# PKU-MARL/HARL

Hardware: AMD Instinct MI355X
Metric: transitions/sec through HAPPO update (MPE spread, 3 agents) (higher is better)
Workload: dtype f32; 1 GPU; MPE simple_spread_v2 3-agent HAPPO update: compute_returns + train(), T=200, n_rollout_threads=4096/GPU (4096 global, weak scaling), obs18/share54/Box5, MLP[128, 128], ppo_epoch=5, critic_epoch=5; episode_length=200, n_rollout_threads_per_gpu=4096, n_rollout_threads_global=4096, n_agents=3, parallelism=dp1, collective=none, world_size=1, ranks_seen=1

## Files before the change

### harl_amd/_lib.py

```python
from __future__ import annotations

import ctypes as C
import os
from typing import Dict, Optional

import torch

from .traffic import algorithmic_bytes, algorithmic_flops

_HERE = os.path.dirname(os.path.abspath(__file__))
LIB_PATH = os.path.join(_HERE, "lib", "libharl_%s.so" % (os.environ.get("HARL_LIB") or "hip"))

PS_STRIDE = 48
DHEAD_LD = 32
SLAB = 32

_vp, _i, _l, _f, _d = C.c_void_p, C.c_int, C.c_long, C.c_float, C.c_double

SIGNATURES = {
    "harl_gae_returns": [_vp] * 8 + [_i, _i, _f, _f, _i, _i, _i, _vp],
    "harl_masked_moments": [_vp, _vp, _l, _vp, _vp, _vp],
    "harl_dist_rows": [_vp, _l, _i, _i, _vp, _f, _f, _vp, _vp, _vp, _i, _i, _vp, _vp, _vp, _vp, _vp, _vp],
    "harl_moments_mean": [_vp, _vp, _vp],
    "harl_clock_probe": [_vp, _l, _vp],
    "harl_build_seq": [_vp, _i, _i, _i, _l, _vp, _vp, _i, _vp, _vp, _vp, _vp, _vp],
    "harl_adv_normalize": [_vp, _vp, _vp, _l, _vp],
    "harl_factor_update": [_vp, _vp, _vp, _l, _i, _i, _vp],
    "harl_sum_sumsq": [_vp, _vp, _l, _vp, _vp],
    "harl_valuenorm_apply": [_vp, _vp, _d, _d, _vp],
    "harl_gradnorm_clip_adam": [_vp, _vp, _vp, _vp, _l, _vp, _i, _f, _d, _d, _d, _f, _f, _d, _d, _vp, _vp],
    "harl_fold_linear": [_vp] * 6 + [_i, _i, _vp],
    "harl_unfold_linear_grads": [_vp, _vp, _i, _vp, _vp, _vp, _vp, _vp, _vp, _vp, _i, _i, _i, _vp],
    "harl_mlp_fwd_input": [_vp, _l, _vp, _l, _i, _vp, _vp, _i, _i, _vp, _vp, _vp, _vp, _vp, _vp, _vp],
    "harl_mlp_x0n_wide": [_vp, _l, _vp, _l, _i, _i, _vp, _vp, _vp, _vp],
    "harl_x0n_multi": [_vp, _i, _i, _vp],
    "harl_mlp_fwd_wide": [_vp, _l, _i, _vp, _i, _vp, _i, _vp, _vp, _vp, _vp, _vp],
    "harl_mlp_linear_wide": [_vp, _l, _i, _vp, _i, _vp, _i, _vp, _vp, _vp],
    "harl_act_ln_fwd": [_vp, _l, _i, _i, _vp, _vp, _vp, _vp],
    "harl_act_bwd": [_vp, _vp, _vp, _vp, _l, _i, _i, _vp],
    "harl_act_ln_tangent": [_vp, _vp, _vp, _vp, _vp, _l, _i, _i, _vp, _vp],
    "harl_mlp_tangent_wide": [_vp, _l, _i, _vp, _i, _vp, _i, _vp, _vp, _vp, _vp, _vp, _vp],
    "harl_mlp_fwd_fused2x": [_vp, _l, _vp, _i, _vp, _vp, _vp, _i, _i, _vp, _vp, _vp, _vp, _vp, _vp, _vp],
    "harl_mlp_fwd_fused2": [_vp, _l, _vp, _l, _i, _vp, _vp, _i, _vp, _vp, _i, _i, _vp, _vp, _vp, _vp, _vp, _vp, _vp, _vp,
                            _vp, _vp],
    "harl_mlp_fwd_hidden": [_vp, _l, _i, _i, _vp, _vp, _vp, _vp, _vp, _vp],
    "harl_mlp_bwd_dx": [_vp, _vp, _vp, _vp, _l, _i, _i, _vp, _vp, _vp, _i, _vp, _i, _vp],
    "harl_mlp_bwd_dx_dw": [_vp, _vp, _vp, _vp, _l, _i, _i, _vp, _vp, _vp, _i, _vp, _vp, _i, _i, _vp],
    "harl_mlp_dw_partials": [_vp, _i, _i, _i, _vp, _i, _l, _vp, _vp, _vp, _i, _l, _vp, _i, _vp],
    "harl_mlp_dw_partials_multi": [_i, _vp, _vp, _vp, _i, _i, _l, _i, _vp],
    "harl_mlp_dw_partials_multi_v": [_i, _vp, _vp, _vp, _i, _vp, _vp, _vp, _l, _i, _vp],
    "harl_gru_dw6": [_vp, _vp, _vp, _vp, _vp, _vp, _vp, _l, _i, _vp],
    "harl_mlp_fwd_trunk": [_vp, _l, _i, _vp, _i, _vp, _i, _vp, _i, _vp, _vp, _vp, _vp, _vp, _vp, _vp, _vp, _vp, _vp],
    "harl_mlp_bwd_trunk": [_l, _i, _i, _vp, _vp, _vp, _vp, _vp, _vp, _vp, _vp, _vp, _vp, _vp],
    "harl_reduce_partials": [_vp, _i, _l, _vp, _vp],
    "harl_reduce_partials_multi": [_vp, _vp, _i, _i, _l, _vp, _vp],
    "harl_adam_fold": [_vp, _vp, _vp, _vp, _l, _vp, _vp, _i, _vp, _vp, _vp, _i, _vp, _i, _f, _i, _i, _vp, _i, _f, _d, _d,
                       _d, _f, _f, _d, _d, _vp, _vp],
    "harl_adam_fold_dev": [_vp, _vp, _vp, _vp, _l, _vp, _vp, _i, _vp, _vp, _vp, _i, _vp, _i, _f, _i, _i, _vp, _i, _f, _vp, _i,
                           _vp, _d, _d, _f, _f, _vp, _vp],
    "harl_pack_scalars_hilo": [_vp, _vp, _vp],
    "harl_reduce_pack_scalars": [_vp, _i, _vp, _vp, _vp],
    "harl_randperm_replay": [_vp, _l, _l, _vp, _vp, _vp],
    "harl_rng_advance": [_vp, _l, _l, _vp],
    "harl_rng_jump": [_vp, _l, _l, _vp],
    "harl_actor_head_logp": [_vp, _l, _i, _vp, _vp, _vp, _f, _f, _i, _i, _vp, _vp, _vp, _vp, _vp, _i, _vp, _l, _l, _vp],
    "harl_actor_head_loss": [_vp, _vp, _vp, _l, _i, _vp, _vp, _vp, _f, _f, _i, _i, _vp, _vp, _vp, _vp, _vp, _vp,
                             _vp, _vp, _d, _f, _i, _i, _l, _l, _vp, _vp, _vp, _vp, _vp, _i, _vp],
    "harl_critic_head_values": [_vp, _l, _i, _vp, _vp, _vp, _vp],
    "harl_critic_head_loss": [_vp, _vp, _vp, _l, _i, _vp, _vp, _vp, _vp, _vp, _vp, _f, _i, _i, _f, _l, _l, _vp, _vp, _vp,
                              _vp, _i, _vp],
    "harl_gru_fwd": [_vp] * 7 + [_i, _i, _l] + [_vp] * 8 + [_i, _vp, _vp],
    "harl_gru_bwd": [_vp] * 9 + [_i, _i, _l] + [_vp] * 8 + [_vp],
    "harl_fold_linear_tangent": [_vp] * 9 + [_i, _i, _vp],
    "harl_fold_table": [_vp, _vp, _vp, _i, _i, _vp],
    "harl_unfold_table": [_vp, _vp, _vp, _vp, _i, _i, _vp],
    "harl_fold_tangent_table": [_vp, _vp, _vp, _vp, _i, _i, _vp],
    "harl_mlp_tangent_input": [_vp, _l, _vp, _l, _i, _vp, _vp, _i, _i, _vp, _vp, _vp, _vp, _vp],
    "harl_gru_gates": [_vp, _vp, _i, _l, _vp, _vp, _vp, _i, _vp],
    "harl_gru_tangent": [_vp] * 15 + [_i, _i, _l, _vp, _vp],
    "harl_mlp_tangent_hidden": [_vp, _vp, _l, _i, _i, _vp, _vp, _vp, _vp, _vp, _vp, _vp, _vp],
    "harl_mlp_tangent_hidden2": [_vp, _vp, _l, _i, _i, _vp, _vp, _vp, _vp, _vp, _vp, _vp, _vp, _vp],
    "harl_actor_head_fvp": [_vp, _vp, _vp, _vp, _l, _i, _vp, _vp, _vp, _vp, _vp, _f, _f, _i, _i, _vp, _l, _l, _vp, _vp, _vp],
    "harl_trpo_kl_sum": [_vp, _vp, _vp, _vp, _f, _f, _l, _i, _i, _vp, _vp],
    "harl_update_supported": [_i, _i, _i, _i],
    "harl_update_fwd_actor": [_vp, _l, _i, _i] + [_vp] * 7 + [_f, _f, _i, _i] + [_vp] * 7 + [_d, _f, _i, _i] + [_vp] * 4 + [_i] + [_vp] * 4,
    "harl_update_logp": [_vp, _l, _i, _i] + [_vp] * 7 + [_f, _f, _i, _i] + [_vp] * 5 + [_i, _vp, _vp],
    "harl_update_last_actor": [_vp, _l, _i] + [_vp] * 5 + [_f, _f, _i, _i] + [_vp] * 8 + [_d, _f, _i, _i] + [_vp] * 4 + [_i, _vp],
    "harl_update_last_critic": [_vp, _l, _i] + [_vp] * 8 + [_f, _i, _i, _f] + [_vp] * 3 + [_i, _vp],
    "harl_update_fwd_critic": [_vp, _l, _i, _i] + [_vp] * 9 + [_f, _i, _i, _f] + [_vp] * 3 + [_i] + [_vp] * 4,
    "harl_update_values": [_vp, _l, _i, _i] + [_vp] * 7 + [_vp],
    "harl_update_bwd": [_vp, _vp, _l, _i, _i] + [_vp] * 5 + [_i, _vp],
    "harl_head_blocks": [_l],
    "harl_trpo_fvp_finish": [_vp, _vp, _vp, _vp, _l, _f, _f, _l, _i, _f, _f, _vp],
    "harl_trpo_cg_step": [_vp, _vp, _vp, _vp, _l, _vp, _vp, _vp],
    "harl_mlp_panel_fwd": [_vp, _l, _i, _vp, _i, _vp, _i, _vp, _vp, _vp, _vp],
    "harl_mlp_panel_bwd": [_vp, _vp, _vp, _vp, _l, _i, _i, _vp, _vp, _vp],
    "harl_head_dw_rows256": [_vp, _l, _i, _vp, _vp, _i, _vp],
    "harl_mlp_panel_tangent": [_vp, _vp, _l, _i, _vp, _vp, _i, _vp, _vp, _vp, _vp, _vp, _vp],
    "harl_reduce_scalars": [_vp, _i, _vp, _vp],
    "harl_mlp_linear": [_vp, _l, _i, _i, _vp, _vp, _vp, _vp],
    "harl_mlp_linear3": [_vp, _vp, _vp, _l, _i, _i, _vp, _vp, _vp, _vp, _vp, _vp, _vp, _vp, _vp, _vp],
    "harl_gru_cell_init": [_vp, _vp, _i, _l, _vp, _vp],
    "harl_gru_cell_fwd": [_vp] * 8 + [_i, _l] + [_vp] * 7 + [_vp],
    "harl_gru_cell_bwd": [_vp] * 10 + [_i, _l] + [_vp] * 5 + [_vp],
    "harl_rownorm": [_vp, _l, _i, _vp, _vp, _vp],
    "harl_gru_cell_tangent": [_vp] * 19 + [_i, _l] + [_vp] * 3,
    "harl_md_head_logp": [_vp, _i, _vp, _i, _vp, _vp, _l, _vp, _vp, _vp, _i, _vp, _i, _vp, _l, _l, _vp],
    "harl_md_head_loss": [_vp, _vp, _i, _vp, _i, _vp, _vp, _l, _vp, _vp, _vp, _i, _vp, _vp, _vp, _vp, _vp, _d, _f, _i, _i,
                          _l, _l, _vp, _vp, _i, _vp],
    "harl_cat_head_logp": [_vp, _i, _vp, _i, _l, _vp, _vp, _vp, _vp, _vp, _vp, _vp, _vp, _l, _l, _vp],
    "harl_cat_head_loss": [_vp, _i, _vp, _i, _l, _vp, _vp, _vp, _vp, _vp, _vp, _vp, _vp, _d, _f, _i, _l, _l, _vp, _vp, _i, _vp],
    "harl_trpo_begin": [_vp, _vp, _l, _i, _vp, _vp, _vp, _vp, _l, _vp, _vp, _vp, _vp],
    "harl_trpo_step": [_vp, _vp, _vp, _vp, _vp, _vp, _l, _f, _vp, _vp, _vp],
    "harl_trpo_ls_candidate": [_vp, _vp, _vp, _vp, _l, _vp],
    "harl_trpo_ls_test": [_vp, _vp, _d, _d, _d, _d, _vp, _vp],
    "harl_reduce_scalars_set": [_vp, _i, _vp, _vp],
    "harl_zero_bytes": [_vp, _l, _vp],
    "harl_comm_create": [_i, _i, _l, _i, _vp, _vp],
    "harl_comm_connect": [_vp, _vp],
    "harl_comm_allreduce": [_vp, _vp, _l, _i, _vp],
    "harl_comm_set_timeout": [_vp, _d],
    "harl_comm_status": [_vp],
    "harl_comm_destroy": [_vp],
    "harl_version": [],
}


class HipLibraryMissing(RuntimeError):
    pass


_lib: Optional[C.CDLL] = None


def load() -> C.CDLL:
    global _lib
    if _lib is not None:
        return _lib
    if not os.path.exists(LIB_PATH):
        raise HipLibraryMissing(
            f"{LIB_PATH} not found: build it with `python -m harl_amd._build` (hipcc, gfx950). "
            "harl_amd has no CPU fallback.")
    lib = C.CDLL(LIB_PATH)
    for name, argtypes in SIGNATURES.items():
        fn = getattr(lib, name)
        fn.argtypes = argtypes
        fn.restype = C.c_int
    lib.harl_last_error.argtypes = []
    lib.harl_last_error.restype = C.c_char_p
    _lib = lib
    return lib


def ptr(t: Optional[torch.Tensor]) -> Optional[int]:
    if t is None:
        return None
    assert t.is_contiguous(), "harl_amd kernels need contiguous tensors"
    return t.data_ptr()


_raw_stream = getattr(torch._C, "_cuda_getCurrentRawStream", None)
_raw_device = getattr(torch._C, "_cuda_getDevice", None)


def stream() -> int:
    if _raw_stream is not None and _raw_device is not None:
        return _raw_stream(_raw_device())
    return torch.cuda.current_stream().cuda_stream

# ... 4 lines not shown

_timing_tags = None


_event_pool: list = []


def reserve_timing_events(n: int) -> None:
    while len(_event_pool) < n:
        _event_pool.append(torch.cuda.Event(enable_timing=True))


def enable_kernel_timing(on: bool, tags=None) -> None:
    global _timing_on, _timing_tags
    _timing_on = bool(on)
    _timing_tags = set(tags) if tags else None
    if on:
        _timing_events.clear()


def collect_kernel_timing() -> dict:
    torch.cuda.synchronize()
    out = {}
    for tag, evs in _timing_events.items():
        ms = [e[0].elapsed_time(e[1]) for e in evs]
        nb = [e[2] for e in evs if e[2] is not None]
        out[tag] = dict(n=len(ms), avg_ms=sum(ms) / max(len(ms), 1), total_ms=sum(ms),
                        bytes=sum(nb) if len(nb) == len(evs) and nb else None,
                        flops=sum(e[3] or 0.0 for e in evs))
    return out


_fn_cache: dict = {}


def call(name: str, *args, tag: Optional[str] = None) -> None:
    fn = _fn_cache.get(name)
    if fn is None:
        fn = _fn_cache[name] = getattr(load(), name)
    if _timing_on and tag is not None and (_timing_tags is None or tag in _timing_tags):
        a = _event_pool.pop() if _event_pool else torch.cuda.Event(enable_timing=True)
        b = _event_pool.pop() if _event_pool else torch.cuda.Event(enable_timing=True)
        a.record()
        rc = fn(*args)
        b.record()
        _timing_events.setdefault(tag, []).append((a, b, algorithmic_bytes(name, args), algorithmic_flops(name, args)))
    else:
        rc = fn(*args)
    if rc != 0:
        raise RuntimeError(f"{name} failed ({rc}): {load().harl_last_error().decode()}")


X0N_MULTI_MAX = 32


class X0nProblem(C.Structure):
    _fields_ = [("X", _vp), ("ldx", _l), ("M", _l), ("D", _i), ("use_ln0", _i), ("x0n", _vp), ("mu0", _vp), ("rstd0", _vp)]


def x0n_multi(problems, max_workgroups: int = 0, tag: Optional[str] = "x0n_multi") -> bool:
    if not 1 <= len(problems) <= X0N_MULTI_MAX:
        return False
    table = (X0nProblem * len(problems))(*[X0nProblem(*p) for p in problems])
    fn = _fn_cache.get("harl_x0n_multi")
    if fn is None:
        fn = _fn_cache["harl_x0n_multi"] = load().harl_x0n_multi
    timed = _timing_on and tag is not None and (_timing_tags is None or tag in _timing_tags)
    if timed:
        a = _event_pool.pop() if _event_pool else torch.cuda.Event(enable_timing=True)
        b = _event_pool.pop() if _event_pool else torch.cuda.Event(enable_timing=True)
        a.record()
    rc = fn(table, len(problems), max_workgroups, stream())
    if rc == 1:
        return False
    if rc != 0:
        raise RuntimeError(f"harl_x0n_multi failed ({rc}): {load().harl_last_error().decode()}")
    if timed:
        b.record()
        nb = sum(4 * ((p[2] + 31) // 32 * 32) * (p[3] + (p[3] + 31) // 32 * 32 + 2) for p in problems)
        _timing_events.setdefault(tag, []).append((a, b, nb, 0.0))
    return True


SCRATCH_BYTES = {"mm": 24640, "cg": 1088}
_scratch: Dict[tuple, torch.Tensor] = {}


def scratch(kind: str) -> int:
    st = torch.cuda.current_stream()
    key = (st.device_index, st.cuda_stream, kind)
    t = _scratch.get(key)
    if t is None:
        t = _scratch[key] = torch.zeros(SCRATCH_BYTES[kind] // 8, dtype=torch.float64, device=torch.device("cuda", st.device_index))
    return t.data_ptr()


def default_device() -> torch.device:
    return torch.device(os.environ.get("HARL_DEVICE") or f"cuda:{int(os.environ.get('LOCAL_RANK', '0'))}")


def require_gpu(device: torch.device) -> None:
    if device.type != "cuda" or not torch.cuda.is_available():
        raise RuntimeError(
            "harl_amd runs on MI355X (PyTorch-ROCm device 'cuda') only; there is no CPU path. "
            f"Got device={device}, torch.cuda.is_available()={torch.cuda.is_available()}")
    load()
```

### harl_amd/csrc/elementwise.hip

```cpp
#include <mutex>
#include <map>
#include <unordered_map>
#include <utility>

#include "common.h"
#include "../../include/harl_hip.h"

#include <cstdio>
#include <cstring>

namespace harl {
bool lds_opt_in_needed(const void *kernel, size_t bytes) {
  static std::mutex mu;
  static std::unordered_map<const void *, size_t> done;
  std::lock_guard<std::mutex> lk(mu);
  size_t &have = done[kernel];
  if (have >= bytes) return false;
  have = bytes;
  return true;
}

static thread_local char g_err[512] = "";
void set_error(const char *msg) {
  std::strncpy(g_err, msg, sizeof(g_err) - 1);
// ... 62 lines not shown
  if (GAE) value_preds[(long)T * N + c] = nv;
  else returns[(long)T * N + c] = nv;
  auto load = [&](int t0, float (&r)[GAE_TC], float (&v0)[GAE_TC], float (&m1)[GAE_TC], float (&b1)[GAE_TC]) {
#pragma unroll
    for (int k = 0; k < GAE_TC; ++k) {
      const int t = t0 - k;
      const bool ok = t >= 0;
      const long o = (long)(ok ? t : 0) * N + c;
      r[k] = rewards[o];
      v0[k] = value_preds[o];
      m1[k] = masks[o + N];
      b1[k] = PTL ? bad_masks[o + N] : 1.f;
    }
  };
  auto scan = [&](int t0, const float (&r)[GAE_TC], const float (&v0)[GAE_TC], const float (&m1)[GAE_TC], const float (&b1)[GAE_TC]) {
#pragma clang fp contract(off)
#pragma unroll
    for (int k = 0; k < GAE_TC; ++k) {
      const int t = t0 - k;
      if (t < 0) break;
      const float dv0 = denorm(ds, v0[k]);
      float ret;
      if (GAE) {
        float delta = r[k] + (gamma * dv1) * m1[k];
        delta = delta - dv0;
        const float carry = FP_ORDER ? (gl * gae) * m1[k] : (gl * m1[k]) * gae;
        gae = delta + carry;
        if (PTL) gae = b1[k] * gae;
        ret = gae + dv0;
        dv1 = dv0;
      } else {
        ret = (ret1 * gamma) * m1[k] + r[k];
        if (PTL) ret = ret * b1[k] + (1.f - b1[k]) * dv0;
        ret1 = ret;
      }
      returns[(long)t * N + c] = ret;
      if (adv) adv[(long)t * N + c] = ret - dv0;
    }
  };
  float rA[GAE_TC], vA[GAE_TC], mA[GAE_TC], bA[GAE_TC], rB[GAE_TC], vB[GAE_TC], mB[GAE_TC], bB[GAE_TC];
  int t0 = T - 1;
  load(t0, rA, vA, mA, bA);
  while (t0 >= 0) {
    if (t0 - GAE_TC >= 0) load(t0 - GAE_TC, rB, vB, mB, bB);
    scan(t0, rA, vA, mA, bA);
    t0 -= GAE_TC;
    if (t0 < 0) break;
    if (t0 - GAE_TC >= 0) load(t0 - GAE_TC, rA, vA, mA, bA);
    scan(t0, rB, vB, mB, bB);
    t0 -= GAE_TC;
  }
}

extern "C" int harl_gae_returns(const float *rewards, float *value_preds, const float *masks,
                                const float *bad_masks, const float *next_value, const float *vn_stats,
                                float *returns, float *advantages, int T, int ncols, float gamma,
                                float gamma_lambda, int use_gae, int use_proper_time_limits, int fp_order,
                                void *stream) {
  if (T <= 0 || ncols <= 0) return 0;
  dim3 block(64), grid((ncols + 63) / 64);
  hipStream_t s = (hipStream_t)stream;
#define LAUNCH(G, P, F)                                                                                     \
  hipLaunchKernelGGL((k_gae<G, P, F>), grid, block, 0, s, rewards, value_preds, masks, bad_masks, next_value, \
                     vn_stats, returns, advantages, T, ncols, gamma, gamma_lambda)
  if (use_gae) {
    if (use_proper_time_limits) {
      if (fp_order) LAUNCH(true, true, true); else LAUNCH(true, true, false);
    } else {
      if (fp_order) LAUNCH(true, false, true); else LAUNCH(true, false, false);
    }
  } else {
    if (use_proper_time_limits) LAUNCH(false, true, false); else LAUNCH(false, false, false);
  }
#undef LAUNCH
  return check_launch("harl_gae_returns");
}

constexpr int MM_MAX_BLOCKS = 1024;
struct MmScratch {
  double part[MM_MAX_BLOCKS][3];
  unsigned ticket;
};

__global__ __launch_bounds__(256) void k_masked_moments(const float *__restrict__ x, const float *__restrict__ active,
                                                        long n, double *__restrict__ out3, MmScratch *__restrict__ ws) {
  double(*g_mm_part)[3] = ws->part;
  unsigned &g_mm_ticket = ws->ticket;
  double s1 = 0, s2 = 0, cnt = 0;
  for (long i = (long)blockIdx.x * blockDim.x + threadIdx.x; i < n; i += (long)gridDim.x * blockDim.x) {
    float a = active ? active[i] : 1.f;
    if (a != 0.f) {
      double v = x[i];
      s1 += v;
      s2 += v * v;
      cnt += 1.0;
    }
  }
  s1 = wave_reduce_sum_d(s1);
  s2 = wave_reduce_sum_d(s2);
  cnt = wave_reduce_sum_d(cnt);
  __shared__ double sh[3][4];
  __shared__ unsigned s_last;
  int w = threadIdx.x >> 6, l = threadIdx.x & 63;
  if (l == 0) {
    sh[0][w] = s1;
    sh[1][w] = s2;
    sh[2][w] = cnt;
  }
  __syncthreads();
  if (threadIdx.x < 3)
    __hip_atomic_store(&g_mm_part[blockIdx.x][threadIdx.x],
                       sh[threadIdx.x][0] + sh[threadIdx.x][1] + sh[threadIdx.x][2] + sh[threadIdx.x][3], __ATOMIC_RELAXED,
                       __HIP_MEMORY_SCOPE_AGENT);
  __syncthreads();
  if (threadIdx.x == 0) {
    __threadfence();
    s_last = __hip_atomic_fetch_add(&g_mm_ticket, 1u, __ATOMIC_ACQ_REL, __HIP_MEMORY_SCOPE_AGENT) == gridDim.x - 1 ? 1u : 0u;
  }
  __syncthreads();
  if (!s_last) return;
  __threadfence();
  __shared__ double red[3][256];
  for (int k = 0; k < 3; ++k) {
    double t = 0;
    for (unsigned b = threadIdx.x; b < gridDim.x; b += 256)
      t += __hip_atomic_load(&g_mm_part[b][k], __ATOMIC_RELAXED, __HIP_MEMORY_SCOPE_AGENT);
    red[k][threadIdx.x] = t;
  }
  __syncthreads();
  if (threadIdx.x < 3) {
    double t = 0;
    for (int i = 0; i < 256; ++i) t += red[threadIdx.x][i];
    out3[threadIdx.x] += t;
  }
}

static_assert(sizeof(MmScratch) <= HARL_MM_SCRATCH_BYTES, "HARL_MM_SCRATCH_BYTES too small");

extern "C" int harl_masked_moments(const float *x, const float *active, long n, double *out3, void *scratch, void *stream) {
  if (n <= 0) return 0;
  long nb = (n + 2047) / 2048;
  if (nb > MM_MAX_BLOCKS) nb = MM_MAX_BLOCKS;
  hipStream_t s = (hipStream_t)stream;
  MmScratch *ws = static_cast<MmScratch *>(scratch);
  if (!ws || (reinterpret_cast<uintptr_t>(ws) & 7) != 0) {
    set_error("harl_masked_moments: scratch must be HARL_MM_SCRATCH_BYTES of 8-byte aligned device memory");
    return -2;
  }
  (void)hipMemsetAsync(&ws->ticket, 0, sizeof(unsigned), s);
  hipLaunchKernelGGL(k_masked_moments, dim3((unsigned)nb), dim3(256), 0, s, x, active, n, out3, ws);
  return check_launch("harl_masked_moments");
}

__global__ __launch_bounds__(256) void k_adv_normalize(const float *__restrict__ adv, const double *__restrict__ mom,
                                                       float *__restrict__ out, long n) {
  double cnt = mom[2];
  double meand = mom[0] / cnt;
  double vard = mom[1] / cnt - meand * meand;
  float mean = (float)meand;
  float denom = (float)sqrt(vard > 0 ? vard : 0.0) + 1e-5f;
  for (long i = (long)blockIdx.x * blockDim.x + threadIdx.x; i < n; i += (long)gridDim.x * blockDim.x)
    out[i] = (adv[i] - mean) / denom;
}

extern "C" int harl_adv_normalize(const float *adv, const double *moments3, float *adv_out, long n, void *stream) {
  if (n <= 0) return 0;
  long nb = (n + 1023) / 1024;
  if (nb > 2048) nb = 2048;
  hipLaunchKernelGGL(k_adv_normalize, dim3((unsigned)nb), dim3(256), 0, (hipStream_t)stream, adv, moments3, adv_out, n);
  return check_launch("harl_adv_normalize");
}

__global__ __launch_bounds__(256) void k_dist_rows(const float *__restrict__ head, long M, int D, int kind,
                                                   const float *__restrict__ log_std, float std_x_coef, float std_y_coef,
                                                   const float *__restrict__ noise, float *__restrict__ actions,
                                                   const int *__restrict__ head_off, int n_heads, int sum_heads,
                                                   float *__restrict__ logp, float *__restrict__ probs,
                                                   float *__restrict__ argmax_out, float *__restrict__ ent_rows,
                                                   float *__restrict__ sigma_out) {
  const long i = (long)blockIdx.x * blockDim.x + threadIdx.x;
  if (kind == 0) {
    if (sigma_out && i < D) sigma_out[i] = (1.0f / (1.0f + expf(-log_std[i] / std_x_coef))) * std_y_coef;
    if (i >= M) return;
    float ent = 0.f;
    for (int d = 0; d < D; ++d) {
      const float sig = (1.0f / (1.0f + expf(-log_std[d] / std_x_coef))) * std_y_coef;
      const float lsig = logf(sig);
      const float mu = head[i * D + d];
      const float a = noise ? mu + sig * noise[i * D + d] : mu;
      if (actions) actions[i * D + d] = a;
      if (logp) {
        const float diff = a - mu;
        logp[i * D + d] = -(diff * diff) / (2.0f * sig * sig) - lsig - 0.9189385332046727f;
      }
      ent += 0.5f + 0.9189385332046727f + lsig;
    }
    if (ent_rows) ent_rows[i] = ent;
    return;
  }
  if (i >= M) return;
  float ent = 0.f, lsum = 0.f;
  for (int hd = 0; hd < n_heads; ++hd) {
    const int lo = head_off ? head_off[hd] : 0, hi = head_off ? head_off[hd + 1] : D;
    int best = lo;
    float bv = head[i * D + lo];
    for (int j = lo; j < hi; ++j) {
      const float lg = head[i * D + j];
      const float p = expf(lg);
      if (probs) probs[i * D + j] = p;
      ent -= fmaxf(lg, -3.4028234663852886e38f) * p;
      if (lg > bv) {
        bv = lg;
        best = j;
      }
    }
    if (argmax_out) argmax_out[i * n_heads + hd] = (float)(best - lo);
    if (logp) {
// ... 59 lines not shown
    return -1;
  }
  const long work = (long)L * m_pad > (long)m_pad * H ? (long)L * m_pad : (long)m_pad * H;
  long blocks = (work + 255) / 256;
  if (blocks > 1024) blocks = 1024;
  hipLaunchKernelGGL(k_build_seq, dim3((unsigned)blocks), dim3(256), 0, (hipStream_t)stream, first, m, m_pad, L, stride,
                     masks_src, h0_src, H, idx, valid_idx, mask_rows, h0);
  return check_launch("harl_build_seq");
}

__global__ void k_clock_probe(long long *__restrict__ out, long long ticks) {
  if (threadIdx.x != 0) return;
  const long long r0 = __builtin_amdgcn_s_memrealtime();
  const long long c0 = __builtin_readcyclecounter();
  long long r;
  do {
    __builtin_amdgcn_s_sleep(64);
    r = __builtin_amdgcn_s_memrealtime();
  } while (r - r0 < ticks);
  out[0] = __builtin_readcyclecounter() - c0;
  out[1] = r - r0;
}

extern "C" int harl_clock_probe(long long *cycles_ticks, long ticks, void *stream) {
  if (ticks <= 0 || ticks > 100000000L) {
    set_error("harl_clock_probe: ticks must be in (0, 1e8]");
    return -1;
  }
  hipLaunchKernelGGL(k_clock_probe, dim3(1), dim3(64), 0, (hipStream_t)stream, cycles_ticks, (long long)ticks);
  return check_launch("harl_clock_probe");
}

__global__ __launch_bounds__(256) void k_factor_update(float *__restrict__ factor, const float *__restrict__ nl,
                                                       const float *__restrict__ ol, long n, int D, int agg_mean) {
  for (long i = (long)blockIdx.x * blockDim.x + threadIdx.x; i < n; i += (long)gridDim.x * blockDim.x) {
    float acc = agg_mean ? 0.f : 1.f;
    for (int d = 0; d < D; ++d) {
      float r = expf(nl[i * D + d] - ol[i * D + d]);
      acc = agg_mean ? acc + r : acc * r;
    }
    if (agg_mean) acc = acc / (float)D;
    factor[i] = factor[i] * acc;
  }
}

extern "C" int harl_factor_update(float *factor, const float *new_logp, const float *old_logp, long n, int act_dim,
                                  int agg_mean, void *stream) {
  if (n <= 0) return 0;
  long nb = (n + 255) / 256;
  if (nb > 2048) nb = 2048;
  hipLaunchKernelGGL(k_factor_update, dim3((unsigned)nb), dim3(256), 0, (hipStream_t)stream, factor, new_logp, old_logp,
                     n, act_dim, agg_mean);
  return check_launch("harl_factor_update");
}

__global__ __launch_bounds__(256) void k_sum_sumsq(const float *__restrict__ x, const int64_t *__restrict__ idx, long m,
                                                   double *__restrict__ out2) {
  double s1 = 0, s2 = 0;
  for (long i = (long)blockIdx.x * blockDim.x + threadIdx.x; i < m; i += (long)gridDim.x * blockDim.x) {
    double v = x[idx ? idx[i] : i];
    s1 += v;
    s2 += v * v;
  }
  s1 = wave_reduce_sum_d(s1);
  s2 = wave_reduce_sum_d(s2);
  __shared__ double sh[2][4];
  int w = threadIdx.x >> 6, l = threadIdx.x & 63;
  if (l == 0) {
    sh[0][w] = s1;
    sh[1][w] = s2;
  }
  __syncthreads();
  if (threadIdx.x < 2) atomicAdd(&out2[threadIdx.x], sh[threadIdx.x][0] + sh[threadIdx.x][1] + sh[threadIdx.x][2] + sh[threadIdx.x][3]);
}

extern "C" int harl_sum_sumsq(const float *x, const int64_t *idx, long m, double *sums2, void *stream) {
  if (m <= 0) return 0;
  long nb = (m + 2047) / 2048;
  if (nb > 1024) nb = 1024;
  hipLaunchKernelGGL(k_sum_sumsq, dim3((unsigned)nb), dim3(256), 0, (hipStream_t)stream, x, idx, m, sums2);
  return check_launch("harl_sum_sumsq");
}

__global__ void k_valuenorm_apply(float *__restrict__ vn, const double *__restrict__ sums2, double count, float w,
                                  float omw) {
#pragma clang fp contract(off)
  if (threadIdx.x == 0 && blockIdx.x == 0) {
    float bm = (float)(sums2[0] / count);
    float bsq = (float)(sums2[1] / count);
    float rm = vn[0] * w;
    vn[0] = rm + bm * omw;
    float rs = vn[1] * w;
    vn[1] = rs + bsq * omw;
    float db = vn[2] * w;
    vn[2] = db + omw;
  }
}

extern "C" int harl_valuenorm_apply(float *vn_stats, const double *sums2, double count, double beta, void *stream) {
  float w = (float)beta;
  float omw = (float)(1.0 - beta);
  hipLaunchKernelGGL(k_valuenorm_apply, dim3(1), dim3(64), 0, (hipStream_t)stream, vn_stats, sums2, count, w, omw);
  return check_launch("harl_valuenorm_apply");
}

__global__ __launch_bounds__(1024) void k_gradnorm_clip_adam(float *__restrict__ p, const float *__restrict__ g,
                                                             float *__restrict__ m, float *__restrict__ v, long n,
                                                             const float *__restrict__ grad_scale, int use_clip,
                                                             float max_norm, float lr_over_bc1, float beta1,
                                                             float beta2, float omb1, float omb2, float eps, float wd,
                                                             float bc2_sqrt, double *__restrict__ info_out) {
  const float scale = grad_scale ? *grad_scale : 1.f;
  double ss = 0;
  for (long i = threadIdx.x; i < n; i += blockDim.x) {
    float gi = g[i] * scale;
    ss += (double)gi * gi;
  }
  ss = wave_reduce_sum_d(ss);
  __shared__ double sh[16];
  __shared__ float s_coef;
  int w = threadIdx.x >> 6, l = threadIdx.x & 63;
  if (l == 0) sh[w] = ss;
  __syncthreads();
  if (threadIdx.x == 0) {
    double t = 0;
    for (int i = 0; i < (int)(blockDim.x >> 6); ++i) t += sh[i];
    float norm = (float)sqrt(t);
    float coef = 1.f;
    if (use_clip) {
      coef = max_norm / (norm + 1e-6f);
      coef = coef > 1.f ? 1.f : coef;
    }
    s_coef = coef;
    if (info_out) info_out[0] += norm;
  }
  __syncthreads();
  const float coef = s_coef * scale;
  for (long i = threadIdx.x; i < n; i += blockDim.x) {
    float gi = g[i] * coef;
    float pi = p[i];
    if (wd != 0.f) gi = gi + wd * pi;
    float mi = m[i];
    mi = mi + omb1 * (gi - mi);
    float vi = v[i] * beta2 + (omb2 * gi) * gi;
    m[i] = mi;
    v[i] = vi;
    float denom = sqrtf(vi) / bc2_sqrt + eps;
    p[i] = pi - lr_over_bc1 * (mi / denom);
  }
}

extern "C" int harl_gradnorm_clip_adam(float *param, float *grad, float *exp_avg, float *exp_avg_sq, long n,
                                       const float *grad_scale, int use_clip, float max_norm, double lr, double beta1,
                                       double beta2, float eps, float weight_decay, double bias_correction1,
                                       double bias_correction2, double *info_out, void *stream) {
  if (n <= 0) return 0;
  float step_size = (float)(lr / bias_correction1);
  float bc2_sqrt = (float)sqrt(bias_correction2);
  hipLaunchKernelGGL(k_gradnorm_clip_adam, dim3(1), dim3(1024), 0, (hipStream_t)stream, param, grad, exp_avg,
                     exp_avg_sq, n, grad_scale, use_clip, max_norm, step_size, (float)beta1, (float)beta2,
                     (float)(1.0 - beta1), (float)(1.0 - beta2), eps, weight_decay, bc2_sqrt, info_out);
  return check_launch("harl_gradnorm_clip_adam");
}

__global__ __launch_bounds__(64) void k_fold_linear(const float *__restrict__ W, const float *__restrict__ b,
                                                    const float *__restrict__ gamma, const float *__restrict__ beta,
// ... 279 lines not shown
  __shared__ double sh[16][64];
  const int j = threadIdx.x & 63, rg = threadIdx.x >> 6;
  double s = 0;
  if (j < PS_STRIDE)
    for (int b = rg; b < n_blocks; b += 16) s += (double)ps[(long)b * PS_STRIDE + j];
  sh[rg][j] = s;
  __syncthreads();
  if (threadIdx.x < PS_STRIDE) {
    double r = 0;
#pragma unroll
    for (int g = 0; g < 16; ++g) r += sh[g][threadIdx.x];
    out[threadIdx.x] = r;
#pragma unroll
    for (int k = 0; k < HILO_PIECES; ++k) {
      const double p = trunc(r / HILO_Q[k]) * HILO_Q[k];
      hilo[k * PS_STRIDE + threadIdx.x] = (float)p;
      r -= p;
    }
  }
}

extern "C" int harl_reduce_pack_scalars(const float *part_scalars, int n_blocks, double *scalars, float *hilo, void *stream) {
  if (n_blocks > 0 && !part_scalars) { set_error("harl_reduce_pack_scalars: part_scalars is NULL"); return -2; }
  hipLaunchKernelGGL(k_reduce_pack_scalars, dim3(1), dim3(1024), 0, (hipStream_t)stream, part_scalars, n_blocks, scalars, hilo);
  return check_launch("harl_reduce_pack_scalars");
}

constexpr int TS = 12;

__global__ __launch_bounds__(64) void k_unfold_table(const float *__restrict__ p, float *__restrict__ g,
                                                     const float *__restrict__ dwp, const int *__restrict__ tab, int n_layers) {
  int k = blockIdx.x, l = 0;
  for (; l < n_layers; ++l) {
    if (k < tab[l * TS + 5]) break;
    k -= tab[l * TS + 5];
  }
  if (l >= n_layers) return;
  const int *t = tab + l * TS;
  const int O = t[4], K = t[5], kp = t[9], op = t[10], go = t[2], beo = t[3];
  const float *dW_ = dwp + t[8];
  const float *db_ = dW_ + (long)op * kp;
  const float gam = go >= 0 ? p[go + k] : 1.f, bet = beo >= 0 ? p[beo + k] : 0.f;
  for (int o = threadIdx.x; o < O; o += 64) {
    const float d = dW_[(long)o * kp + k], dbo = db_[o];
    g[t[0] + (long)o * K + k] = d * gam + dbo * bet;
    if (k == 0) g[t[1] + o] = dbo;
  }
  if (go < 0) return;
  for (int l2 = 0; l2 < l; ++l2)
    if (tab[l2 * TS + 2] == go) return;
  float accg = 0.f, accb = 0.f;
  bool first = true;
  for (int l2 = l; l2 < n_layers; ++l2) {
    const int *t2 = tab + l2 * TS;
    if (t2[2] != go) continue;
    const int O2 = t2[4], K2 = t2[5], kp2 = t2[9], op2 = t2[10];
    const float *dW2 = dwp + t2[8];
    const float *db2 = dW2 + (long)op2 * kp2;
    double sg = 0.0, sb = 0.0;
    for (int o = threadIdx.x; o < O2; o += 64) {
      const float w = p[t2[0] + (long)o * K2 + k];
      sg += (double)w * (double)dW2[(long)o * kp2 + k];
      sb += (double)w * (double)db2[o];
    }
    sg = wave_reduce_sum_d(sg);
    sb = wave_reduce_sum_d(sb);
    accg = first ? (float)sg : (float)((double)accg + sg);
    accb = first ? (float)sb : (float)((double)accb + sb);
    first = false;
  }
  if (threadIdx.x == 0) {
    g[go + k] = accg;
    g[beo + k] = accb;
  }
}

extern "C" int harl_unfold_table(const float *param, float *grad, const float *dwp, const int *table, int n_layers,
                                 int total_cols, void *stream) {
  if (n_layers <= 0 || total_cols <= 0) return 0;
  hipLaunchKernelGGL(k_unfold_table, dim3(total_cols), dim3(64), 0, (hipStream_t)stream, param, grad, dwp, table, n_layers);
  return check_launch("harl_unfold_table");
}

__global__ __launch_bounds__(64) void k_fold_table(const float *__restrict__ p, float *__restrict__ packs,
                                                   const int *__restrict__ tab, int n_layers) {
  int o = blockIdx.x, l = 0;
  for (; l < n_layers; ++l) {
    if (o < tab[l * TS + 4]) break;
    o -= tab[l * TS + 4];
  }
  if (l >= n_layers) return;
  const int *t = tab + l * TS;
  const int in_dim = t[5];
  const float *W = p + t[0], *b = p + t[1];
  const float *gamma = t[2] >= 0 ? p + t[2] : nullptr, *beta = t[3] >= 0 ? p + t[3] : nullptr;
  float *Wp = packs + t[6], *bp = packs + t[7];
  float acc = 0.f;
  for (int k = threadIdx.x; k < in_dim; k += 64) {
    float w = W[(long)o * in_dim + k];
    Wp[(long)o * in_dim + k] = gamma ? w * gamma[k] : w;
    if (beta) acc += w * beta[k];
  }
  acc = wave_reduce_sum(acc);
  if (threadIdx.x == 0) bp[o] = b[o] + acc;
}

extern "C" int harl_fold_table(const float *param, float *packs, const int *table, int n_layers, int total_rows, void *stream) {
  if (n_layers <= 0 || total_rows <= 0) return 0;
  hipLaunchKernelGGL(k_fold_table, dim3(total_rows), dim3(64), 0, (hipStream_t)stream, param, packs, table, n_layers);
  return check_launch("harl_fold_table");
}

__global__ __launch_bounds__(64) void k_fold_tangent_table(const float *__restrict__ p, const float *__restrict__ vec,
                                                           float *__restrict__ packd, const int *__restrict__ tab, int n_layers) {
  int o = blockIdx.x, l = 0;
  for (; l < n_layers; ++l) {
    if (o < tab[l * TS + 4]) break;
    o -= tab[l * TS + 4];
  }
  if (l >= n_layers) return;
  const int *t = tab + l * TS;
  const int K = t[5], go = t[2], beo = t[3];
  const float *W = p + t[0] + (long)o * K, *Wd = vec + t[0] + (long)o * K;
  float *Wpd = packd + t[6] + (long)o * K;
  float acc = 0.f;
  for (int k = threadIdx.x; k < K; k += 64) {
    const float w = W[k], wd = Wd[k];
    Wpd[k] = go >= 0 ? wd * p[go + k] + w * vec[go + k] : wd;
    if (beo >= 0) acc += wd * p[beo + k] + w * vec[beo + k];
  }
  acc = wave_reduce_sum(acc);
  if (threadIdx.x == 0) packd[t[7] + o] = vec[t[1] + o] + acc;
}

extern "C" int harl_fold_tangent_table(const float *param, const float *vec, float *pack_d, const int *table, int n_layers,
                                       int total_rows, void *stream) {
  if (n_layers <= 0 || total_rows <= 0) return 0;
  hipLaunchKernelGGL(k_fold_tangent_table, dim3(total_rows), dim3(64), 0, (hipStream_t)stream, param, vec, pack_d, table,
                     n_layers);
  return check_launch("harl_fold_tangent_table");
}

#ifndef HARL_REDUCE_DEPTH
#define HARL_REDUCE_DEPTH 16
#endif
__global__ __launch_bounds__(256) void k_reduce_partials_multi(const float *__restrict__ part, const int *__restrict__ tab,
                                                               int n_layers, int n_wg, float *__restrict__ dwp) {
  __shared__ double sh[4][64];
  const int lane = threadIdx.x & 63, rg = threadIdx.x >> 6;
  long e = (long)blockIdx.x * 64 + lane;
  double total = 0.0;
  long out_idx = -1;
  for (int l = 0; l < n_layers; ++l) {
    const int *t = tab + l * TS;
    const long elems = (long)t[10] * t[9] + t[10];
    if (e < elems) {
      const float *p = part + (long)t[11] + e;
      constexpr int RD = HARL_REDUCE_DEPTH;
      double acc[RD];
#pragma unroll
      for (int u = 0; u < RD; ++u) acc[u] = 0.0;
      int w = rg;
      for (; w + 4 * (RD - 1) < n_wg; w += 4 * RD) {
        float v[RD];
#pragma unroll
        for (int u = 0; u < RD; ++u) v[u] = p[(long)(w + 4 * u) * elems];
#pragma unroll
        for (int u = 0; u < RD; ++u) acc[u] += (double)v[u];
      }
      for (; w < n_wg; w += 4) acc[0] += (double)p[(long)w * elems];
#pragma unroll
      for (int st = 1; st < RD; st *= 2)
#pragma unroll
        for (int u = 0; u + st < RD; u += 2 * st) acc[u] += acc[u + st];
      total = acc[0];
      out_idx = t[8] + e;
      break;
    }
    e -= elems;
  }
  sh[rg][lane] = total;
  __syncthreads();
  if (rg == 0 && out_idx >= 0) dwp[out_idx] = (float)((sh[0][lane] + sh[1][lane]) + (sh[2][lane] + sh[3][lane]));
}

extern "C" int harl_reduce_partials_multi(const float *part, const int *table, int n_layers, int n_wg, long total_elems,
                                          float *dwp, void *stream) {
  if (total_elems <= 0) return 0;
  hipLaunchKernelGGL(k_reduce_partials_multi, dim3((unsigned)((total_elems + 63) / 64)), dim3(256), 0,
                     (hipStream_t)stream, part, table, n_layers, n_wg, dwp);
  return check_launch("harl_reduce_partials_multi");
}

// ... 674 lines not shown
```

### harl_amd/csrc/heads.hip

```cpp
#include "common.h"
#include "../../include/harl_hip.h"

using namespace harl;

#include "heads_common.h"

namespace {

template <int H, int DAP, bool DISCRETE, bool TRAIN, bool FUSE = false>
__global__ __launch_bounds__(WG_THREADS, (FUSE && DAP <= 8) ? 2 : 1) void k_actor_head(ActorArgs A) {
  extern __shared__ __attribute__((aligned(16))) float lds[];
  PHASE_BEGIN();
  float *whl = lds;
  float *cst = whl + 2 * (H / 2) * DAP;
  float *red = cst + 7 * DAP;
  float *dwl = red + 4 * PS_STRIDE;
  constexpr bool LDSACC = FUSE && DAP <= 8;
  constexpr int HROWS = DAP <= 8 ? DAP : 8;
  float *hacc = dwl + WAVES_PER_WG * HeadDw<H>::WAVE_FLOATS;
  if (FUSE)
    for (int e = threadIdx.x; e < WAVES_PER_WG * HeadDw<H>::WAVE_FLOATS; e += WG_THREADS) dwl[e] = 0.f;
  if (LDSACC)
    for (int e = threadIdx.x; e < WAVES_PER_WG * HROWS * H; e += WG_THREADS) hacc[e] = 0.f;
  stage_head<H, DAP>(whl, cst, A.Whp, A.bhp, A.act_dim);
// ... 410 lines not shown
  for (int k = threadIdx.x; k < in_dim; k += 64) {
    const float w = W[(long)o * in_dim + k], wd = Wd[(long)o * in_dim + k];
    Wpd[(long)o * in_dim + k] = g ? wd * g[k] + w * gd[k] : wd;
    if (be) acc += wd * be[k] + w * bed[k];
  }
  acc = wave_reduce_sum(acc);
  if (threadIdx.x == 0) bpd[o] = bd[o] + acc;
}

template <int H, int DAP, bool DISC>
void launch_fvp(const FvpArgs &A, int grid, hipStream_t s) {
  const size_t shm = ((size_t)4 * (H / 2) * DAP + 10 * DAP) * sizeof(float);
  allow_big_lds(k_actor_head_fvp<H, DAP, DISC>, shm);
  hipLaunchKernelGGL((k_actor_head_fvp<H, DAP, DISC>), dim3(grid), dim3(WG_THREADS), shm, s, A);
}

int head_grid(long M) { return persistent_grid(n_slabs_of(M), 4); }

template <int H, int DAP, bool DISC, bool TRAIN>
void launch_actor(const ActorArgs &A, int grid, hipStream_t s) {
  const size_t base = ((size_t)2 * (H / 2) * DAP + 7 * DAP + 4 * PS_STRIDE) * sizeof(float);
  if constexpr (TRAIN && DAP <= 32) {
    if (A.dw_part) {
      size_t fl = (size_t)WAVES_PER_WG * HeadDw<H>::WAVE_FLOATS;
      if (fl < (size_t)HeadDw<H>::OUT_FLOATS) fl = HeadDw<H>::OUT_FLOATS;
      if (DAP <= 8) fl = (size_t)WAVES_PER_WG * HeadDw<H>::WAVE_FLOATS + (size_t)WAVES_PER_WG * DAP * H;
      const size_t shm = base + fl * sizeof(float);
      allow_big_lds(k_actor_head<H, DAP, DISC, true, true>, shm);
      hipLaunchKernelGGL((k_actor_head<H, DAP, DISC, true, true>), dim3(grid), dim3(WG_THREADS), shm, s, A);
      return;
    }
  }
  hipLaunchKernelGGL((k_actor_head<H, DAP, DISC, TRAIN>), dim3(grid), dim3(WG_THREADS), base, s, A);
}

template <bool TRAIN>
int dispatch_actor(const ActorArgs &A, int H, int discrete, int grid, hipStream_t s) {
  const int D = A.act_dim;
  if (D < 1 || D > 64 || (D > 32 && !discrete)) {
    set_error("actor head: act_dim must be in [1, 32] (Categorical heads: [1, 64])");
    return -2;
  }
  if (D > 32 && A.dw_part) {
    set_error("actor head: the fused head weight gradient stops at 32 outputs (pass dw_part = NULL and run harl_mlp_dw_partials on the ATL(64) dhead image)");
    return -2;
  }
  const int dap = D <= 4 ? 4 : (D <= 8 ? 8 : (D <= 16 ? 16 : (D <= 32 ? 32 : 64)));
#define CASE(Hv, DAPv)                                                    \
  if (H == Hv && dap == DAPv) {                                           \
    if (discrete) launch_actor<Hv, DAPv, true, TRAIN>(A, grid, s);        \
    else launch_actor<Hv, DAPv, false, TRAIN>(A, grid, s);                \
    return check_launch("harl_actor_head");                               \
  }
  CASE(128, 4) CASE(128, 8) CASE(128, 16) CASE(128, 32) CASE(64, 4) CASE(64, 8) CASE(64, 16) CASE(64, 32)
  CASE(256, 4) CASE(256, 8) CASE(256, 16) CASE(256, 32)
#undef CASE
  if (dap == 64 && (H == 64 || H == 128)) {
    if (H == 64) launch_actor<64, 64, true, TRAIN>(A, grid, s);
    else launch_actor<128, 64, true, TRAIN>(A, grid, s);
    return check_launch("harl_actor_head");
  }
  set_error("actor head: hidden width must be 64 or 128");
  return -2;
}
}

HARL_PHASE_ACCESSOR(heads)

extern "C" int harl_head_blocks(long M) { return head_grid(M); }

extern "C" int harl_actor_head_logp(const float *xL, long M, int H, const float *Whp, const float *bhp,
                                    const float *log_std, float std_x_coef, float std_y_coef, int discrete,
                                    int act_dim, const float *actions, const float *avail, float *logp_out,
                                    const float *old_logp, float *factor, int agg_mean, float *head_out, long m_valid,
                                    long m_pad, void *stream) {
  if (M <= 0) return 0;
  ActorArgs A{};
  A.head_out = head_out;
  A.m_valid = m_valid; A.m_pad = m_pad;
  A.xL = xL; A.M = M; A.Whp = Whp; A.bhp = bhp; A.log_std = log_std;
  A.std_x_coef = std_x_coef; A.std_y_coef = std_y_coef; A.act_dim = act_dim;
  A.actions = actions; A.avail = avail; A.old_logp = old_logp; A.agg_mean = agg_mean;
  A.logp_out = logp_out; A.factor_out = factor; A.n_slabs = n_slabs_of(M);
  if (factor && !old_logp) {
    set_error("harl_actor_head_logp: factor update needs old_logp");
    return -2;
  }
  return dispatch_actor<false>(A, H, discrete, head_grid(M), (hipStream_t)stream);
}

extern "C" int harl_actor_head_loss(const float *xL, const uint32_t *relu_mask, const float *rstd, long M, int H,
                                    const float *Whp, const float *bhp, const float *log_std, float std_x_coef,
                                    float std_y_coef, int discrete, int act_dim, const int64_t *idx,
                                    const float *actions, const float *avail, const float *old_logp, const float *adv,
                                    const double *adv_moments, const float *factor, const float *active,
                                    double clip_param, float entropy_coef, int agg_mean, int trpo, long m_valid,
                                    long m_pad, float *logp_out, float *dzL, float *dhead, float *part_scalars,
                                    float *dw_part, int n_wg, void *stream) {
  if (M <= 0) return 0;
  ActorArgs A{};
  A.trpo = trpo;
  A.logp_out = logp_out;
  A.dw_part = dw_part;
  if (dw_part && n_wg <= 0) { set_error("harl_actor_head_loss: fused head gradient needs n_wg > 0"); return -2; }
  A.m_valid = m_valid; A.m_pad = m_pad;
  A.xL = xL; A.relu_mask = relu_mask; A.rstd = rstd; A.M = M; A.Whp = Whp; A.bhp = bhp; A.log_std = log_std;
  A.std_x_coef = std_x_coef; A.std_y_coef = std_y_coef; A.act_dim = act_dim; A.idx = idx;
  A.actions = actions; A.avail = avail; A.old_logp = old_logp; A.adv = adv; A.adv_moments = adv_moments;
  A.factor_in = factor; A.active = active; A.entropy_coef = entropy_coef;
  A.clip_lo = (float)(1.0 - clip_param); A.clip_hi = (float)(1.0 + clip_param);
  A.agg_mean = agg_mean; A.dzL = dzL; A.dhead = dhead; A.part_scalars = part_scalars; A.n_slabs = n_slabs_of(M);
  return dispatch_actor<true>(A, H, discrete, dw_part ? n_wg : head_grid(M), (hipStream_t)stream);
}

extern "C" int harl_critic_head_values(const float *xL, long M, int H, const float *Whp, const float *bhp,
                                       float *values, void *stream) {
  if (M <= 0) return 0;
  CriticArgs A{};
  A.xL = xL; A.M = M; A.Whp = Whp; A.bhp = bhp; A.values_out = values; A.n_slabs = n_slabs_of(M);
  const int grid = head_grid(M);
  const size_t shm = ((size_t)2 * (H / 2) * 4 + 20 + 4 * PS_STRIDE) * sizeof(float);
  if (H == 128) hipLaunchKernelGGL((k_critic_head<128, false>), dim3(grid), dim3(WG_THREADS), shm, (hipStream_t)stream, A);
  else if (H == 64) hipLaunchKernelGGL((k_critic_head<64, false>), dim3(grid), dim3(WG_THREADS), shm, (hipStream_t)stream, A);
  else if (H == 256) hipLaunchKernelGGL((k_critic_head<256, false>), dim3(grid), dim3(WG_THREADS), shm, (hipStream_t)stream, A);
  else { set_error("critic head: hidden width must be 64, 128 or 256"); return -2; }
  return check_launch("harl_critic_head_values");
}

extern "C" int harl_critic_head_loss(const float *xL, const uint32_t *relu_mask, const float *rstd, long M, int H,
                                     const float *Whp, const float *bhp, const int64_t *idx, const float *value_preds,
                                     const float *returns, const float *vn_stats, float clip_param, int use_clipped,
                                     int use_huber, float huber_delta, long m_valid, long m_pad, float *dzL, float *dhead,
                                     float *part_scalars, float *dw_part, int n_wg, void *stream) {
  if (M <= 0) return 0;
  CriticArgs A{};
  A.m_valid = m_valid; A.m_pad = m_pad;
  A.xL = xL; A.relu_mask = relu_mask; A.rstd = rstd; A.M = M; A.Whp = Whp; A.bhp = bhp; A.idx = idx;
  A.value_preds = value_preds; A.returns = returns; A.vn_stats = vn_stats; A.clip_param = clip_param;
  A.huber_delta = huber_delta; A.use_clipped = use_clipped; A.use_huber = use_huber; A.dzL = dzL; A.dhead = dhead;
  A.part_scalars = part_scalars; A.n_slabs = n_slabs_of(M);
  A.dw_part = dw_part;
  if (dw_part && n_wg <= 0) { set_error("harl_critic_head_loss: fused head gradient needs n_wg > 0"); return -2; }
  const int grid = dw_part ? n_wg : head_grid(M);
  const size_t base = ((size_t)2 * (H / 2) * 4 + 20 + 4 * PS_STRIDE) * sizeof(float);
  hipStream_t s = (hipStream_t)stream;
#define CL(Hv)                                                                                                     \
  if (H == Hv) {                                                                                                   \
    if (dw_part) {                                                                                                 \
      const size_t fl = (size_t)WAVES_PER_WG * HeadDw<Hv>::WAVE_FLOATS + (size_t)WAVES_PER_WG * Hv;    \
      const size_t shm = base + fl * sizeof(float);                                                                \
      allow_big_lds(k_critic_head<Hv, true, true>, shm);                                                           \
      hipLaunchKernelGGL((k_critic_head<Hv, true, true>), dim3(grid), dim3(WG_THREADS), shm, s, A);                \
    } else {                                                                                                       \
      hipLaunchKernelGGL((k_critic_head<Hv, true>), dim3(grid), dim3(WG_THREADS), base, s, A);                     \
    }                                                                                                              \
    return check_launch("harl_critic_head_loss");                                                                  \
  }
  CL(128) CL(64) CL(256)
#undef CL
  set_error("critic head: hidden width must be 64 or 128");
  return -2;
}

extern "C" int harl_actor_head_fvp(const float *xL, const float *xLdot, const uint32_t *relu_mask, const float *rstd, long M,
                                   int H, const float *Whp, const float *bhp, const float *Whdp, const float *bhdp,
                                   const float *log_std, float std_x_coef, float std_y_coef, int discrete, int act_dim,
// ... 52 lines not shown
```

### harl_amd/csrc/heads_common.h

```cpp
#pragma once
#include "common.h"

using namespace harl;

namespace {
constexpr float LOG_SQRT_2PI = 0.918938533204672741780329736406f;
constexpr float HALF_LOG_2PI_PLUS_HALF = 1.418938533204672741780329736406f;

struct ActorArgs {
  const float *xL;
  const uint32_t *relu_mask;
  const float *rstd;
  long M;
  const float *Whp, *bhp, *log_std;
  float std_x_coef, std_y_coef;
  int act_dim;
  const int64_t *idx;
  const float *actions, *avail, *old_logp, *adv;
  const double *adv_moments;
  const float *factor_in, *active;
  float clip_lo, clip_hi, entropy_coef;
  int agg_mean;
  float *dzL, *dhead, *part_scalars;
  float *dw_part;
// ... 364 lines not shown
        float *p = buf + 32 * H + lane;
        *p = (w == 0 ? 0.f : *p) + v;
      }
    }
    __syncthreads();
  }
  for (int e = threadIdx.x; e < HeadDw<H>::OUT_FLOATS; e += WG_THREADS) out[e] = buf[e];
}

template <int DAP>
__device__ __forceinline__ void store_dhead(float *__restrict__ dhead, long slab, int lane, const float (&dzh)[DAP]) {
  const int i = lane & 31, h = lane >> 5;
  if constexpr (DAP <= 32) {
    float *dh = dhead + (slab * SLAB + i) * DHEAD_LD + 16 * h;
#pragma unroll
    for (int c = 0; c < 16; ++c) {
      float v0 = 0.f, v1 = 0.f;
      if (c < DAP) v0 = dzh[c < DAP ? c : 0];
      if (16 + c < DAP) v1 = dzh[16 + c < DAP ? 16 + c : 0];
      dh[c] = h ? v1 : v0;
    }
  } else {
    static_assert(DAP == 64, "wide heads are padded to 64 outputs");
    float v[32];
#pragma unroll
    for (int R = 0; R < 32; ++R) {
      const int f0 = 32 * (R >> 4) + (R & 3) + 8 * ((R & 15) >> 2);
      v[R] = h ? dzh[f0 + 4] : dzh[f0];
    }
    atl_store<64>(dhead, slab, lane, v);
  }
}

template <int NV>
__device__ __forceinline__ void block_reduce_store(float (&v)[NV], float *red , float *out_row) {
  const int lane = threadIdx.x & 63, wave = wave_id();
#pragma unroll
  for (int k = 0; k < NV; ++k) {
    float t = wave_reduce_sum(v[k]);
    if (lane == 0) red[wave * PS_STRIDE + k] = t;
  }
  __syncthreads();
  if (threadIdx.x < PS_STRIDE) {
    float t = 0.f;
    if (threadIdx.x < NV)
      t = (red[0 * PS_STRIDE + threadIdx.x] + red[1 * PS_STRIDE + threadIdx.x]) +
          (red[2 * PS_STRIDE + threadIdx.x] + red[3 * PS_STRIDE + threadIdx.x]);
    out_row[threadIdx.x] = t;
  }
}

template <int DAP>
struct ActorRow {
  float a[DAP];
  float olp[DAP];
  float av[DAP];
  float act, adv, fct;
};
template <int DAP, bool DISCRETE, bool TRAIN, int DA = 0>
__device__ __forceinline__ void actor_row_load(const ActorArgs &A, long slab, int lane, ActorRow<DAP> &R) {
  const int i = lane & 31;
  const int D = DA ? DA : A.act_dim;
  const long j = slab * SLAB + i;
  const long jc = j < A.M ? j : A.M - 1;
  const long row = A.idx ? A.idx[jc] : jc;
  const long orow = TRAIN ? row : jc;
  if (!DISCRETE) {
#pragma unroll
    for (int d = 0; d < DAP; ++d) {
      R.a[d] = (A.actions && d < D) ? A.actions[row * D + d] : 0.f;
      R.olp[d] = ((TRAIN || A.old_logp) && d < D) ? A.old_logp[orow * D + d] : 0.f;
    }
  } else {
    R.a[0] = A.actions ? A.actions[row] : 0.f;
    R.olp[0] = (TRAIN || A.old_logp) ? A.old_logp[orow] : 0.f;
#pragma unroll
    for (int d = 0; d < DAP; ++d) R.av[d] = (A.avail && d < D) ? A.avail[row * D + d] : 1.f;
  }
  if (TRAIN) {
    R.act = A.active ? A.active[row] : 1.f;
    R.adv = A.adv[row];
    R.fct = A.factor_in ? A.factor_in[row] : 1.f;
  } else {
    R.fct = A.factor_out ? A.factor_out[jc] : 1.f;
  }
}

__device__ __forceinline__ long row_index_request(const int64_t *idx, const float *mapped, long slab, int lane, long M) {
  const long j = slab * SLAB + (lane & 31);
  const long jc = j < M ? j : M - 1;
  const int64_t *p = idx ? idx + jc : reinterpret_cast<const int64_t *>(mapped);
  return *p;
}
__device__ __forceinline__ long row_index_resolve(const int64_t *idx, long raw, long slab, int lane, long M) {
  const long j = slab * SLAB + (lane & 31);
  return idx ? raw : (j < M ? j : M - 1);
}
template <int DAP, bool DISCRETE, bool TRAIN, int DA>
__device__ __forceinline__ void actor_row_load_at(const ActorArgs &A, long slab, int lane, long row, ActorRow<DAP> &R) {
  static_assert(DA > 0 && DA <= DAP, "compile-time action width");
  const long j = slab * SLAB + (lane & 31);
  const long jc = j < A.M ? j : A.M - 1;
  const long orow = TRAIN ? row : jc;
  const float *mapped = A.Whp;
  const bool has_olp = TRAIN || A.old_logp;
  if (!DISCRETE) {
    const float *ap = A.actions ? A.actions + row * DA : mapped;
    const float *op = has_olp ? A.old_logp + orow * DA : mapped;
#pragma unroll
    for (int d = 0; d < DAP; ++d) {
      R.a[d] = d < DA ? ap[d < DA ? d : 0] : 0.f;
      R.olp[d] = d < DA ? op[d < DA ? d : 0] : 0.f;
    }
  } else {
    R.a[0] = *(A.actions ? A.actions + row : mapped);
    R.olp[0] = *(has_olp ? A.old_logp + orow : mapped);
    const float *vp = A.avail ? A.avail + row * DA : mapped;
#pragma unroll
    for (int d = 0; d < DAP; ++d) R.av[d] = d < DA ? vp[d < DA ? d : 0] : 1.f;
  }
  if (TRAIN) {
    R.act = *(A.active ? A.active + row : mapped);
    R.adv = A.adv[row];
    R.fct = *(A.factor_in ? A.factor_in + row : mapped);
  } else {
    R.fct = *(A.factor_out ? A.factor_out + jc : mapped);
  }
}

template <int DAP, bool DISCRETE, bool TRAIN, int DA = 0>
__device__ __forceinline__ bool actor_sample(const ActorArgs &A, const float *cst, float (&z)[DAP], long slab, int lane,
                                             float adv_mean, float adv_den, float (&sc)[8 + DAP], float (&dzh)[DAP],
                                             float &s1_out, float &s2_out, const ActorRow<DAP> &R) {
  const int i = lane & 31, h = lane >> 5;
  const int D = DA ? DA : A.act_dim;
  const int act_w = DISCRETE ? 1 : D;
  const float inv_D = uniform_f(1.0f / (float)D);
  float zlin[DAP];
#pragma unroll
  for (int d = 0; d < DAP; ++d) zlin[d] = z[d] - cst[d];

  const long j = slab * SLAB + i;
  const bool valid = j < A.M && (A.m_pad == 0 || (j % A.m_pad) < A.m_valid);
  const long jc = j < A.M ? j : A.M - 1;
  const long row = A.idx ? A.idx[jc] : jc;
  const bool count_me = valid && h == 0;

#pragma unroll
  for (int d = 0; d < DAP; ++d) dzh[d] = 0.f;

  float imp = 1.f;
  float ratio_d[DAP];
  float ent = 0.f;
  float logp_d[DAP];

  if (!DISCRETE) {
    float prod = 1.f, sum = 0.f;
#pragma unroll
    for (int d = 0; d < DAP; ++d) {
      ratio_d[d] = 1.f;
      logp_d[d] = 0.f;
      if (d < D) {
        const float sig = cst[DAP + d], lsig = cst[2 * DAP + d];
        const float a = A.actions ? R.a[d] : z[d];
        const float diff = a - z[d];
        const float var = sig * sig;
        const float lp = -(diff * diff) * (0.5f * cst[6 * DAP + d]) - lsig - LOG_SQRT_2PI;
        logp_d[d] = lp;
        ent += HALF_LOG_2PI_PLUS_HALF + lsig;
        if (TRAIN || A.old_logp) {
          const float r = expf(lp - R.olp[d]);
          ratio_d[d] = r;
          prod *= r;
          sum += r;
        }
      }
    }
    imp = A.agg_mean ? sum * inv_D : prod;
  } else {
    float mx = -3.0e38f;
#pragma unroll
    for (int d = 0; d < DAP; ++d) {
      if (d < D) {
        if (A.avail && R.av[d] == 0.f) z[d] = -1e10f;
        mx = fmaxf(mx, z[d]);
      }
    }
    float se = 0.f;
#pragma unroll
    for (int d = 0; d < DAP; ++d)
      if (d < D) se += expf(z[d] - mx);
    const float lse = mx + logf(se);
    const int a = A.actions ? (int)R.a[0] : 0;
    float lpa = 0.f;
#pragma unroll
    for (int d = 0; d < DAP; ++d) {
      logp_d[d] = 0.f;
      ratio_d[d] = 0.f;
      if (d < D) {
        const float lp = z[d] - lse;
        logp_d[d] = lp;
        const float p = expf(lp);
        ratio_d[d] = p;
        ent -= fmaxf(lp, -3.4028234663852886e38f) * p;
        if (d == a) lpa = lp;
      }
    }
    if (TRAIN || A.old_logp) imp = expf(lpa - R.olp[0]);
    z[0] = lpa;
  }

  if (!TRAIN) {
    if (valid && h == 0 && A.head_out) {
#pragma unroll
      for (int d = 0; d < DAP; ++d)
        if (d < D) A.head_out[j * D + d] = DISCRETE ? logp_d[d] : z[d];
    }
    if (valid && h == 0) {
      if (A.logp_out) {
        if (DISCRETE) A.logp_out[j] = z[0];
        else {
#pragma unroll
          for (int d = 0; d < DAP; ++d)
            if (d < D) A.logp_out[j * D + d] = logp_d[d];
        }
      }
      if (A.factor_out) A.factor_out[j] = R.fct * imp;
    }
    return false;
  }

  if (A.logp_out && valid && h == 0) {
    if (DISCRETE) A.logp_out[j] = z[0];
    else {
#pragma unroll
      for (int d = 0; d < DAP; ++d)
        if (d < D) A.logp_out[j * D + d] = logp_d[d];
    }
  }
  const float act = A.active ? R.act : 1.f;
  const float advn = (R.adv - adv_mean) * adv_den;
  const float fct = A.factor_in ? R.fct : 1.f;
  const float lo = A.clip_lo, hi = A.clip_hi;
  const float surr1 = imp * advn;
  const float impc = fminf(fmaxf(imp, lo), hi);
  const float surr2 = impc * advn;
  const float mn = fminf(surr1, surr2);
  const float inrange = (imp >= lo && imp <= hi) ? 1.f : 0.f;
  float gsel = surr1 < surr2 ? 1.f : (surr1 > surr2 ? inrange : 0.5f + 0.5f * inrange);
  if (A.trpo != 0) gsel = 1.f;
  const float dimp = valid ? (A.trpo == 1 ? fct * act * advn : -fct * act * advn * gsel) : 0.f;
  const float ecoef = (valid && A.trpo != 1) ? -A.entropy_coef * act : 0.f;

  if (count_me) {
    sc[0] += A.trpo == 1 ? surr1 * fct * act : -fct * (A.trpo == 2 ? surr1 : mn) * act;
    sc[1] += act;
    sc[2] += ent * act;
    sc[3] += imp;
    sc[4] += 1.f;
  }

  if (!DISCRETE) {
#pragma unroll
    for (int d = 0; d < DAP; ++d) {
      if (d < D) {
        const float sig = cst[DAP + d];
        const float var = sig * sig;
        const float a = R.a[d];
        const float diff = a - z[d];
        const float dlp = dimp * (A.agg_mean ? ratio_d[d] * inv_D : imp);
        const float isig = cst[5 * DAP + d], ivar = cst[6 * DAP + d];
        dzh[d] = dlp * diff * ivar;
        const float dsig = dlp * (diff * diff * ivar * isig - isig) + ecoef * isig;
        if (h == 0) sc[8 + d] += dsig * cst[3 * DAP + d];
      }
    }
  } else {
    const int a = (int)R.a[0];
    const float dlp = dimp * imp;
#pragma unroll
    for (int d = 0; d < DAP; ++d) {
      if (d < D) {
        const float p = ratio_d[d];
        const float onehot = d == a ? 1.f : 0.f;
        dzh[d] = dlp * (onehot - p) + ecoef * (-p * (logp_d[d] + ent));
        if (p == 0.f) dzh[d] = dlp * onehot;
      }
    }
  }
  float s1 = 0.f, s2 = 0.f;
#pragma unroll
  for (int d = 0; d < DAP; ++d) {
    s1 += dzh[d] * cst[4 * DAP + d];
    s2 += dzh[d] * zlin[d];
  }
  s1_out = s1;
  s2_out = s2;
  return true;
}

struct CriticArgs {
  const float *xL;
  const uint32_t *relu_mask;
  const float *rstd;
  long M;
  const float *Whp, *bhp;
  const int64_t *idx;
  const float *value_preds, *returns, *vn_stats;
  float clip_param, huber_delta;
  long m_valid, m_pad;
// ... 66 lines not shown
```

### harl_amd/csrc/update.hip

```cpp
#include <type_traits>
#include "common.h"
#include "split_mfma.h"
#include "heads_common.h"
#include "mfma_transpose.h"
#include "../../include/harl_hip.h"

using namespace harl;

namespace {

int bad(const char *m) {
  set_error(m);
  return -2;
}

template <int H, bool MASK>
__device__ __forceinline__ void relu_ln(const f32x16 (&acc)[H / 32], float (&v)[H / 2], uint32_t (&bits)[(H / 2 + 31) / 32],
                                        float &rstd_out) {
  constexpr int NR = H / 2;
#pragma unroll
  for (int w = 0; w < (NR + 31) / 32; ++w) bits[w] = 0u;
#pragma unroll
  for (int R = 0; R < NR; ++R) {
    if constexpr (MASK) v[R] = relu_push(acc[R >> 4][R & 15], bits[R >> 5]);
// ... 579 lines not shown
#define CASE(Hv, Kv)                                                                \
  if (H == Hv && kp0 == Kv) {                                                       \
    const int rc = launch_actor_width<Hv, Kv, TRAIN>(U, A, discrete, s);             \
    return rc ? rc : check_launch("harl_update_fwd");                               \
  }
  CASE(128, 32) CASE(128, 64) CASE(64, 32) CASE(64, 64)
#undef CASE
  return bad("harl_update_fwd: hidden width must be 64 or 128");
}

int dispatch_last_actor(const UpdFwdArgs &U, const ActorArgs &A, int H, int discrete, hipStream_t s) {
  const int D = A.act_dim;
  if (D < 1 || D > 8) return bad("harl_update_last_actor: act_dim must be in [1, 8]");
  int rc;
  if (H == 128) rc = launch_actor_width<128, 0, true>(U, A, discrete, s);
  else if (H == 64) rc = launch_actor_width<64, 0, true>(U, A, discrete, s);
  else return bad("harl_update_last_actor: hidden width must be 64 or 128");
  return rc ? rc : check_launch("harl_update_last_actor");
}

int dispatch_last_critic(const UpdFwdArgs &U, const CriticArgs &A, int H, hipStream_t s) {
  int rc;
  if (H == 128) rc = launch_fwd<128, 0, 1, false, true, CriticArgs>(U, A, s);
  else if (H == 64) rc = launch_fwd<64, 0, 1, false, true, CriticArgs>(U, A, s);
  else return bad("harl_update_last_critic: hidden width must be 64 or 128");
  return rc ? rc : check_launch("harl_update_last_critic");
}

template <bool TRAIN>
int dispatch_fwd_critic(const UpdFwdArgs &U, const CriticArgs &A, int H, hipStream_t s) {
  const int kp0 = U.D <= 32 ? 32 : 64;
#define CASE(Hv, Kv)                                                     \
  if (H == Hv && kp0 == Kv) {                                            \
    const int rc = launch_fwd<Hv, Kv, 1, false, TRAIN, CriticArgs>(U, A, s); \
    return rc ? rc : check_launch("harl_update_fwd");                        \
  }
  CASE(128, 32) CASE(128, 64) CASE(64, 32) CASE(64, 64)
#undef CASE
  return bad("harl_update_fwd: hidden width must be 64 or 128");
}

}

HARL_PHASE_ACCESSOR(update)

extern "C" int harl_update_supported(int D, int H, int act_dim, int kind) {
  if (!(D >= 0 && D <= 64 && (H == 64 || H == 128) && act_dim >= 1 && act_dim <= 8)) return 0;
  const int dap = act_dim <= 4 ? 4 : 8;
  const int hrows = kind == 0 ? 0 : (kind == 2 ? 1 : act_dim);
  return fwd_lds_bytes(H, D == 0 ? 0 : (D <= 32 ? 32 : 64), dap, hrows, kind == 2 ? 1 : act_dim) <= LDS_PER_WG_MAX ? 1 : 0;
}

extern "C" int harl_update_fwd_actor(const float *x0n, long M, int D, int H, const float *W1p, const float *b1p,
                                     const float *W2p, const float *b2p, const float *Whp, const float *bhp,
                                     const float *log_std, float std_x_coef, float std_y_coef, int discrete, int act_dim,
                                     const float *actions, const float *avail, const float *old_logp, const float *adv,
                                     const double *adv_moments, const float *factor, const float *active,
                                     double clip_param, float entropy_coef, int agg_mean, int trpo, float *logp_out,
                                     float *dz2, float *part_scalars, float *dw_part_head, int n_part_rows, float *xh1,
                                     uint32_t *rmask1, float *rstd1, void *stream) {
  if (M <= 0) return 0;
  if (D < 1 || D > 64) return bad("harl_update_fwd_actor: input width must be <= 64");
  if (!dz2 || !part_scalars || !dw_part_head || n_part_rows <= 0) return bad("harl_update_fwd_actor: missing outputs");
  if (xh1 && (!rmask1 || !rstd1)) return bad("harl_update_fwd_actor: xh1 needs rmask1 and rstd1");
  UpdFwdArgs U{x0n, W1p, b1p, W2p, b2p, D, n_slabs_of(M), dz2, n_part_rows, xh1, rmask1, rstd1};
  if (fwd_grid(U.n_slabs) > n_part_rows) return bad("harl_update_fwd_actor: n_part_rows smaller than the launch grid");
  ActorArgs A{};
  A.trpo = trpo;
  A.logp_out = logp_out;
  A.dw_part = dw_part_head;
  A.M = M; A.Whp = Whp; A.bhp = bhp; A.log_std = log_std;
  A.std_x_coef = std_x_coef; A.std_y_coef = std_y_coef; A.act_dim = act_dim;
  A.actions = actions; A.avail = avail; A.old_logp = old_logp; A.adv = adv; A.adv_moments = adv_moments;
  A.factor_in = factor; A.active = active; A.entropy_coef = entropy_coef;
  A.clip_lo = (float)(1.0 - clip_param); A.clip_hi = (float)(1.0 + clip_param);
  A.agg_mean = agg_mean; A.part_scalars = part_scalars; A.n_slabs = U.n_slabs;
  return dispatch_fwd_actor<true>(U, A, H, discrete, (hipStream_t)stream);
}

extern "C" int harl_update_logp(const float *x0n, long M, int D, int H, const float *W1p, const float *b1p,
                                const float *W2p, const float *b2p, const float *Whp, const float *bhp,
                                const float *log_std, float std_x_coef, float std_y_coef, int discrete, int act_dim,
                                const float *actions, const float *avail, float *logp_out, const float *old_logp,
                                float *factor, int agg_mean, float *head_out, void *stream) {
  if (M <= 0) return 0;
  if (D < 1 || D > 64) return bad("harl_update_logp: input width must be <= 64");
  if (factor && !old_logp) return bad("harl_update_logp: factor update needs old_logp");
  UpdFwdArgs U{x0n, W1p, b1p, W2p, b2p, D, n_slabs_of(M), nullptr, 0, nullptr, nullptr, nullptr};
  ActorArgs A{};
  A.head_out = head_out;
  A.M = M; A.Whp = Whp; A.bhp = bhp; A.log_std = log_std;
  A.std_x_coef = std_x_coef; A.std_y_coef = std_y_coef; A.act_dim = act_dim;
  A.actions = actions; A.avail = avail; A.old_logp = old_logp; A.agg_mean = agg_mean;
  A.logp_out = logp_out; A.factor_out = factor; A.n_slabs = U.n_slabs;
  return dispatch_fwd_actor<false>(U, A, H, discrete, (hipStream_t)stream);
}

extern "C" int harl_update_fwd_critic(const float *x0n, long M, int D, int H, const float *W1p, const float *b1p,
                                      const float *W2p, const float *b2p, const float *Whp, const float *bhp,
                                      const float *value_preds, const float *returns, const float *vn_stats,
                                      float clip_param, int use_clipped, int use_huber, float huber_delta, float *dz2,
                                      float *part_scalars, float *dw_part_head, int n_part_rows, float *xh1,
                                      uint32_t *rmask1, float *rstd1, void *stream) {
  if (M <= 0) return 0;
  if (D < 1 || D > 64) return bad("harl_update_fwd_critic: input width must be <= 64");
  if (!dz2 || !part_scalars || !dw_part_head || n_part_rows <= 0) return bad("harl_update_fwd_critic: missing outputs");
  if (xh1 && (!rmask1 || !rstd1)) return bad("harl_update_fwd_critic: xh1 needs rmask1 and rstd1");
  UpdFwdArgs U{x0n, W1p, b1p, W2p, b2p, D, n_slabs_of(M), dz2, n_part_rows, xh1, rmask1, rstd1};
  if (fwd_grid(U.n_slabs) > n_part_rows) return bad("harl_update_fwd_critic: n_part_rows smaller than the launch grid");
  CriticArgs A{};
  A.M = M; A.Whp = Whp; A.bhp = bhp;
  A.value_preds = value_preds; A.returns = returns; A.vn_stats = vn_stats; A.clip_param = clip_param;
  A.huber_delta = huber_delta; A.use_clipped = use_clipped; A.use_huber = use_huber;
  A.part_scalars = part_scalars; A.n_slabs = U.n_slabs;
  A.dw_part = dw_part_head;
  return dispatch_fwd_critic<true>(U, A, H, (hipStream_t)stream);
}

extern "C" int harl_update_last_actor(const float *xin, long M, int H, const float *Wp, const float *bp, const float *Whp,
                                      const float *bhp, const float *log_std, float std_x_coef, float std_y_coef,
                                      int discrete, int act_dim, const int64_t *idx, const float *actions,
                                      const float *avail, const float *old_logp, const float *adv,
                                      const double *adv_moments, const float *factor, const float *active,
                                      double clip_param, float entropy_coef, int agg_mean, int trpo, float *logp_out,
                                      float *dz, float *part_scalars, float *dw_part_head, int n_part_rows, void *stream) {
  if (M <= 0) return 0;
  if (!xin || !dz || !part_scalars || !dw_part_head || n_part_rows <= 0) return bad("harl_update_last_actor: missing arguments");
  UpdFwdArgs U{xin, nullptr, nullptr, Wp, bp, 0, n_slabs_of(M), dz, n_part_rows, nullptr, nullptr, nullptr};
  if (fwd_grid(U.n_slabs) > n_part_rows) return bad("harl_update_last_actor: n_part_rows smaller than the launch grid");
  ActorArgs A{};
  A.trpo = trpo;
  A.logp_out = logp_out;
  A.dw_part = dw_part_head;
  A.M = M; A.Whp = Whp; A.bhp = bhp; A.log_std = log_std;
  A.std_x_coef = std_x_coef; A.std_y_coef = std_y_coef; A.act_dim = act_dim; A.idx = idx;
  A.actions = actions; A.avail = avail; A.old_logp = old_logp; A.adv = adv; A.adv_moments = adv_moments;
  A.factor_in = factor; A.active = active; A.entropy_coef = entropy_coef;
  A.clip_lo = (float)(1.0 - clip_param); A.clip_hi = (float)(1.0 + clip_param);
  A.agg_mean = agg_mean; A.part_scalars = part_scalars; A.n_slabs = U.n_slabs;
  return dispatch_last_actor(U, A, H, discrete, (hipStream_t)stream);
}

extern "C" int harl_update_last_critic(const float *xin, long M, int H, const float *Wp, const float *bp, const float *Whp,
                                       const float *bhp, const int64_t *idx, const float *value_preds, const float *returns,
                                       const float *vn_stats, float clip_param, int use_clipped, int use_huber,
                                       float huber_delta, float *dz, float *part_scalars, float *dw_part_head,
                                       int n_part_rows, void *stream) {
  if (M <= 0) return 0;
  if (!xin || !dz || !part_scalars || !dw_part_head || n_part_rows <= 0) return bad("harl_update_last_critic: missing arguments");
  UpdFwdArgs U{xin, nullptr, nullptr, Wp, bp, 0, n_slabs_of(M), dz, n_part_rows, nullptr, nullptr, nullptr};
  if (fwd_grid(U.n_slabs) > n_part_rows) return bad("harl_update_last_critic: n_part_rows smaller than the launch grid");
  CriticArgs A{};
  A.M = M; A.Whp = Whp; A.bhp = bhp; A.idx = idx;
  A.value_preds = value_preds; A.returns = returns; A.vn_stats = vn_stats; A.clip_param = clip_param;
  A.huber_delta = huber_delta; A.use_clipped = use_clipped; A.use_huber = use_huber;
  A.part_scalars = part_scalars; A.n_slabs = U.n_slabs;
  A.dw_part = dw_part_head;
  return dispatch_last_critic(U, A, H, (hipStream_t)stream);
}

extern "C" int harl_update_values(const float *x0n, long M, int D, int H, const float *W1p, const float *b1p,
                                  const float *W2p, const float *b2p, const float *Whp, const float *bhp, float *values,
                                  void *stream) {
  if (M <= 0) return 0;
  if (D < 1 || D > 64) return bad("harl_update_values: input width must be <= 64");
  UpdFwdArgs U{x0n, W1p, b1p, W2p, b2p, D, n_slabs_of(M), nullptr, 0, nullptr, nullptr, nullptr};
  CriticArgs A{};
  A.M = M; A.Whp = Whp; A.bhp = bhp; A.values_out = values; A.n_slabs = U.n_slabs;
  return dispatch_fwd_critic<false>(U, A, H, (hipStream_t)stream);
}

extern "C" int harl_update_bwd(const float *x0n, const float *dz2, long M, int D, int H, const float *W1p,
                               const float *b1p, const float *W2p, float *dw_part1, float *dw_part2, int n_part_rows,
                               void *stream) {
  if (M <= 0) return 0;
  if (D < 1 || D > 64) return bad("harl_update_bwd: input width must be <= 64");
  if (!dw_part1 || !dw_part2 || n_part_rows <= 0) return bad("harl_update_bwd: missing outputs");
// ... 25 lines not shown
```

### harl_amd/dropin.py

```python
from __future__ import annotations

import os
import runpy
import sys
import types
from typing import Optional

_INSTALLED = False


def stub_optional_modules() -> None:
    def missing(name):
        try:
            __import__(name)
            return False
        except ImportError:
            return True

    if missing("absl"):
        absl, flags = types.ModuleType("absl"), types.ModuleType("absl.flags")
        flags.FLAGS = lambda argv: argv
        absl.flags = flags
        sys.modules["absl"], sys.modules["absl.flags"] = absl, flags
    if missing("setproctitle"):
        sp = types.ModuleType("setproctitle")
        sp.setproctitle = lambda s: None
        sys.modules["setproctitle"] = sp
    if missing("tensorboardX"):
        tb = types.ModuleType("tensorboardX")

        class SummaryWriter:
            def __init__(self, *a, **k):
                self.scalars = {}

            def add_scalars(self, main_tag, tag_scalar_dict, global_step=None):
                for k, v in tag_scalar_dict.items():
                    self.scalars.setdefault(f"{main_tag}/{k}", []).append((global_step, float(v)))

            def export_scalars_to_json(self, path):
                import json
                with open(path, "w", encoding="utf-8") as f:
                    json.dump(self.scalars, f)

            def close(self):
                pass

        tb.SummaryWriter = SummaryWriter
        sys.modules["tensorboardX"] = tb


def _runner_class(base_cls, ours):
    import torch

    class Runner(base_cls):
        __doc__ = f"harl_amd drop-in: {base_cls.__module__}.{base_cls.__name__} + device-resident {ours.__name__} methods"

        _init_update_state = ours._init_update_state
        _ensure_update_state = ours._ensure_update_state
        _critic_first_ok = getattr(ours, "_critic_first_ok", None)
        _prepare_inputs = ours._prepare_inputs
        _fp_normalised_advantages = ours._fp_normalised_advantages
        _check_comms = ours._check_comms
        warmup = ours.warmup
        insert = ours.insert
        compute = ours.compute
        train = ours.train
        after_update = ours.after_update

        def __init__(self, *a, **k):
            super().__init__(*a, **k)
            if not self.algo_args["render"]["use_render"]:
                from .dist import Comm
                self.comm = Comm()
                self._critic_comm = self.comm.second_group()
                self._init_update_state()

        @torch.no_grad()
        def collect(self, step):
            values, actions, logp, rnn, rnn_c = ours.collect(self, step)
            return values, actions.cpu().numpy(), logp, rnn, rnn_c

    Runner.__name__ = ours.__name__
    Runner.__qualname__ = ours.__name__
    return Runner


def install(reference_root: Optional[str] = None, stubs: bool = True) -> dict:
    global _INSTALLED
    if reference_root and reference_root not in sys.path:
        sys.path.insert(0, reference_root)
    if stubs:
        stub_optional_modules()
    import harl.algorithms.actors as ref_actors
    import harl.runners as ref_runners
    import harl.runners.on_policy_base_runner as base

    from . import buffers, runner, valuenorm
    from .happo import HAA2C, HAPPO
    from .hatrpo import HATRPO
    from .mappo import MAPPO
    from .v_critic import VCritic

    ours_algos = {"happo": HAPPO, "hatrpo": HATRPO, "haa2c": HAA2C, "mappo": MAPPO}
    ref_actors.ALGO_REGISTRY.update(ours_algos)
    base.ALGO_REGISTRY = ref_actors.ALGO_REGISTRY
    base.VCritic = VCritic
    base.ValueNorm = valuenorm.ValueNorm
    base.OnPolicyActorBuffer = buffers.OnPolicyActorBuffer
    base.OnPolicyCriticBufferEP = buffers.OnPolicyCriticBufferEP
    base.OnPolicyCriticBufferFP = buffers.OnPolicyCriticBufferFP
    ha = _runner_class(base.OnPolicyBaseRunner, runner.OnPolicyHARunner)
    ma = _runner_class(base.OnPolicyBaseRunner, runner.OnPolicyMARunner)
    installed = {"happo": ha, "hatrpo": ha, "haa2c": ha, "mappo": ma}
    ref_runners.RUNNER_REGISTRY.update(installed)
    _INSTALLED = True
    return installed


def main(argv=None) -> None:
    argv = list(sys.argv[1:] if argv is None else argv)
    ref = os.environ.get("HARL_REFERENCE")
    if "--reference" in argv:
        i = argv.index("--reference")
        ref = argv[i + 1]
        del argv[i:i + 2]
    if "--" in argv:
        argv.remove("--")
    if not ref or not os.path.exists(os.path.join(ref, "examples", "train.py")):
        raise SystemExit("harl_amd.dropin: --reference /path/to/HARL (or HARL_REFERENCE) must contain examples/train.py")
    install(ref)
    sys.argv = [os.path.join(ref, "examples", "train.py")] + argv
    runpy.run_path(sys.argv[0], run_name="__main__")


if __name__ == "__main__":
    main()
```

### harl_amd/happo.py

```python
from __future__ import annotations

import os
from typing import Optional

import numpy as np
import torch

from . import _lib, graphs
from ._lib import PS_STRIDE, call, ptr, stream
from .buffers import OnPolicyActorBuffer, consume_randperm, minibatch_indices, rng_sync
from .dist import Comm, local_minibatch_rows
from .nets import FusedAdam, StochasticPolicy, build_seq, seq_compact
from .valuenorm import _as_dev


class OnPolicyBase:

    def __init__(self, args, obs_space, act_space, device=torch.device("cuda:0")):
        self.args = args
        self.device = torch.device(device)
        _lib.require_gpu(self.device)
        self.tpdv = dict(dtype=torch.float32, device=self.device)
        self.data_chunk_length = args["data_chunk_length"]
        self.use_recurrent_policy = args["use_recurrent_policy"]
        self.use_naive_recurrent_policy = args["use_naive_recurrent_policy"]
        self.use_policy_active_masks = args["use_policy_active_masks"]
        self.action_aggregation = args["action_aggregation"]
        self.lr = args["lr"]
        self.opti_eps = args["opti_eps"]
        self.weight_decay = args["weight_decay"]
        self.obs_space = obs_space
        self.act_space = act_space
        self.actor = StochasticPolicy(args, obs_space, act_space, self.device)
        self.actor_optimizer = FusedAdam(self.actor, self.lr, self.opti_eps, self.weight_decay)
        self.comm = Comm()
        self.shard = None
        self._old_logp: Optional[torch.Tensor] = None
        self._graph = graphs.GraphedStep("the actor")
        self._graph_bufs: dict = {}
        self._graph_gen = None

    def graph_stats(self) -> dict:
        return self._graph.stats()

    def _graph_config_ok(self) -> bool:
        return (graphs.enabled() and not (self.use_recurrent_policy or self.use_naive_recurrent_policy)
                and not self.actor.recurrent and not self.actor.grouped and not self.comm.enabled and self.shard is None)

    def _graph_stage(self, name: str, t: Optional[torch.Tensor]) -> Optional[torch.Tensor]:
        if t is None:
            return None
        b = self._graph_bufs.get(name)
        if b is None or b.shape != t.shape or b.dtype != t.dtype or b.device != t.device:
            b = self._graph_bufs[name] = torch.empty_like(t, memory_format=torch.contiguous_format)
        b.copy_(t)
        return b

    def lr_decay(self, episode, episodes):
        lr = self.lr - (self.lr * ((episode - 1) / float(episodes)))
        for g in self.actor_optimizer.param_groups:
            g["lr"] = lr

    def _logp_pass(self, obs, actions, avail, M, logp_out, old_logp=None, factor=None, head_out=None,
                   rnn_states=None, masks=None, h_last=False, reuse_trunk=False):
        net = self.actor
        agg = int(self.action_aggregation == "mean")
        if net.grouped and not net.recurrent:
            if not reuse_trunk:
                net.forward_trunk(obs, None, M, for_backward=False)
            net.md_logits(M)
            if net.cat_wide:
                call("harl_cat_head_logp", *net.cat_layout(), M, None, ptr(actions), ptr(avail), ptr(logp_out), None,
                     ptr(old_logp), ptr(factor), ptr(head_out), 0, 0, stream(), tag="cat_head_logp")
                return None
            call("harl_md_head_logp", *net.md_layout(), M, ptr(actions), ptr(logp_out), ptr(old_logp),
                 0 if old_logp is None else old_logp.shape[1], ptr(factor), agg, ptr(head_out), 0, 0, stream(),
                 tag="md_head_logp")
            return None
        if not reuse_trunk and net.fused_update_ok(None, train=False):
            call("harl_update_logp", *net.fused_args(obs, M), ptr(net.log_std()), net.std_x_coef, net.std_y_coef,
                 int(net.discrete), net.act_dim, ptr(actions), ptr(avail), ptr(logp_out), ptr(old_logp), ptr(factor), agg,
                 ptr(head_out), stream(), tag="update_logp")
            return None
        if not net.recurrent:
            if not reuse_trunk:
                net.forward_trunk(obs, None, M, for_backward=False)
            Wp, bp = net._packs[-1]
            call("harl_actor_head_logp", ptr(net.xh[-1]), M, net.hidden_sizes[-1], ptr(Wp), ptr(bp), ptr(net.log_std()),
                 net.std_x_coef, net.std_y_coef, int(net.discrete), net.act_dim, ptr(actions), ptr(avail), ptr(logp_out),
                 ptr(old_logp), ptr(factor), agg, ptr(head_out), 0, 0, stream(), tag="actor_head_logp")
            return None
        H = net.hidden_sizes[-1]
        m = rnn_states.shape[0]
        L = M // m
        HS = H * net.recurrent_n
        seq = build_seq(self.device, L, m, HS, h0=_as_dev(rnn_states, self.device).reshape(m, HS),
                        masks_src=_as_dev(masks, self.device), want_h_last=h_last)
        idx, Mp = seq["idx"], L * seq["m_pad"]
        padded = idx is not None
        g = (lambda t: None if t is None else t[idx].contiguous()) if padded else (lambda t: t)
        tmp = (lambda t: None if t is None else torch.empty(Mp, *t.shape[1:], **self.tpdv)) if padded else (lambda t: t)
        a_p, av_p, old_p, f_p = g(actions), g(avail), g(old_logp), g(factor)
        lo_p, ho_p = tmp(logp_out), tmp(head_out)
        net.forward_trunk(obs, idx, Mp, for_backward=False, seq=seq)
        fx, _, _, fh = net.feat()
        Wp, bp = net._packs[-1]
        if net.cat_wide:
            net.md_logits(Mp)
            call("harl_cat_head_logp", *net.cat_layout(), Mp, None, ptr(a_p), ptr(av_p), ptr(lo_p), None, ptr(old_p), ptr(f_p),
                 ptr(ho_p), m, seq["m_pad"], stream(), tag="cat_head_logp")
        elif net.md:
            net.md_logits(Mp)
            call("harl_md_head_logp", *net.md_layout(), Mp, ptr(a_p), ptr(lo_p), ptr(old_p),
                 0 if old_p is None else old_p.shape[1], ptr(f_p), agg, ptr(ho_p), m, seq["m_pad"], stream(),
                 tag="md_head_logp")
        else:
            call("harl_actor_head_logp", ptr(fx), Mp, fh, ptr(Wp), ptr(bp), ptr(net.log_std()), net.std_x_coef,
                 net.std_y_coef, int(net.discrete), net.act_dim, ptr(a_p), ptr(av_p), ptr(lo_p), ptr(old_p), ptr(f_p), agg,
                 ptr(ho_p), m, seq["m_pad"], stream(), tag="actor_head_logp")
        if padded:
            for dst, src in ((logp_out, lo_p), (head_out, ho_p), (factor, f_p)):
                if dst is not None:
                    dst.copy_(seq_compact(src, seq))
        return None if not h_last else seq["h_last"][:m]

    def _dist_rows(self, head, M, *, noise=None, actions=None, logp=None, probs=None, argmax_out=None, ent_rows=None,
                   sigma_out=None):
        net = self.actor
        if net.md and getattr(self, "_head_off", None) is None:
            off = [0]
            for n in net.nvec:
                off.append(off[-1] + int(n))
            self._head_off = torch.tensor(off, dtype=torch.int32, device=self.device)
        call("harl_dist_rows", ptr(head), M, net.act_dim, int(net.discrete), None if net.discrete else ptr(net.log_std()),
             net.std_x_coef, net.std_y_coef, ptr(noise), ptr(actions), ptr(self._head_off) if net.md else None,
             len(net.nvec) if net.md else 1, 1, ptr(logp), ptr(probs), ptr(argmax_out), ptr(ent_rows), ptr(sigma_out), stream(),
             tag="dist_rows")

    def evaluate_actions(self, obs, rnn_states_actor, action, masks, available_actions=None, active_masks=None):
        obs = _as_dev(obs, self.device)
        obs = obs.reshape(obs.shape[0], -1)
        action = _as_dev(action, self.device).reshape(obs.shape[0], -1)
        avail = None if available_actions is None else _as_dev(available_actions, self.device).reshape(obs.shape[0], -1)
        M = obs.shape[0]
        net = self.actor
        out = torch.empty(M, net.act_w, **self.tpdv)
        head = torch.empty(M, net.act_dim, **self.tpdv)
        net.fold()
        self._logp_pass(obs, action, avail, M, out, head_out=head, rnn_states=rnn_states_actor, masks=masks)
        ent_rows = torch.empty(M, **self.tpdv)
        sigma = None if net.discrete else torch.empty(net.act_dim, **self.tpdv)
        self._dist_rows(head, M, ent_rows=ent_rows, sigma_out=sigma)
        am = None
        if not net.md and active_masks is not None and self.use_policy_active_masks:
            am = _as_dev(active_masks, self.device).reshape(M).contiguous()
        mom = torch.zeros(3, dtype=torch.float64, device=self.device)
        entropy = torch.empty((), **self.tpdv)
        call("harl_masked_moments", ptr(ent_rows), ptr(am), M, ptr(mom), _lib.scratch("mm"), stream())
        call("harl_moments_mean", ptr(mom), ptr(entropy), stream())
        if net.md:
            return out, entropy, None
        dist = (torch.distributions.Categorical(logits=head) if net.discrete
                else torch.distributions.Normal(head, sigma.expand_as(head)))
        return out, entropy, dist

# ... 354 lines not shown
```

### harl_amd/nets.py

```python
from __future__ import annotations

import math
import os
from typing import Dict, List, Optional, Sequence, Tuple

import torch
import torch.nn as nn

from . import _lib
from . import graphs as _graphs
from ._lib import DHEAD_LD, PS_STRIDE, SLAB, call, ptr, stream
from .configs import CAT_WIDE_REFUSALS

SUPPORTED_WIDTHS = (64, 128, 256)
ACT_IDS = {"relu": 0, "leaky_relu": 1, "tanh": 2, "sigmoid": 3, "selu": 4}


_FUSED_UPDATE_MODES = ("hybrid", "logp", "1", "actor", "0")


def _fused_update_mode() -> str:
    mode = os.environ.get("HARL_FUSED_UPDATE", "hybrid")
    if mode not in _FUSED_UPDATE_MODES:
        raise ValueError(f"HARL_FUSED_UPDATE={mode!r}: expected one of {_FUSED_UPDATE_MODES}")
# ... 207 lines not shown

    @property
    def grouped(self) -> bool:
        return bool(self._md_sp)

    def _build_tables(self) -> None:
        ents = self._entries()
        dev = self.device_
        L = len(self.hidden_sizes)
        rows, pack_off, dwp_off = [], 0, 0
        pack_slots = []
        self._dwp_offs, self._elems = [], []
        if self.recurrent:
            H = self.hidden_sizes[-1]
        for ei, (wo, bo, go, beo, o, k) in enumerate(ents):
            gru_i = ei - L if (self.recurrent and L <= ei < L + 6 * self.recurrent_n) else -1
            if gru_i >= 0:
                layer, within = divmod(gru_i, 6)
                mat, gate = divmod(within, 3)
                base = self._gru_pack_base + (2 * layer + mat) * (3 * H * H + 3 * H)
                pw, pb = base + gate * H * H, base + 3 * H * H + gate * H
            else:
                if self.recurrent and ei == L:
                    pass
                orows = self._md_sp[ei - (len(ents) - len(self._md_sp))] if (self.grouped and ei >= len(ents) - len(self._md_sp)) else o
                pw, pb = pack_off, pack_off + orows * k
                pack_off += orows * k + orows
                if self.recurrent and ei == L - 1:
                    self._gru_pack_base = pack_off
                    pack_off += 2 * self.recurrent_n * (3 * H * H + 3 * H)
            kp, op = ((k + 31) // 32) * 32, ((o + 31) // 32) * 32
            if self.grouped and ei >= len(ents) - len(self._md_sp):
                op = self._md_sp[ei - (len(ents) - len(self._md_sp))]
            elems = op * kp + op
            rows.append([wo, bo, go, beo, o, k, pw, pb, dwp_off, kp, op, 0])
            pack_slots.append((pw, pb, o, k))
            self._dwp_offs.append(dwp_off)
            self._elems.append(elems)
            dwp_off += elems
        self._table_rows = rows
        self.n_entries = len(rows)
        self._ws_gen = getattr(self, "_ws_gen", 0) + 1
        self.pack_arena = torch.zeros(pack_off, dtype=torch.float32, device=dev)
        self.dwp_msg = torch.zeros(dwp_off + 4 * PS_STRIDE, dtype=torch.float32, device=dev)
        self.dwp = self.dwp_msg[:dwp_off]
        self.total_dwp = dwp_off
        self._pack_slots = pack_slots
        views = [(self.pack_arena[pw:pw + o * k], self.pack_arena[pb:pb + o]) for (pw, pb, o, k) in pack_slots]
        self._packs = views[:L] + [views[-1]]
        nh = len(self._head_layers())
        self._head_packs = views[-nh:]
        if self.recurrent:
            n = 3 * H * H
            self.gru_packs = []
            for l in range(self.recurrent_n):
                b0 = self._gru_pack_base + 2 * l * (n + 3 * H)
                self.gru_packs.append(dict(Wih=self.pack_arena[b0:b0 + n], bih=self.pack_arena[b0 + n:b0 + n + 3 * H],
                                           Whh=self.pack_arena[b0 + n + 3 * H:b0 + 2 * n + 3 * H],
                                           bhh=self.pack_arena[b0 + 2 * n + 3 * H:b0 + 2 * n + 6 * H]))
            self.gru_pack = self.gru_packs[0]
        covered = sum(o * k + o for (_, _, _, _, o, k) in ents)
        covered += sum(k for go, k in {(go, k) for (_, _, go, _, _, k) in ents if go >= 0}) * 2
        if isinstance(self, StochasticPolicy) and not self.discrete:
            covered += self.act_dim
        assert covered == self.n_params, f"layer table covers {covered} of {self.n_params} parameters"
        self.table = None

    def fold(self) -> None:
        if not self._packs:
            self._build_tables()
        ver = self.flat_param._version
        if getattr(self, "_fold_version", None) == ver and os.environ.get("HARL_ALWAYS_FOLD", "0") != "1":
            return
        s = stream()
        fp, pa = self.flat_param, self.pack_arena
        if self.table is not None and os.environ.get("HARL_FOLD_TABLE", "1") != "0":
            call("harl_fold_table", ptr(fp), ptr(pa), ptr(self.table), self.n_entries, sum(r[4] for r in self._table_rows), s)
            self._fold_version = ver
            return
        for (wo, bo, go, beo, o, k), (pw, pb, _, _) in zip(self._entries(), self._pack_slots):
            call("harl_fold_linear", ptr(fp[wo:]), ptr(fp[bo:]), ptr(fp[go:]) if go >= 0 else None,
                 ptr(fp[beo:]) if beo >= 0 else None, ptr(pa[pw:]), ptr(pa[pb:]), o, k, s)
        self._fold_version = ver

    def _ensure_ws(self, M: int) -> None:
        if M <= self._max_rows:
            return
        dev = self.device_
        self._ws_gen = getattr(self, "_ws_gen", 0) + 1
        n_slabs = (M + SLAB - 1) // SLAB
        mp = n_slabs * SLAB
        f32, u32 = torch.float32, torch.int32
        self.xh = [torch.empty(mp * h, dtype=f32, device=dev) for h in self.hidden_sizes]
        self.rmask = [torch.empty(n_slabs * max(h // 64, 1) * 64, dtype=u32, device=dev) for h in self.hidden_sizes]
        self.rstd = [torch.empty(mp, dtype=f32, device=dev) for _ in self.hidden_sizes]
        self.mu0 = torch.empty(mp, dtype=f32, device=dev)
        self.rstd0 = torch.empty(mp, dtype=f32, device=dev)
        self.kp0 = ((self.in_dim + 31) // 32) * 32
        self.wide = 32 < self.in_dim <= 512
        self._x0n_key = None
        self.x0n = torch.empty(mp * self.kp0, dtype=f32, device=dev) if (self.in_dim <= 64 or self.wide) else None
        self.w1img = (torch.empty(3 * self.hidden_sizes[0] * self.kp0 // 2, dtype=f32, device=dev)
                      if (self.wide or self.act_id) else None)
        hmax = max(self.hidden_sizes)
        if self.act_id:
            self.zraw = torch.empty(mp * hmax, dtype=f32, device=dev)
            self.amean = [torch.empty(mp, dtype=f32, device=dev) for _ in self.hidden_sizes]
            self.ones_mask = torch.full((n_slabs * 64 * 2,), -1, dtype=u32, device=dev)
        self.dz = [torch.empty(mp * hmax, dtype=f32, device=dev) for _ in range(3 if len(self.hidden_sizes) == 3 and self.trunk_fused() else 2)]
        self._trunk_cache = {}
        self.wide_head = (not self.grouped) and self._layers()[-1][4] > 32
        self.dhead = torch.zeros(mp * (64 if self.wide_head else DHEAD_LD), dtype=f32, device=dev)
        self.md_z = [torch.zeros(mp * sp, dtype=f32, device=dev) for sp in self._md_sp]
        n_iter = (n_slabs + 1) // 2
        nwg_env = os.environ.get("HARL_NWG")
        nwg_cap = int(nwg_env) if nwg_env else max(256, min(512, n_slabs // 10))
        if (not nwg_env and _bwd_fused_mode(M) == "1" and len(self.hidden_sizes) >= 2 and all(h == 128 for h in self.hidden_sizes)
                and ((self.in_dim + 31) // 32) * 32 == 32 and not (self.recurrent or self.grouped or self.act_id or self.panel)):
            nwg_cap = 256
        self.n_wg = max(1, min(nwg_cap, n_iter))
        part_off, rows = 0, [list(r) for r in self._table_rows]
        self._part_offs = []
        for r, elems in zip(rows, self._elems):
            r[11] = part_off
            self._part_offs.append(part_off)
            part_off += self.n_wg * elems
        self.part = torch.empty(part_off, dtype=f32, device=dev)
        self.table = torch.tensor(rows, dtype=torch.int32, device=dev).reshape(-1).contiguous()
        if self.recurrent:
            H = self.hidden_sizes[-1]
            a = lambda: torch.empty(mp * H, dtype=f32, device=dev)
            self.rnn_y, self.rnn_rstd = a(), torch.empty(mp, dtype=f32, device=dev)
            self.rnn_saved_l = [[a() for _ in range(5)] for _ in range(self.recurrent_n)]
            self.rnn_dgate_l = [[a() for _ in range(4)] for _ in range(self.recurrent_n)]
            self.rnn_saved, self.rnn_dgate = self.rnn_saved_l[0], self.rnn_dgate_l[0]
            self.rnn_ones = torch.full((n_slabs * 64 * ((H // 2 + 31) // 32),), -1, dtype=u32, device=dev)
            self.rnn_gi = torch.empty(3 * mp * H, dtype=f32, device=dev)
            if self.gru_wide:
                from . import gru_wide
                gru_wide.ensure_ws(self, mp)
        self.n_head_blocks = max(_lib.load().harl_head_blocks(M), self.n_wg)
        self.part_scalars = torch.zeros(self.n_head_blocks * PS_STRIDE, dtype=f32, device=dev)
        self.scalars = torch.zeros(PS_STRIDE, dtype=torch.float64, device=dev)
        self._max_rows = M

    def feat(self):
        if self.recurrent:
            return self.rnn_y, self.rnn_ones, self.rnn_rstd, self.hidden_sizes[-1]
        if self.act_id:
            return self.xh[-1], self.ones_mask, self.rstd[-1], self.hidden_sizes[-1]
        return self.xh[-1], self.rmask[-1], self.rstd[-1], self.hidden_sizes[-1]

    def forward_rnn(self, seq: dict, save: bool, gates_done: bool = False) -> None:
        if self.gru_wide:
            from . import gru_wide
            return gru_wide.forward(self, seq, save)
        gp = self.gru_pack
        sv = self.rnn_saved
        call("harl_gru_fwd", ptr(self.xh[-1]), ptr(seq["mask_rows"]), ptr(seq["h0"]), ptr(gp["Wih"]), ptr(gp["bih"]),
             ptr(gp["Whh"]), ptr(gp["bhh"]), self.hidden_sizes[-1], seq["L"], seq["m_pad"], ptr(self.rnn_y),
             ptr(self.rnn_rstd), ptr(sv[0]), ptr(sv[1]), ptr(sv[2]), ptr(sv[3]), ptr(sv[4]), ptr(seq.get("h_last")),
             int(save) | (2 if gates_done else 0), ptr(self.rnn_gi), stream(), tag="gru_fwd")

    def trunk_fused(self) -> bool:
        hs = self.hidden_sizes
        return (os.environ.get("HARL_TRUNK_FUSED", "1") != "0" and self.wide and not self.act_id and not self.panel
# ... 769 lines not shown
```

### harl_amd/runner.py

```python
from __future__ import annotations

import os
from typing import List, Optional

import torch

from . import _lib
from .buffers import OnPolicyActorBuffer, OnPolicyCriticBufferEP, OnPolicyCriticBufferFP, rng_sync
from ._lib import call, ptr, stream
from .dist import Comm, shard_columns
from .happo import HAA2C, HAPPO
from .hatrpo import HATRPO
from .mappo import MAPPO
from .v_critic import VCritic
from .valuenorm import ValueNorm

ALGO_REGISTRY = {"happo": HAPPO, "hatrpo": HATRPO, "haa2c": HAA2C, "mappo": MAPPO}


class OnPolicyHARunner:
    CRITIC_STREAM_MAX_ROWS = 150_000

    def __init__(self, args: dict, algo_args: dict, env_args: Optional[dict] = None, *, obs_spaces=None,
                 share_obs_space=None, act_spaces=None, device: Optional[torch.device] = None,
# ... 20 lines not shown
        self.share_param = bool(algo_args["algo"].get("share_param", False))
        if self.share_param and algo != "mappo":
            raise NotImplementedError("share_param is a MAPPO feature (HAPPO/HATRPO/HAA2C need per-agent actors)")
        self.fixed_order = algo_args["algo"].get("fixed_order", True)
        self.action_aggregation = algo_args["algo"]["action_aggregation"]
        if self.share_param and self.comm.world_size > 1 and (algo_args["model"].get("use_recurrent_policy")
                                                             or algo_args["model"].get("use_naive_recurrent_policy")):
            raise NotImplementedError("share_param with recurrent policies under data parallelism is not implemented")

        n_global = algo_args["train"]["n_rollout_threads"]
        lo, hi = shard_columns(n_global, self.comm.rank, self.comm.world_size)
        self.n_global, self.col_lo, self.col_hi = n_global, lo, hi
        train_local = dict(algo_args["train"])
        train_local["n_rollout_threads"] = hi - lo
        margs = {**algo_args["model"], **algo_args["algo"]}
        self.actor: List[HAPPO] = []
        for a in range(self.num_agents):
            if self.share_param and a > 0:
                self.actor.append(self.actor[0])
            else:
                self.actor.append(ALGO_REGISTRY[algo](margs, obs_spaces[a], act_spaces[a], device=self.device))
        self.actor_buffer = [OnPolicyActorBuffer({**train_local, **algo_args["model"]}, obs_spaces[a], act_spaces[a],
                                                 device=self.device) for a in range(self.num_agents)]
        self.critic = VCritic(margs, share_obs_space, device=self.device)
        cb_args = {**train_local, **algo_args["model"], **algo_args["algo"]}
        if self.state_type == "EP":
            self.critic_buffer = OnPolicyCriticBufferEP(cb_args, share_obs_space, device=self.device)
        else:
            self.critic_buffer = OnPolicyCriticBufferFP(cb_args, share_obs_space, self.num_agents, device=self.device)
        self.value_normalizer = ValueNorm(1, device=self.device) if algo_args["train"]["use_valuenorm"] else None
        self._critic_comm = self.comm.second_group()
        self._init_update_state(n_global)
        if algo_args["train"].get("model_dir") is not None:
            self.restore(algo_args["train"]["model_dir"])

    def _init_update_state(self, n_global: Optional[int] = None, comm: Optional[Comm] = None) -> None:
        if not hasattr(self, "comm") or self.comm is None:
            self.comm = comm if comm is not None else Comm()
        if n_global is None:
            n_global = self.algo_args["train"]["n_rollout_threads"]
        if not hasattr(self, "col_lo"):
            self.n_global = n_global
            self.col_lo, self.col_hi = shard_columns(n_global, self.comm.rank, self.comm.world_size)
        shard = (self.n_global, self.col_lo, self.col_hi) if self.comm.enabled else None
        for x in list(self.actor) + [self.critic]:
            x.comm, x.shard = self.comm, shard
        self.critic.comm = getattr(self, "_critic_comm", None) or self.comm
        self._logp_old = None
        self._counts_host = None
        self._update_state_ready = True

    def _ensure_update_state(self) -> None:
        if not getattr(self, "_update_state_ready", False):
            self._init_update_state()

    def _check_comms(self) -> None:
        self.comm.check()
        if self.critic.comm is not self.comm:
            self.critic.comm.check()

    @torch.no_grad()
    def compute(self):
        self._ensure_update_state()
        cb = self.critic_buffer
        if self.state_type == "EP":
            next_value, _ = self.critic.get_values(cb.share_obs[-1], cb.rnn_states_critic[-1], cb.masks[-1])
        else:
            so = cb.share_obs[-1]
            rows = so.shape[0] * so.shape[1]
            next_value, _ = self.critic.get_values(so.reshape(rows, -1), cb.rnn_states_critic[-1].reshape(rows, 1, -1),
                                                   cb.masks[-1].reshape(rows, 1))
        cb.compute_returns(next_value, self.value_normalizer)

    @torch.no_grad()
    def train(self):
        self._ensure_update_state()
        T = self.algo_args["train"]["episode_length"]
        N = self.col_hi - self.col_lo
        B = T * N
        dev = self.device
        actor_train_infos = []
        for x in self.actor:
            x.actor.invalidate_caches()
        self._prepare_inputs()
        factor = torch.ones(T, N, 1, dtype=torch.float32, device=dev)
        advantages = self.critic_buffer.advantages
        if self.state_type == "FP":
            advantages = self._fp_normalised_advantages(advantages)
        if self.fixed_order:
            agent_order = list(range(self.num_agents))
        else:
            rng_sync()
            agent_order = [int(a) for a in torch.randperm(self.num_agents).numpy()]
        fast = [hasattr(a, "masked_moments") for a in self.actor]
        mom_all = torch.zeros(self.num_agents, 3, dtype=torch.float64, device=dev)
        for a in range(self.num_agents):
            if fast[a]:
                adv_a = advantages if self.state_type == "EP" else advantages[:, :, a].contiguous()
                self.actor[a].masked_moments(self.actor_buffer[a], adv_a, mom_all[a])
        self.comm.all_reduce_sum(mom_all)
        if self._counts_host is None or self._counts_host.numel() != self.num_agents:
            self._counts_host = torch.empty(self.num_agents, dtype=torch.float64, pin_memory=torch.cuda.is_available())
        self._counts_host.copy_(mom_all[:, 2], non_blocking=True)
        ev = torch.cuda.Event()
        ev.record()
        cinfo, critic_done = None, None
        if self._critic_first_ok(fast):
            cs_mode = os.environ.get("HARL_CRITIC_STREAM", "auto")
            if (dev.type == "cuda" and (not self.comm.enabled or self.critic.comm is not self.comm)
                    and cs_mode != "0" and (cs_mode == "1" or B <= self.CRITIC_STREAM_MAX_ROWS)):
                if getattr(self, "_critic_stream", None) is None:
                    self._critic_stream = torch.cuda.Stream(device=dev)
                main_s = torch.cuda.current_stream(dev)
                self._critic_stream.wait_stream(main_s)
                with torch.cuda.stream(self._critic_stream):
                    cinfo = self.critic.train(self.critic_buffer, self.value_normalizer, _defer=True)
                    critic_done = torch.cuda.Event()
                    critic_done.record(self._critic_stream)
            else:
                cinfo = self.critic.train(self.critic_buffer, self.value_normalizer, _defer=True)
        ev.synchronize()
        counts = self._counts_host.tolist()
        rng_after = None
        if (cinfo is None and dev.type == "cuda" and all(hasattr(a, "rng_footprint") for a in self.actor)
                and (not self.comm.enabled or self.critic.comm is not self.comm)
                and os.environ.get("HARL_CRITIC_STREAM", "1") != "0" and os.environ.get("HARL_CRITIC_EARLY", "1") != "0"):
            from .buffers import consume_randperm
            rng_sync()
            rng_start = torch.get_rng_state()
            for a in agent_order:
                if counts[a] > 0.0:
                    for n in self.actor[a].rng_footprint(self.actor_buffer[a]):
                        consume_randperm(n)
            rng_sync()
            if getattr(self, "_critic_stream", None) is None:
                self._critic_stream = torch.cuda.Stream(device=dev)
            self._critic_stream.wait_stream(torch.cuda.current_stream(dev))
            staggered = dict(gen=self.critic._train_epochs(self.critic_buffer, self.value_normalizer), state=torch.get_rng_state(),
                             left=self.critic.critic_epoch)
            torch.set_rng_state(rng_start)

            def critic_epoch(after_event=None, _st=staggered):
                if _st["left"] <= 0:
                    return
                rng_sync()
                actor_state = torch.get_rng_state()
                torch.set_rng_state(_st["state"])
                if after_event is not None:
                    self._critic_stream.wait_event(after_event)
                with torch.cuda.stream(self._critic_stream):
                    next(_st["gen"])
                _st["left"] -= 1
                rng_sync()
                _st["state"] = torch.get_rng_state()
                torch.set_rng_state(actor_state)
            rng_after = staggered
        old_all, old_ev = {}, {}
        side_agents = [a for a in agent_order
                       if not (fast[a] and self.actor[a].fuses_old_logp() and counts[a] > 0.0) and os.environ.get("HARL_SIDE_STREAM", "1") != "0"]
        def enqueue_old_logp(a):
            act_a, buf_a = self.actor[a], self.actor_buffer[a]
            with torch.cuda.stream(self._side_stream):
                act_a.actor.fold()
                kw_a = dict(rnn_states=buf_a.rnn_states[0], masks=buf_a.flat("masks")) if act_a.actor.recurrent else {}
                act_a._logp_pass(buf_a.flat("obs"), buf_a.flat("actions"),
                                 None if buf_a.available_actions is None else buf_a.flat("available_actions"), B, old_all[a], **kw_a)
                old_ev[a] = torch.cuda.Event()
                old_ev[a].record(self._side_stream)

        side_lazy = os.environ.get("HARL_SIDE_AHEAD", "1") != "0"
        side_pending = []
        if side_agents:
            if getattr(self, "_side_stream", None) is None:
                self._side_stream = torch.cuda.Stream(device=dev)
            main = torch.cuda.current_stream(dev)
            self._side_stream.wait_stream(main)
            for a in side_agents:
                act_a, buf_a = self.actor[a], self.actor_buffer[a]
                old_all[a] = torch.empty(B, act_a.actor.act_w, dtype=torch.float32, device=dev)
            side_pending = list(side_agents)
            for a in (side_pending[:1] if side_lazy else list(side_pending)):
                enqueue_old_logp(a)
                side_pending.remove(a)
        pending = []
        post_ok = dev.type == "cuda" and os.environ.get("HARL_POST_STREAM", "1") != "0"
        factor_ev, keep_alive, prev_overlapped = None, [], False
        last_post = os.environ.get("HARL_LAST_POST_PASS", "0") == "1" or dev.type != "cuda"
        for pos, agent_id in enumerate(agent_order):
            buf, actor = self.actor_buffer[agent_id], self.actor[agent_id]
            if agent_id in old_ev:
                torch.cuda.current_stream(dev).wait_event(old_ev[agent_id])
            buf.update_factor(factor)
            if prev_overlapped:
                keep_alive.append(self._logp_old)
                self._logp_old = None
            obs, actions = buf.flat("obs"), buf.flat("actions")
            avail = None if buf.available_actions is None else buf.flat("available_actions")
            if self._logp_old is None or self._logp_old.shape != (B, actor.actor.act_w):
                self._logp_old = torch.empty(B, actor.actor.act_w, dtype=torch.float32, device=dev)
            actor.actor.fold()
            rnn_kw = dict(rnn_states=buf.rnn_states[0], masks=buf.flat("masks")) if actor.actor.recurrent else {}
            adv_a = advantages if self.state_type == "EP" else advantages[:, :, agent_id].contiguous()
            kw = dict(_pre=(mom_all[agent_id], counts[agent_id]), _defer=True) if fast[agent_id] else {}
            fused_old = fast[agent_id] and actor.fuses_old_logp() and counts[agent_id] > 0.0
            if fused_old:
                kw["_old_logp_out"] = self._logp_old
            elif agent_id in old_all:
                self._logp_old = old_all.pop(agent_id)
            else:
                actor._logp_pass(obs, actions, avail, B, self._logp_old, **rnn_kw)
            if factor_ev is not None and hasattr(actor, "_factor_ready"):
                actor._factor_ready = factor_ev
            info = actor.train(buf, adv_a, self.state_type, **kw)
            if side_pending:
                enqueue_old_logp(side_pending.pop(0))
            if rng_after is not None and rng_after["left"] > 0:
                ev_a = torch.cuda.Event()
                ev_a.record(torch.cuda.current_stream(dev))
                critic_epoch(ev_a)
            if factor_ev is not None:
                if hasattr(actor, "_factor_ready"):
                    actor._factor_ready = None
                torch.cuda.current_stream(dev).wait_event(factor_ev)
                factor_ev = None
            pending.append((len(actor_train_infos), info, actor._INFO_KEYS) if torch.is_tensor(info) else None)
            actor_train_infos.append(info)
            nxt = agent_order[pos + 1] if pos + 1 < len(agent_order) else None
            prev_overlapped = bool(post_ok and nxt is not None and actor.actor.recurrent and hasattr(self.actor[nxt], "_factor_ready"))
            if nxt is None and not last_post:
                continue
            if prev_overlapped:
                if getattr(self, "_post_stream", None) is None:
                    self._post_stream = torch.cuda.Stream(device=dev)
                ps = self._post_stream
                ps.wait_stream(torch.cuda.current_stream(dev))
                keep_alive += [factor, self._logp_old]
                with torch.cuda.stream(ps):
                    new_factor = factor.clone()
                    actor._logp_pass(obs, actions, avail, B, None, old_logp=self._logp_old, factor=new_factor.reshape(B), **rnn_kw)
                    factor_ev = torch.cuda.Event()
                    factor_ev.record(ps)
                factor = new_factor
                continue
            new_factor = factor.clone()
            actor._logp_pass(obs, actions, avail, B, None, old_logp=self._logp_old, factor=new_factor.reshape(B), **rnn_kw)
            factor = new_factor
        if keep_alive:
            torch.cuda.current_stream(dev).wait_stream(self._post_stream)
            keep_alive.clear()
        if rng_after is not None:
            while rng_after["left"] > 0:
                critic_epoch(None)
            for _ in rng_after["gen"]:
                pass
            with torch.cuda.stream(self._critic_stream):
                cinfo = self.critic._train_result(True)
                critic_done = torch.cuda.Event()
                critic_done.record(self._critic_stream)
        if cinfo is None:
            cinfo = self.critic.train(self.critic_buffer, self.value_normalizer, _defer=True)
        if critic_done is not None:
            torch.cuda.current_stream(dev).wait_event(critic_done)
        rng_sync()
        if rng_after is not None:
            torch.set_rng_state(rng_after["state"])
        dev_infos = [p[1] for p in pending if p is not None] + [cinfo]
        flat = torch.cat([t.reshape(-1) for t in dev_infos]).cpu().tolist()
        self._check_comms()
        off = 0
        for p in pending:
            if p is not None:
                i, _, keys = p
                actor_train_infos[i] = dict(zip(keys, flat[off:off + len(keys)]))
                off += len(keys)
        critic_train_info = {"value_loss": flat[off], "critic_grad_norm": flat[off + 1]}
        return actor_train_infos, critic_train_info

    def _prepare_inputs(self) -> None:
        from . import graphs
        if os.environ.get("HARL_X0N_MULTI", "1") == "0" or self.device.type != "cuda" or graphs.enabled():
            return
        from .nets import prepare_x0n_multi
        items = []
        for a, buf in zip(self.actor, self.actor_buffer):
            if hasattr(a, "fuses_old_logp") and a.fuses_old_logp():
                items.append((a.actor, buf.flat("obs")))
        c = self.critic
        crit = (c.critic_num_mini_batch == 1 and not (c.use_recurrent_policy or c.use_naive_recurrent_policy)
                and hasattr(c, "_inputs_prepared"))
        if crit:
            c.critic.invalidate_caches()
            items.append((c.critic, self.critic_buffer.flat("share_obs")))
        for net, _ in items:
            net.fold()
        built = prepare_x0n_multi([(net, X, X.shape[0]) for net, X in items])
        if crit and built:
            c._inputs_prepared = True

    def graph_stats(self) -> dict:
        from .graphs import sum_stats
        return sum_stats(list(self.actor) + [self.critic])

    def _critic_first_ok(self, fast) -> bool:
        if not all(fast) or os.environ.get("HARL_CRITIC_FIRST", "1") == "0":
            return False
        c = self.critic
        if c.critic_num_mini_batch != 1 or c.use_recurrent_policy or c.use_naive_recurrent_policy:
            return False
        return all(hasattr(a, "fuses_old_logp") and a.fuses_old_logp() for a in self.actor)

    def after_update(self):
        for b in self.actor_buffer:
            b.after_update()
        self.critic_buffer.after_update()

    def _fp_normalised_advantages(self, advantages):
        dev = self.device
        active = torch.stack([b.active_masks[:-1] for b in self.actor_buffer], dim=2).contiguous()
        mom = torch.zeros(3, dtype=torch.float64, device=dev)
        n = advantages.numel()
        call("harl_masked_moments", ptr(advantages), ptr(active), n, ptr(mom), _lib.scratch("mm"), stream())
        self.comm.all_reduce_sum(mom)
        adv_n = torch.empty_like(advantages)
        call("harl_adv_normalize", ptr(advantages), ptr(mom), ptr(adv_n), n, stream())
        return adv_n

    def warmup(self):
        obs, share_obs, available_actions = self.envs.reset()
        obs = torch.as_tensor(obs, dtype=torch.float32).to(self.device)
        for a in range(self.num_agents):
            self.actor_buffer[a].obs[0].copy_(obs[:, a])
            if self.actor_buffer[a].available_actions is not None:
                av = torch.as_tensor(available_actions, dtype=torch.float32).to(self.device)
                self.actor_buffer[a].available_actions[0].copy_(av[:, a])
        so = torch.as_tensor(share_obs, dtype=torch.float32).to(self.device)
        self.critic_buffer.share_obs[0].copy_(so[:, 0] if self.state_type == "EP" else so)

    @torch.no_grad()
    def collect(self, step: int):
        acts, logps, rnns = [], [], []
        for a in range(self.num_agents):
            b = self.actor_buffer[a]
            action, logp, rnn = self.actor[a].get_actions(
                b.obs[step], b.rnn_states[step], b.masks[step],
                b.available_actions[step] if b.available_actions is not None else None)
            acts.append(action)
            logps.append(logp)
            rnns.append(rnn.reshape(rnn.shape[0], b.recurrent_n, -1))
        actions, action_log_probs, rnn_states = torch.stack(acts, 1), torch.stack(logps, 1), torch.stack(rnns, 1)
        cb = self.critic_buffer
        if self.state_type == "EP":
            values, rnn_c = self.critic.get_values(cb.share_obs[step], cb.rnn_states_critic[step], cb.masks[step])
            rnn_c = rnn_c.reshape(values.shape[0], cb.recurrent_n, -1)
        else:
            so = cb.share_obs[step]
            N, A = so.shape[:2]
            values, rnn_c = self.critic.get_values(so.reshape(N * A, -1), cb.rnn_states_critic[step].reshape(N * A, 1, -1),
                                                   cb.masks[step].reshape(N * A, 1))
            values, rnn_c = values.reshape(N, A, 1), rnn_c.reshape(N, A, cb.recurrent_n, -1)
        return values, actions, action_log_probs, rnn_states, rnn_c

    @torch.no_grad()
    def insert(self, data):
        (obs, share_obs, rewards, dones, infos, available_actions, values, actions, action_log_probs, rnn_states,
         rnn_states_critic) = data
        dev, A = self.device, self.num_agents
        up = lambda x: torch.as_tensor(x, dtype=torch.float32).to(dev)
        dones = torch.as_tensor(dones).to(dev).bool()
        N = dones.shape[0]
        dones_env = dones.all(dim=1)
        keep = (~dones_env).to(torch.float32)
        rnn_states = rnn_states * keep.view(N, 1, 1, 1)
        rnn_states_critic = rnn_states_critic * (keep.view(N, 1, 1) if self.state_type == "EP" else keep.view(N, 1, 1, 1))
        masks = keep.view(N, 1, 1).expand(N, A, 1)
        active_masks = torch.where(dones & ~dones_env.view(N, 1), 0.0, 1.0).view(N, A, 1)
        if self.state_type == "EP":
            bad = [[0.0] if info[0].get("bad_transition", False) is True else [1.0] for info in infos]
        else:
            bad = [[[0.0] if info[a].get("bad_transition", False) is True else [1.0] for a in range(A)] for info in infos]
        bad_masks = torch.tensor(bad, dtype=torch.float32, device=dev)
# ... 221 lines not shown
```

### harl_amd/traffic.py

```python
from __future__ import annotations

from typing import Callable, Dict, Optional, Sequence


def _act(H: int) -> float:
    return 4.0 * H + H / 8.0 + 4.0


def _kp(D: int) -> int:
    return 32 * ((int(D) + 31) // 32)


def _fwd_fused2x(a: Sequence) -> float:
    M, D, H, store1 = a[1], a[3], a[7], a[8]
    return M * (4.0 * _kp(D) + (_act(H) if store1 else 0.0) + _act(H))


def _fwd_fused2(a: Sequence) -> float:
    M, D, H, store1, x0n = a[3], a[4], a[10], a[11], a[20]
    return M * (4.0 * D + (8.0 if a[2] else 0.0) + (_act(H) if store1 else 0.0) + _act(H) + 8.0 + (4.0 * _kp(D) if x0n else 0.0))


def _fwd_hidden(a: Sequence) -> float:
    return a[1] * (4.0 * a[2] + _act(a[3]))
# ... 36 lines not shown


def _gru_fwd(a: Sequence) -> float:
    H, L, m_pad, save = a[7], a[8], a[9], a[18]
    xin = 3 * 4.0 * H if (save & 2) else 4.0 * H
    return L * m_pad * (xin + 4.0 + 4.0 * H + 4.0 + (5 * 4.0 * H if (save & 1) else 0.0))


def _gru_bwd(a: Sequence) -> float:
    H, L, m_pad = a[9], a[10], a[11]
    if not a[19]:
        return L * m_pad * (6 * 4.0 * H + 4.0 + 4 * 4.0 * H)
    return L * m_pad * (6 * 4.0 * H + 4.0 + _act(H) + 4 * 4.0 * H + 4.0 * H)


def _cat_head_logp(a: Sequence) -> float:
    G, n, M = a[1], a[3], a[4]
    row = 4.0 * sum(a[2][g] for g in range(G)) + (4.0 * n if a[7] else 0.0) + (8.0 if a[5] else 0.0)
    row += sum(4.0 for k in (6, 8, 9, 10) if a[k]) + (8.0 if a[11] else 0.0) + (4.0 * n if a[12] else 0.0)
    return M * row


def _cat_head_loss(a: Sequence) -> float:
    G, n, M = a[1], a[3], a[4]
    row = 2 * 4.0 * sum(a[2][g] for g in range(G)) + (4.0 * n if a[7] else 0.0) + (8.0 if a[5] else 0.0)
    row += 3 * 4.0 + sum(4.0 for k in (11, 12, 18) if a[k])
    return M * row


def _nonnull(arr) -> int:
    return sum(1 for p in arr if p)


def _fwd_trunk(a: Sequence) -> float:
    M, KP, H = a[1], a[2], a[6]
    return M * (4.0 * KP + _nonnull(a[11]) * _act(H) + (3 * 4.0 * H if a[17] else 0.0))


def _bwd_trunk(a: Sequence) -> float:
    M, H, nh = a[0], a[1], a[2]
    top = (3 * 4.0 * H + _act(H) + 4.0 * H) if a[3] else 4.0 * H
    return M * (top + nh * (_act(H) + 4.0 * H))


def _dw_partials_multi_v(a: Sequence) -> float:
    n, HO, M = a[0], a[4], a[8]
    return M * sum(4.0 * HO + 4.0 * 32 * a[7][k] for k in range(n))


def _head_rows(discrete: int, act_dim: int, avail) -> float:
    w = 1 if discrete else act_dim
    return 4.0 * w + 4.0 * w + (4.0 * act_dim if avail else 0.0)


def _actor_head_loss(a: Sequence) -> float:
    M, H, disc, ad = a[3], a[4], a[10], a[11]
    w = 1 if disc else ad
    return M * (_act(H) + _head_rows(disc, ad, a[14]) + 4.0 + (4.0 if a[18] else 0.0) + (4.0 if a[19] else 0.0)
                + (4.0 * w if a[26] else 0.0) + 4.0 * H + (4.0 * 32 if (a[28] and not a[30]) else 0.0))


def _actor_head_logp(a: Sequence) -> float:
    M, H, disc, ad = a[1], a[2], a[8], a[9]
    w = 1 if disc else ad
    return M * (4.0 * H + 4.0 * w + (4.0 * ad if a[11] else 0.0) + (4.0 * w if a[12] else 0.0) + (4.0 * w if a[13] else 0.0)
                + (8.0 if a[14] else 0.0) + (4.0 * ad if a[16] else 0.0))


def _critic_head_loss(a: Sequence) -> float:
    return a[3] * (_act(a[4]) + 8.0 + 4.0 * a[4])


def _update_fwd_actor(a: Sequence) -> float:
    M, D, H, disc, ad = a[1], a[2], a[3], a[13], a[14]
    w = 1 if disc else ad
    return M * (4.0 * _kp(D) + _head_rows(disc, ad, a[16]) + 4.0 + (4.0 if a[20] else 0.0) + (4.0 if a[21] else 0.0)
                + (4.0 * w if a[26] else 0.0) + 4.0 * H + (_act(H) if a[31] else 0.0))


def _update_logp(a: Sequence) -> float:
    M, D, disc, ad = a[1], a[2], a[13], a[14]
    w = 1 if disc else ad
    return M * (4.0 * _kp(D) + 4.0 * w + (4.0 * ad if a[16] else 0.0) + (4.0 * w if a[17] else 0.0) + (4.0 * w if a[18] else 0.0)
                + (8.0 if a[19] else 0.0) + (4.0 * ad if a[21] else 0.0))


def _update_fwd_critic(a: Sequence) -> float:
    return a[1] * (4.0 * _kp(a[2]) + 8.0 + 4.0 * a[3] + (_act(a[3]) if a[21] else 0.0))


def _update_last_actor(a: Sequence) -> float:
    M, H, disc, ad = a[1], a[2], a[10], a[11]
    w = 1 if disc else ad
    return M * (4.0 * H + _head_rows(disc, ad, a[14]) + 4.0 + (4.0 if a[18] else 0.0) + (4.0 if a[19] else 0.0)
                + (4.0 * w if a[24] else 0.0) + 4.0 * H)


def _update_last_critic(a: Sequence) -> float:
    return a[1] * (4.0 * a[2] + 8.0 + 4.0 * a[2])


def _update_values(a: Sequence) -> float:
    return a[1] * (4.0 * _kp(a[2]) + 4.0)


def _update_bwd(a: Sequence) -> float:
    return a[2] * (4.0 * _kp(a[3]) + 4.0 * a[4])


def _panel_fwd(a: Sequence) -> float:
    return a[1] * (4.0 * a[2] + _act(a[6]))


def _panel_bwd(a: Sequence) -> float:
    return a[4] * (4.0 * a[5] + _act(a[6]) + 4.0 * a[6])


def _tangent_hidden(a: Sequence) -> float:
    return a[2] * (2 * 4.0 * a[3] + _act(a[4]) + 4.0 * a[4])


def _gae(a: Sequence) -> float:
    T, n = a[8], a[9]
    return 4.0 * n * (T + 3 * (T + 1) + (T + 1) + T)


ALGORITHMIC_BYTES: Dict[str, Callable[[Sequence], float]] = {
    "harl_mlp_fwd_fused2x": _fwd_fused2x,
    "harl_mlp_fwd_fused2": _fwd_fused2,
    "harl_mlp_fwd_hidden": _fwd_hidden,
    "harl_mlp_fwd_wide": _fwd_wide,
    "harl_mlp_fwd_input": _fwd_input,
    "harl_mlp_x0n_wide": _x0n_wide,
    "harl_mlp_tangent_wide": _tangent_wide,
    "harl_mlp_bwd_dx": _bwd_dx,
    "harl_mlp_bwd_dx_dw": _bwd_dx_dw,
    "harl_mlp_dw_partials": _dw_partials,
    "harl_mlp_dw_partials_multi": _dw_partials_multi,
    "harl_mlp_dw_partials_multi_v": _dw_partials_multi_v,
    "harl_gru_dw6": lambda a: a[7] * 6 * 4.0 * 64,
    "harl_mlp_fwd_trunk": _fwd_trunk,
    "harl_mlp_bwd_trunk": _bwd_trunk,
    "harl_gru_fwd": _gru_fwd,
    "harl_gru_bwd": _gru_bwd,
    "harl_actor_head_loss": _actor_head_loss,
    "harl_actor_head_logp": _actor_head_logp,
    "harl_critic_head_loss": _critic_head_loss,
    "harl_update_fwd_actor": _update_fwd_actor,
    "harl_update_logp": _update_logp,
    "harl_update_fwd_critic": _update_fwd_critic,
    "harl_update_values": _update_values,
    "harl_update_last_actor": _update_last_actor,
    "harl_update_last_critic": _update_last_critic,
    "harl_update_bwd": _update_bwd,
    "harl_gae_returns": _gae,
    "harl_mlp_panel_fwd": _panel_fwd,
    "harl_mlp_panel_bwd": _panel_bwd,
    "harl_cat_head_logp": _cat_head_logp,
    "harl_cat_head_loss": _cat_head_loss,
    "harl_mlp_tangent_hidden": _tangent_hidden,
    "harl_mlp_tangent_hidden2": _tangent_hidden,
}


def algorithmic_bytes(name: str, args: Sequence) -> Optional[float]:
    f = ALGORITHMIC_BYTES.get(name)
    return None if f is None else float(f(args))


def _f_fused2x(a):
    return 2.0 * a[1] * (a[3] * a[7] + a[7] * a[7])


def _f_fused2(a):
    return 2.0 * a[3] * (a[4] * a[10] + a[10] * a[10])


def _f_update_fwd_actor(a):
    M, D, H, ad = a[1], a[2], a[3], a[14]
    return 2.0 * M * (D * H + H * H + 3 * ad * H)


def _f_update_logp(a):
    M, D, H, ad = a[1], a[2], a[3], a[14]
    return 2.0 * M * (D * H + H * H + ad * H)


def _f_update_fwd_critic(a):
    M, D, H = a[1], a[2], a[3]
    return 2.0 * M * (D * H + H * H + 3 * H)


def _f_update_values(a):
    M, D, H = a[1], a[2], a[3]
    return 2.0 * M * (D * H + H * H + H)


def _f_update_last_actor(a):
    return 2.0 * a[1] * (a[2] * a[2] + 3 * a[11] * a[2])


def _f_update_last_critic(a):
    return 2.0 * a[1] * (a[2] * a[2] + 3 * a[2])


def _f_update_bwd(a):
    M, D, H = a[2], a[3], a[4]
    return 2.0 * M * (2 * D * H + 2 * H * H + D * H)


def _f_bwd_dx(a):
    M, HO, HI = a[4], a[5], a[6]
    return 2.0 * M * (HO * HI + (HI * a[10] if a[9] else 0))


def _f_bwd_dx_dw(a):
    M, HO, HI = a[4], a[5], a[6]
    return 2.0 * M * (2 * HO * HI + (HI * a[10] if a[9] else 0))


def _f_dw(a):
    return 2.0 * a[11] * a[3] * a[10]


def _f_dw_multi(a):
    return 2.0 * a[0] * a[6] * a[4] * a[5]


def _f_gru_fwd(a):
    H, L, m_pad = a[7], a[8], a[9]
    return 2.0 * L * m_pad * (3 if (a[18] & 2) else 6) * H * H

# ... 67 lines not shown
```

### harl_amd/v_critic.py

```python
from __future__ import annotations

import os
from typing import Optional

import torch

from . import _lib, graphs
from ._lib import PS_STRIDE, call, ptr, stream
from .buffers import OnPolicyCriticBufferEP, consume_randperm, minibatch_indices, rng_sync
from .dist import Comm, local_minibatch_rows
from .nets import FusedAdam, VNet, build_seq
from .valuenorm import ValueNorm, _as_dev


class VCritic:
    def __init__(self, args, cent_obs_space, device=torch.device("cuda:0")):
        self.args = args
        self.device = torch.device(device)
        _lib.require_gpu(self.device)
        self.tpdv = dict(dtype=torch.float32, device=self.device)
        self.clip_param = args["clip_param"]
        self.critic_epoch = args["critic_epoch"]
        self.critic_num_mini_batch = args["critic_num_mini_batch"]
        self.data_chunk_length = args["data_chunk_length"]
        self.value_loss_coef = args["value_loss_coef"]
        self.max_grad_norm = args["max_grad_norm"]
        self.huber_delta = args["huber_delta"]
        self.use_recurrent_policy = args["use_recurrent_policy"]
        self.use_naive_recurrent_policy = args["use_naive_recurrent_policy"]
        self.use_max_grad_norm = args["use_max_grad_norm"]
        self.use_clipped_value_loss = args["use_clipped_value_loss"]
        self.use_huber_loss = args["use_huber_loss"]
        self.use_policy_active_masks = args["use_policy_active_masks"]
        self.critic_lr = args["critic_lr"]
        self.opti_eps = args["opti_eps"]
        self.weight_decay = args["weight_decay"]
        self.share_obs_space = cent_obs_space
        self.critic = VNet(args, cent_obs_space, self.device)
        self.critic_optimizer = FusedAdam(self.critic, self.critic_lr, self.opti_eps, self.weight_decay)
        self.comm = Comm()
        self.shard = None
        self._inputs_prepared = False
        self._info = torch.zeros(2, dtype=torch.float64, device=self.device)
        self._grad_tap = None
        self._trace = None
        self._state_tap = None
        self._graph = graphs.GraphedStep("the critic")
        self._graph_idx: Optional[torch.Tensor] = None
        self._graph_gen = None

    def graph_stats(self) -> dict:
        return self._graph.stats()

    def _graph_config_ok(self) -> bool:
        return (graphs.enabled() and not (self.use_recurrent_policy or self.use_naive_recurrent_policy)
                and not self.critic.recurrent and not self.comm.enabled and self.shard is None)

    def lr_decay(self, episode, episodes):
        lr = self.critic_lr - (self.critic_lr * ((episode - 1) / float(episodes)))
        for g in self.critic_optimizer.param_groups:
            g["lr"] = lr

    def get_values(self, cent_obs, rnn_states_critic, masks):
        x = _as_dev(cent_obs, self.device)
        x = x.reshape(x.shape[0], -1)
        M = x.shape[0]
        net = self.critic
        net.fold()
        Wp, bp = net._packs[-1]
        out = torch.empty(M, 1, **self.tpdv)
        if net.fused_update_ok(None, train=False):
            call("harl_update_values", *net.fused_args(x, M), ptr(out), stream(), tag="update_values")
            return out, (None if rnn_states_critic is None else _as_dev(rnn_states_critic, self.device))
        if not net.recurrent:
            net.forward_trunk(x, None, M, for_backward=False)
            call("harl_critic_head_values", ptr(net.xh[-1]), M, net.hidden_sizes[-1], ptr(Wp), ptr(bp), ptr(out), stream())
            return out, (None if rnn_states_critic is None else _as_dev(rnn_states_critic, self.device))
        H = net.hidden_sizes[-1]
        h0 = _as_dev(rnn_states_critic, self.device)
        m = h0.shape[0]
        HS = H * net.recurrent_n
        seq = build_seq(self.device, M // m, m, HS, h0=h0.reshape(m, HS), masks_src=_as_dev(masks, self.device),
                        want_h_last=True)
        Mp = seq["L"] * seq["m_pad"]
        net.forward_trunk(x, seq["idx"], Mp, for_backward=False, seq=seq)
        fx, _, _, fh = net.feat()
        outp = out if seq["idx"] is None else torch.empty(Mp, 1, **self.tpdv)
        call("harl_critic_head_values", ptr(fx), Mp, fh, ptr(Wp), ptr(bp), ptr(outp), stream())
        if seq["idx"] is not None:
            out.copy_(outp.reshape(seq["L"], seq["m_pad"], 1)[:, :m].reshape(M, 1))
        return out, seq["h_last"][:m].reshape(m, net.recurrent_n, H).clone()

    def _update_core(self, share_obs, idx, m, m_global, value_preds, returns, vn: Optional[ValueNorm], seq=None, _graph=False):
        if not _graph:
            return self._step(share_obs, idx, m, m_global, value_preds, returns, vn, seq)
        G, net, opt = self._graph, self.critic, self.critic_optimizer
        step = lambda: self._step(share_obs, idx, m, m_global, value_preds, returns, vn, seq)
        if (seq is not None or m <= 0 or self._trace is not None or self._grad_tap is not None or self._state_tap is not None
                or not graphs.launches_capturable(self.device) or opt.hyper_rows_left() < 1):
            return G.eager(step)
        net.prepare_x0n(share_obs, idx, m)
        if self._graph_gen != net._ws_gen:
            G.drop()
            self._graph_gen = net._ws_gen
        p = lambda t: 0 if t is None else t.data_ptr()
        g = opt.param_groups[0]
        e = os.environ.get
        warm = (m, m_global, idx is None, vn is None, float(self.clip_param), bool(self.use_clipped_value_loss),
                bool(self.use_huber_loss), float(self.huber_delta), float(self.value_loss_coef), bool(self.use_max_grad_norm),
                float(self.max_grad_norm), tuple(g["betas"]), float(g["eps"]), float(g["weight_decay"]),
                None if vn is None else vn.beta, e("HARL_FUSED_UPDATE"), e("HARL_BWD_FUSED"), e("HARL_BWD_K64"),
                e("HARL_TRUNK_FUSED"))
        key = warm + (p(share_obs), p(idx), p(value_preds), p(returns), None if vn is None else (p(vn.stats), p(vn._sums)),
                      p(self._info), p(net.flat_param), p(net.pack_arena), p(opt.exp_avg), p(opt._hyper_dev), opt._hyper_rows)
        G.run(warm, key, step, opt)

    def _step(self, share_obs, idx, m, m_global, value_preds, returns, vn: Optional[ValueNorm], seq=None):
        net = self.critic
        s = stream()
        if vn is not None:
            vidx = seq["valid_idx"] if seq is not None else idx
            vn.update(returns, vidx, count=m_global, reduce_fn=self.comm.all_reduce_sum if self.comm.enabled else None,
                      local_count=(seq["L"] * seq["m"] if seq is not None else m))
        net._ensure_ws(max(m, 1))
        sc = net.scalars
        self._forward_backward(net, share_obs, idx, m, value_preds, returns, vn, seq, s)
        nblk = net.n_wg if m > 0 else 0
        ps_kw = dict(part_scalars=net.part_scalars, n_scalar_blocks=nblk)
        if self.comm.enabled:
            if m <= 0:
                net.dwp.zero_()
            hilo = net.dwp_msg[net.total_dwp:]
            call("harl_reduce_pack_scalars", ptr(net.part_scalars), nblk, ptr(sc), ptr(hilo), s)
            self.comm.all_reduce_message(net.dwp_msg)
            ps_kw = dict(scalars_hilo=hilo)
        scale = float(self.value_loss_coef) / float(m_global)
        if self._state_tap is not None:
            o = self.critic_optimizer
            self._state_tap.append((net.flat_param.clone(), o.exp_avg.clone(), o.exp_avg_sq.clone(), o.step_count))
        self.critic_optimizer.step(1, scale, self.use_max_grad_norm, self.max_grad_norm, self._info, **ps_kw)
        if self._trace is not None:
            self._trace.append(self._info.clone())
        if self._grad_tap is not None:
            self._grad_tap(net.flat_grad * scale, sc.clone())

    def _forward_backward(self, net, share_obs, idx, m, value_preds, returns, vn, seq, s) -> None:
        if m > 0 and net.fused_update_ok(idx, seq):
            call("harl_update_fwd_critic", *net.fused_args(share_obs, m), ptr(value_preds), ptr(returns),
                 ptr(vn.stats) if vn is not None else None, float(self.clip_param), int(self.use_clipped_value_loss),
                 int(self.use_huber_loss), float(self.huber_delta), ptr(net.dz[0]), ptr(net.part_scalars),
                 ptr(net.part[net._part_offs[-1]:]), net.n_wg, *net.hybrid_outputs(), s, tag="update_fwd_critic")
            net.backward_after_fused(share_obs, m)
        elif m > 0 and net.fused_last_ok(idx, seq):
            L = len(net.hidden_sizes)
            net.forward_trunk(share_obs, idx, m, upto=L - 1)
            (Wl, bl), (Wh, bh) = net._packs[L - 1], net._packs[-1]
            call("harl_update_last_critic", ptr(net.xh[L - 2]), m, net.hidden_sizes[-1], ptr(Wl), ptr(bl), ptr(Wh), ptr(bh),
                 ptr(idx), ptr(value_preds), ptr(returns), ptr(vn.stats) if vn is not None else None, float(self.clip_param),
                 int(self.use_clipped_value_loss), int(self.use_huber_loss), float(self.huber_delta), ptr(net.dz[0]),
                 ptr(net.part_scalars), ptr(net.part[net._part_offs[-1]:]), net.n_wg, s, tag="update_last_critic")
            net.backward_trunk(share_obs, idx, m, head_dw_done=True)
        elif m > 0:
            net.forward_trunk(share_obs, idx, m, seq=seq)
            Wp, bp = net._packs[-1]
            fx, fmask, frstd, fh = net.feat()
            mv, mp = (seq["m"], seq["m_pad"]) if seq is not None else (0, 0)
            call("harl_critic_head_loss", ptr(fx), ptr(fmask), ptr(frstd), m, fh,
                 ptr(Wp), ptr(bp), ptr(idx), ptr(value_preds), ptr(returns), ptr(vn.stats) if vn is not None else None,
                 float(self.clip_param), int(self.use_clipped_value_loss), int(self.use_huber_loss), float(self.huber_delta),
                 mv, mp, ptr(net.dz[0]), ptr(net.dhead), ptr(net.part_scalars), ptr(net.part[net._part_offs[-1]:]),
                 net.n_wg, s, tag="critic_head_loss")
            net.backward_trunk(share_obs, idx, m, seq=seq, head_dw_done=True)

    def update(self, sample, value_normalizer=None):
        share_obs, _rnn, value_preds, returns, _masks = sample
        dev = self.device
        x = _as_dev(share_obs, dev)
        m = x.shape[0]
        before = self._info.clone()
        self.critic.fold()
        if self.critic.recurrent:
            HS = self.critic.hidden_sizes[-1] * self.critic.recurrent_n
            h0 = _as_dev(_rnn, dev)
            seq = build_seq(dev, m // h0.shape[0], h0.shape[0], HS, h0=h0.reshape(-1, HS), masks_src=_as_dev(_masks, dev))
            self._update_core(x.reshape(m, -1), seq["idx"], seq["L"] * seq["m_pad"], m, _as_dev(value_preds, dev).reshape(m),
                              _as_dev(returns, dev).reshape(m), value_normalizer, seq=seq)
            d = self._info - before
            return d[0], d[1]
        self._update_core(x.reshape(m, -1), None, m, m, _as_dev(value_preds, dev).reshape(m),
                          _as_dev(returns, dev).reshape(m), value_normalizer)
        d = self._info - before
        return d[0], d[1]

    def train(self, critic_buffer: OnPolicyCriticBufferEP, value_normalizer: Optional[ValueNorm] = None, _defer=False):
        for _ in self._train_epochs(critic_buffer, value_normalizer):
            pass
        return self._train_result(_defer)

    def _train_result(self, _defer: bool):
        n_upd = self.critic_epoch * self.critic_num_mini_batch
        if _defer:
            return self._info / n_upd
        rng_sync()
        vals = (self._info / n_upd).cpu().tolist()
        return {"value_loss": vals[0], "critic_grad_norm": vals[1]}

    def _train_epochs(self, critic_buffer: OnPolicyCriticBufferEP, value_normalizer: Optional[ValueNorm] = None):
        buf = critic_buffer
        T, N = buf.rewards.shape[:2]
        A = getattr(buf, "num_agents", None)
        B = T * N * (A or 1)
        dev = self.device
        self._info.zero_()
        if self._inputs_prepared:
            self._inputs_prepared = False
        else:
            self.critic.invalidate_caches()
        buf.__dict__.pop("_seq_cache", None)
        self.critic.fold()
        share_obs = buf.flat("share_obs")
        value_preds = buf.flat("value_preds").reshape(B)
        returns = buf.flat("returns").reshape(B)
        n_global = self.shard[0] * T * (A or 1) if self.shard else B
        graph = False
        if self._graph_config_ok():
            self.critic_optimizer.begin_steps(self.critic_epoch * self.critic_num_mini_batch)
            graph = graphs.launches_capturable(dev)
        try:
            yield from self._epochs(buf, share_obs, value_preds, returns, value_normalizer, A, B, n_global, graph)
        finally:
            self.critic_optimizer.end_steps()

    def _epochs(self, buf, share_obs, value_preds, returns, value_normalizer, A, B, n_global, graph: bool):
        dev = self.device
        for _ in range(self.critic_epoch):
            if self.use_recurrent_policy or self.use_naive_recurrent_policy:
                for seq in buf.recurrent_batches(self.critic_num_mini_batch, self.data_chunk_length,
                                                 naive=not self.use_recurrent_policy, shard=self.shard):
                    if seq.get("empty"):
                        self._update_core(share_obs, None, 0, seq["L"] * seq["m_global"], value_preds, returns,
                                          value_normalizer)
                        continue
                    self._update_core(share_obs, seq["idx"], seq["L"] * seq["m_pad"], seq["L"] * seq["m_global"],
                                      value_preds, returns, value_normalizer, seq=seq)
                yield
                continue
            if self.critic_num_mini_batch == 1:
                consume_randperm(n_global)
                self._update_core(share_obs, None, B, n_global, value_preds, returns, value_normalizer, _graph=graph)
                yield
                continue
            sampler = minibatch_indices(n_global, self.critic_num_mini_batch, dev)
            for ind in sampler:
                m_global = ind.numel()
                if self.shard:
                    ind = local_minibatch_rows(ind, self.shard[0], self.shard[1], self.shard[2], agents=A or 1)
                if graph:
                    if self._graph_idx is None or self._graph_idx.shape != ind.shape or self._graph_idx.device != dev:
                        self._graph_idx = torch.empty(ind.shape, dtype=ind.dtype, device=dev)
                    self._graph_idx.copy_(ind)
                self._update_core(share_obs, self._graph_idx if graph else ind.to(dev), ind.numel(), m_global, value_preds, returns,
                                  value_normalizer, _graph=graph)
            yield

    def prep_training(self):
        self.critic.train()
        self.critic.invalidate_caches()

    def prep_rollout(self):
        self.critic.eval()
        self.critic.invalidate_caches()
```

### harl_amd/valuenorm.py

```python
from __future__ import annotations

from typing import Optional

import numpy as np
import torch

from . import _lib
from ._lib import call, ptr, stream


class ValueNorm:
    def __init__(self, input_shape=1, norm_axes=1, beta=0.99999, per_element_update=False, epsilon=1e-5,
                 device=torch.device("cuda:0")):
        if input_shape != 1 or norm_axes != 1 or per_element_update:
            raise NotImplementedError("only the scalar-value configuration used by the on-policy runners")
        _lib.require_gpu(torch.device(device))
        self.device = torch.device(device)
        self.beta = float(beta)
        self.epsilon = float(epsilon)
        self.stats = torch.zeros(3, dtype=torch.float32, device=self.device)
        self._sums = torch.zeros(2, dtype=torch.float64, device=self.device)

    @property
    def running_mean(self):
        return self.stats[0:1]

    @property
    def running_mean_sq(self):
        return self.stats[1:2]

    @property
    def debiasing_term(self):
        return self.stats[2]

    def running_mean_var(self):
        d = self.stats[2].clamp(min=self.epsilon)
        mean = self.stats[0:1] / d
        var = (self.stats[1:2] / d - mean ** 2).clamp(min=1e-2)
        return mean, var

    @torch.no_grad()
    def update(self, input_vector, idx: Optional[torch.Tensor] = None, count: Optional[int] = None, reduce_fn=None,
               local_count: Optional[int] = None):
        x = _as_dev(input_vector, self.device).reshape(-1)
        m = x.numel() if idx is None else idx.numel()
        if local_count is not None and idx is None:
            m = local_count
        self._sums.zero_()
        if m > 0:
            call("harl_sum_sumsq", ptr(x), ptr(idx), m, ptr(self._sums), stream())
        if reduce_fn is not None:
            reduce_fn(self._sums)
        call("harl_valuenorm_apply", ptr(self.stats), ptr(self._sums), float(count if count is not None else m),
             self.beta, stream())

    def normalize(self, input_vector):
        x = _as_dev(input_vector, self.device)
        mean, var = self.running_mean_var()
        return (x - mean[None]) / torch.sqrt(var)[None]

    def denormalize(self, input_vector):
        x = _as_dev(input_vector, self.device)
        mean, var = self.running_mean_var()
        return (x * torch.sqrt(var)[None] + mean[None]).cpu().numpy()

    def state_dict(self):
        return {"running_mean": self.stats[0:1].clone(), "running_mean_sq": self.stats[1:2].clone(),
                "debiasing_term": self.stats[2].clone()}

    def load_state_dict(self, sd):
        if not sd:
            return
        self.stats[0] = torch.as_tensor(sd["running_mean"]).reshape(-1)[0]
        self.stats[1] = torch.as_tensor(sd["running_mean_sq"]).reshape(-1)[0]
        self.stats[2] = torch.as_tensor(sd["debiasing_term"]).reshape(-1)[0]

    def to(self, *a, **k):
        return self


def _as_dev(x, device) -> torch.Tensor:
    if isinstance(x, np.ndarray):
        x = torch.from_numpy(x)
    elif x.dtype == torch.float32 and x.device == device and x.is_contiguous():
        return x
    return x.to(device=device, dtype=torch.float32).contiguous()
```

### include/harl_hip.h

```cpp
#ifndef HARL_HIP_H
#define HARL_HIP_H

#include <stdint.h>

#ifdef __cplusplus
extern "C" {
#endif

#define HARL_PS_STRIDE 48
#define HARL_DHEAD_LD 32
#define HARL_MD_MAX_HEADS 8
#define HARL_MD_MAX_GROUPS 4
#define HARL_MM_SCRATCH_BYTES 24640
#define HARL_CG_SCRATCH_BYTES 1088

int harl_version(void);
const char *harl_last_error(void);

int harl_gae_returns(const float *rewards, float *value_preds, const float *masks, const float *bad_masks,
                     const float *next_value, const float *vn_stats, float *returns, float *advantages,
                     int T, int ncols, float gamma, float gamma_lambda, int use_gae,
                     int use_proper_time_limits, int fp_order, void *stream);

int harl_masked_moments(const float *x, const float *active, long n, double *out3, void *scratch, void *stream);

int harl_dist_rows(const float *head, long M, int act_dim, int kind, const float *log_std, float std_x_coef, float std_y_coef,
                   const float *noise, float *actions, const int *head_off, int n_heads, int sum_heads, float *logp,
                   float *probs, float *argmax_out, float *ent_rows, float *sigma_out, void *stream);
int harl_moments_mean(const double *moments3, float *mean_out, void *stream);
int harl_build_seq(const int64_t *first, int m, int m_pad, int L, long stride, const float *masks_src, const float *h0_src,
                   int H, int64_t *idx, int64_t *valid_idx, float *mask_rows, float *h0, void *stream);
int harl_clock_probe(long long *cycles_ticks, long ticks, void *stream);
int harl_adv_normalize(const float *adv, const double *moments3, float *adv_out, long n, void *stream);

int harl_factor_update(float *factor, const float *new_logp, const float *old_logp, long n, int act_dim,
                       int agg_mean, void *stream);

int harl_sum_sumsq(const float *x, const int64_t *idx, long m, double *sums2, void *stream);
int harl_valuenorm_apply(float *vn_stats, const double *sums2, double count, double beta, void *stream);

int harl_gradnorm_clip_adam(float *param, float *grad, float *exp_avg, float *exp_avg_sq, long n,
                            const float *grad_scale, int use_clip, float max_norm, double lr, double beta1,
                            double beta2, float eps, float weight_decay, double bias_correction1,
                            double bias_correction2, double *info_out, void *stream);

int harl_fold_linear(const float *W, const float *b, const float *gamma, const float *beta, float *Wp,
                     float *bp, int out_dim, int in_dim, void *stream);
int harl_unfold_linear_grads(const float *dWp, const float *dbp, int ldp, const float *W, const float *gamma,
                             const float *beta, float *dW, float *db, float *dgamma, float *dbeta,
                             int out_dim, int in_dim, int accumulate, void *stream);

int harl_mlp_fwd_input(const float *X, long ldx, const int64_t *idx, long M, int D, const float *Wp,
                       const float *bp, int use_ln0, int H, float *xout, uint32_t *relu_mask, float *rstd,
                       float *mu0, float *rstd0, float *x0n, void *stream);
int harl_mlp_x0n_wide(const float *X, long ldx, const int64_t *idx, long M, int D, int use_ln0, float *x0n, float *mu0,
                      float *rstd0, void *stream);
#define HARL_X0N_MULTI_MAX 32
typedef struct {
  const float *X;
  long ldx, M;
  int D, use_ln0;
  float *x0n, *mu0, *rstd0;
} harl_x0n_problem;
int harl_x0n_multi(const harl_x0n_problem *table, int n, int max_workgroups, void *stream);
int harl_mlp_fwd_wide(const float *x0n, long M, int KP, const float *Wp, int D, const float *bp, int H, void *w_img,
                      float *xout, uint32_t *relu_mask, float *rstd, void *stream);
int harl_mlp_panel_fwd(const float *xin, long M, int KP, const float *Wp, int D, const float *bp, int HO, float *xout,
                       uint32_t *relu_mask, float *rstd, void *stream);
int harl_head_dw_rows256(const float *dhead, long M, int act_dim, const float *xhat, float *part, int n_wg, void *stream);
int harl_mlp_panel_tangent(const float *xin_dot, const float *xin, long M, int KP, const float *Wp, const float *Wdp, int D,
                           const float *bdp, const float *xprimal, const uint32_t *mask_in, const float *rstd_in,
                           float *xout_dot, void *stream);
int harl_mlp_panel_bwd(const float *dz, const float *xprev, const uint32_t *relu_mask_prev, const float *rstd_prev, long M,
                       int HO, int HI, const float *Wp, float *dz_prev, void *stream);
int harl_mlp_fwd_fused2x(const float *x0n, long M, const float *W1p, int D, const float *b1p, const float *W2p,
                         const float *b2p, int H, int store1, float *x1out, uint32_t *mask1, float *rstd1, float *x2out,
                         uint32_t *mask2, float *rstd2, void *stream);
int harl_mlp_fwd_fused2(const float *X, long ldx, const int64_t *idx, long M, int D, const float *W1p,
                        const float *b1p, int use_ln0, const float *W2p, const float *b2p, int H, int store1,
                        float *x1out, uint32_t *mask1, float *rstd1, float *mu0, float *rstd0, float *x2out,
                        uint32_t *mask2, float *rstd2, float *x0n, void *stream);
int harl_mlp_fwd_hidden(const float *xin, long M, int HI, int HO, const float *Wp, const float *bp,
                        float *xout, uint32_t *relu_mask, float *rstd, void *stream);
int harl_mlp_bwd_dx(const float *dz, const float *xprev, const uint32_t *relu_mask_prev, const float *rstd_prev,
                    long M, int HO, int HI, const float *Wp, float *dz_prev, const float *x0n, int kp0, float *dw_part,
                    int n_wg, void *stream);
int harl_mlp_bwd_dx_dw(const float *dz, const float *xprev, const uint32_t *relu_mask_prev, const float *rstd_prev,
                       long M, int HO, int HI, const float *Wp, float *dz_prev, const float *x0n, int kp0, float *dw1_part,
                       float *dw2_part, int n_wg, int fill, void *stream);
int harl_mlp_dw_partials(const float *a, int a_kind, int lda, int HO, const float *b, int b_kind, long ldx,
                         const int64_t *idx, const float *mu0, const float *rstd0, int K, long M, float *part,
                         int n_wg, void *stream);
int harl_mlp_dw_partials_multi(int n, const float *const *a, const float *const *b, float *const *part, int HO, int K,
                               long M, int n_wg, void *stream);
int harl_mlp_dw_partials_multi_v(int n, const float *const *a, const float *const *b, float *const *part, int HO, const int *K,
                                 const int *tile0, const int *nt, long M, int n_wg, void *stream);
int harl_gru_dw6(const float *dr, const float *dz, const float *dn, const float *dhn, const float *xhat, const float *hpm,
                 float *const *part, long M, int n_wg, void *stream);
int harl_mlp_fwd_trunk(const float *x0n, long M, int KP, const float *W1p, int D, const float *b1p, int H, void *w_img,
                       int n_hidden, const float *const *Wp, const float *const *bp, float *const *xout,
                       uint32_t *const *relu_mask, float *const *rstd, const float *Wih, const float *bih, const float *bhh,
                       float *gi_ws, void *stream);
int harl_mlp_bwd_trunk(long M, int H, int n_hidden, const float *Wih, const float *dr, const float *dzg, const float *dn,
                       const float *dz_in, const float *const *Wp, const float *const *xh, const uint32_t *const *relu_mask,
                       const float *const *rstd, float *const *dz_out, void *stream);
int harl_reduce_partials(const float *part, int n_wg, long elems, float *out, void *stream);

#define HARL_TABLE_STRIDE 12
int harl_reduce_partials_multi(const float *part, const int *table, int n_layers, int n_wg, long total_elems,
                               float *dwp, void *stream);
int harl_fold_table(const float *param, float *packs, const int *table, int n_layers, int total_rows, void *stream);
int harl_unfold_table(const float *param, float *grad, const float *dwp, const int *table, int n_layers, int total_cols,
                      void *stream);
int harl_fold_tangent_table(const float *param, const float *vec, float *pack_d, const int *table, int n_layers,
                            int total_rows, void *stream);
int harl_pack_scalars_hilo(const double *scalars, float *hilo, void *stream);
int harl_reduce_pack_scalars(const float *part_scalars, int n_blocks, double *scalars, float *hilo, void *stream);
int harl_adam_fold(float *param, float *grad, float *exp_avg, float *exp_avg_sq, long n, const float *dwp,
                   const int *table, int n_layers, float *packs, double *scalars, const float *part_scalars,
                   int n_scalar_blocks, const float *scalars_hilo, int mode, float const_scale, int logstd_off,
                   int act_dim, double *info,
                   int use_clip, float max_norm, double lr, double beta1, double beta2, float eps, float weight_decay,
                   double bias_correction1, double bias_correction2, void *ws, void *stream);
int harl_adam_fold_dev(float *param, float *grad, float *exp_avg, float *exp_avg_sq, long n, const float *dwp,
                       const int *table, int n_layers, float *packs, double *scalars, const float *part_scalars,
                       int n_scalar_blocks, const float *scalars_hilo, int mode, float const_scale, int logstd_off,
                       int act_dim, double *info, int use_clip, float max_norm, const double *hyper, int n_hyper_rows,
                       int *step_idx, double beta1, double beta2, float eps, float weight_decay, void *ws, void *stream);

int harl_actor_head_logp(const float *xL, long M, int H, const float *Whp, const float *bhp,
                         const float *log_std, float std_x_coef, float std_y_coef, int discrete, int act_dim,
                         const float *actions, const float *avail, float *logp_out, const float *old_logp,
                         float *factor, int agg_mean, float *head_out, long m_valid, long m_pad, void *stream);
int harl_actor_head_loss(const float *xL, const uint32_t *relu_mask, const float *rstd, long M, int H,
                         const float *Whp, const float *bhp, const float *log_std, float std_x_coef,
                         float std_y_coef, int discrete, int act_dim, const int64_t *idx, const float *actions,
                         const float *avail, const float *old_logp, const float *adv, const double *adv_moments,
                         const float *factor, const float *active, double clip_param, float entropy_coef,
                         int agg_mean, int trpo, long m_valid, long m_pad, float *logp_out, float *dzL, float *dhead,
                         float *part_scalars, float *dw_part, int n_wg, void *stream);
int harl_critic_head_values(const float *xL, long M, int H, const float *Whp, const float *bhp, float *values,
                            void *stream);
int harl_critic_head_loss(const float *xL, const uint32_t *relu_mask, const float *rstd, long M, int H,
                          const float *Whp, const float *bhp, const int64_t *idx, const float *value_preds,
                          const float *returns, const float *vn_stats, float clip_param, int use_clipped,
                          int use_huber, float huber_delta, long m_valid, long m_pad, float *dzL, float *dhead,
                          float *part_scalars, float *dw_part, int n_wg, void *stream);
int harl_fold_linear_tangent(const float *W, const float *gamma, const float *beta, const float *Wd, const float *bd,
                             const float *gammad, const float *betad, float *Wpd, float *bpd, int out_dim, int in_dim,
                             void *stream);
int harl_mlp_tangent_input(const float *X, long ldx, const int64_t *idx, long M, int D, const float *Wdp,
                           const float *bdp, int use_ln0, int H, const float *x1, const uint32_t *mask1,
                           const float *rstd1, float *x1dot, void *stream);
int harl_mlp_linear_wide(const float *x0n, long M, int KP, const float *Wp, int D, const float *bp, int H, void *w_img,
                         float *zout, void *stream);
int harl_act_ln_fwd(const float *z, long M, int H, int act, float *xhat, float *mean, float *rstd, void *stream);
int harl_act_bwd(float *dz, const float *xhat, const float *mean, const float *rstd, long M, int H, int act, void *stream);
int harl_act_ln_tangent(const float *zd1, const float *zd2, const float *xhat, const float *mean, const float *rstd, long M,
                        int H, int act, float *xhat_dot, void *stream);
int harl_mlp_tangent_wide(const float *x0n, long M, int KP, const float *Wdp, int D, const float *bdp, int H, void *w_img,
                          const float *x1, const uint32_t *mask1, const float *rstd1, float *x1dot, void *stream);
int harl_gru_gates(const float *xin, const float *W, int H, long n_slabs, float *out_r, float *out_z, float *out_n,
                   int acc_mask, void *stream);
int harl_gru_tangent(const float *g_r, const float *g_z, const float *g_nx, const float *g_nh, const float *mask_rows,
                     const float *Whh, const float *bihd, const float *bhhd, const float *hpm, const float *r,
                     const float *z, const float *n, const float *hn, const float *y, const float *rstd_y, int H, int L,
                     long m_pad, float *ydot, void *stream);
int harl_mlp_tangent_hidden(const float *xin_dot, const float *xin, long M, int HI, int HO, const float *Wp,
                            const float *Wdp, const float *bdp, const float *xprimal, const uint32_t *mask_in,
                            const float *rstd_in, float *xout_dot, void *stream);
int harl_mlp_tangent_hidden2(const float *xin_dot, const float *xin, long M, int HI, int HO, const float *Wp,
                             const float *Wdp, const float *bdp, void *w_img, const float *xprimal,
                             const uint32_t *mask_in, const float *rstd_in, float *xout_dot, void *stream);
int harl_actor_head_fvp(const float *xL, const float *xLdot, const uint32_t *relu_mask, const float *rstd, long M, int H,
                        const float *Whp, const float *bhp, const float *Whdp, const float *bhdp, const float *log_std,
                        float std_x_coef, float std_y_coef, int discrete, int act_dim, const float *avail, long m_valid,
                        long m_pad, float *dzL, float *dhead, void *stream);
int harl_trpo_fvp_finish(const float *grad, const float *vec, const float *log_std, float *out, long n, float m_global,
                         float damping, long logstd_off, int act_dim, float std_x_coef, float std_y_coef, void *stream);
int harl_trpo_cg_step(float *x, float *r, float *p, const float *avp, long n, float *state, void *scratch, void *stream);
#define HARL_TRPO_STATE 16
int harl_trpo_begin(const float *grad_sum, const double *scalars, long logstd_off, int act_dim, float *g, float *x, float *r,
                    float *p, long n, float *cg_state, double *st, void *scratch, void *stream);
int harl_trpo_step(const float *x, const float *fx, const float *g, const float *theta, float *theta_save, float *full_step,
                   long n, float kl_threshold, double *st, void *scratch, void *stream);
int harl_trpo_ls_candidate(const float *theta_save, const float *full_step, const double *st, float *theta, long n, void *stream);
int harl_trpo_ls_test(const double *scalars, double *kl_sum, double m_global, double kl_threshold, double accept_ratio,
                      double backtrack_coeff, double *st, void *stream);
int harl_reduce_scalars_set(const float *part_scalars, int n_blocks, double *scalars, void *stream);
int harl_zero_bytes(void *p, long bytes, void *stream);
int harl_trpo_kl_sum(const float *head_old, const float *head_new, const float *log_std_old, const float *log_std_new,
                     float std_x_coef, float std_y_coef, long M, int act_dim, int discrete, double *out_sum,
                     void *stream);

int harl_mlp_linear(const float *xin, long M, int HI, int HO, const float *Wp, const float *bp, float *xout, void *stream);
int harl_mlp_linear3(const float *x0, const float *x1, const float *x2, long M, int HI, int HO, const float *W0, const float *W1,
                     const float *W2, const float *b0, const float *b1, const float *b2, float *o0, float *o1, float *o2,
                     void *stream);
int harl_md_head_logp(const float *const *z, int n_groups, const int *sp, int n_heads, const int *nvec,
                      const int *head_group, long M, const float *actions, float *logp_out, const float *old_logp,
                      int old_w, float *factor, int agg_mean, float *head_out, long m_valid, long m_pad, void *stream);
int harl_md_head_loss(const float *const *z, float *const *dz, int n_groups, const int *sp, int n_heads, const int *nvec,
                      const int *head_group, long M, const int64_t *idx, const float *actions, const float *old_logp,
                      int old_w, const float *adv, const double *adv_moments, const float *factor, const float *active,
                      const float *ent_scale, double clip_param, float entropy_coef, int agg_mean, int mode, long m_valid,
                      long m_pad, float *logp_out, float *part_scalars, int n_blocks, void *stream);

int harl_cat_head_logp(const float *const *z, int n_groups, const int *sp, int n, long M, const int64_t *idx,
                       const float *actions, const float *avail, float *logp_out, float *ent_out, const float *old_logp,
                       float *factor, float *head_out, long m_valid, long m_pad, void *stream);
int harl_cat_head_loss(float *const *z, int n_groups, const int *sp, int n, long M, const int64_t *idx, const float *actions,
                       const float *avail, const float *old_logp, const float *adv, const double *adv_moments,
                       const float *factor, const float *active, double clip_param, float entropy_coef, int mode,
                       long m_valid, long m_pad, float *logp_out, float *part_scalars, int n_blocks, void *stream);

int harl_update_supported(int D, int H, int act_dim, int kind);
int harl_update_fwd_actor(const float *x0n, long M, int D, int H, const float *W1p, const float *b1p, const float *W2p,
                          const float *b2p, const float *Whp, const float *bhp, const float *log_std, float std_x_coef,
                          float std_y_coef, int discrete, int act_dim, const float *actions, const float *avail,
                          const float *old_logp, const float *adv, const double *adv_moments, const float *factor,
                          const float *active, double clip_param, float entropy_coef, int agg_mean, int trpo,
                          float *logp_out, float *dz2, float *part_scalars, float *dw_part_head, int n_part_rows,
                          float *xh1, uint32_t *rmask1, float *rstd1, void *stream);
int harl_update_logp(const float *x0n, long M, int D, int H, const float *W1p, const float *b1p, const float *W2p,
                     const float *b2p, const float *Whp, const float *bhp, const float *log_std, float std_x_coef,
                     float std_y_coef, int discrete, int act_dim, const float *actions, const float *avail,
                     float *logp_out, const float *old_logp, float *factor, int agg_mean, float *head_out, void *stream);
int harl_update_fwd_critic(const float *x0n, long M, int D, int H, const float *W1p, const float *b1p, const float *W2p,
                           const float *b2p, const float *Whp, const float *bhp, const float *value_preds,
                           const float *returns, const float *vn_stats, float clip_param, int use_clipped, int use_huber,
                           float huber_delta, float *dz2, float *part_scalars, float *dw_part_head, int n_part_rows,
                           float *xh1, uint32_t *rmask1, float *rstd1, void *stream);
int harl_update_last_actor(const float *xin, long M, int H, const float *Wp, const float *bp, const float *Whp,
                           const float *bhp, const float *log_std, float std_x_coef, float std_y_coef, int discrete,
                           int act_dim, const int64_t *idx, const float *actions, const float *avail,
                           const float *old_logp, const float *adv, const double *adv_moments, const float *factor,
                           const float *active, double clip_param, float entropy_coef, int agg_mean, int trpo,
                           float *logp_out, float *dz, float *part_scalars, float *dw_part_head, int n_part_rows,
                           void *stream);
int harl_update_last_critic(const float *xin, long M, int H, const float *Wp, const float *bp, const float *Whp,
                            const float *bhp, const int64_t *idx, const float *value_preds, const float *returns,
                            const float *vn_stats, float clip_param, int use_clipped, int use_huber, float huber_delta,
                            float *dz, float *part_scalars, float *dw_part_head, int n_part_rows, void *stream);
int harl_update_values(const float *x0n, long M, int D, int H, const float *W1p, const float *b1p, const float *W2p,
                       const float *b2p, const float *Whp, const float *bhp, float *values, void *stream);
int harl_update_bwd(const float *x0n, const float *dz2, long M, int D, int H, const float *W1p, const float *b1p,
                    const float *W2p, float *dw_part1, float *dw_part2, int n_part_rows, void *stream);

int harl_gru_fwd(const float *xin, const float *mask_rows, const float *h0, const float *Wih, const float *bih,
                 const float *Whh, const float *bhh, int H, int L, long m_pad, float *y, float *rstd_y, float *hpm, float *r,
                 float *z, float *n, float *hn, float *h_last, int save, float *gi_ws, void *stream);
int harl_gru_cell_init(const float *h0, const float *mask_rows, int H, long m_pad, float *hpm0, void *stream);
int harl_gru_cell_fwd(const float *gi_r, const float *gi_z, const float *gi_n, const float *gh_r, const float *gh_z,
                      const float *gh_n, const float *hpm, const float *mask_next, int H, long m_pad, float *r, float *z,
                      float *n, float *hn, float *h, float *hpm_next, float *h_last, void *stream);
int harl_gru_cell_bwd(const float *dh_out, const float *t_r, const float *t_z, const float *t_n, const float *mask_next,
                      const float *r, const float *z, const float *n, const float *hn, const float *hpm, int H, long m_pad,
                      float *gz, float *dr, float *dz, float *dn, float *dhn, void *stream);
int harl_rownorm(const float *x, long M, int H, float *y, float *rstd, void *stream);
int harl_gru_cell_tangent(const float *gia_r, const float *gia_z, const float *gia_n, const float *gib_r, const float *gib_z,
                          const float *gib_n, const float *gha_r, const float *gha_z, const float *gha_n, const float *ghb_r,
                          const float *ghb_z, const float *ghb_n, const float *r, const float *z, const float *n,
                          const float *hn, const float *hpm, const float *hpm_dot, const float *mask_next, int H, long m_pad,
                          float *h_dot, float *hpm_dot_next, void *stream);
int harl_gru_bwd(const float *dhout, const float *mask_rows, const float *Wih, const float *Whh, const float *hpm,
                 const float *r, const float *z, const float *n, const float *hn, int H, int L, long m_pad,
                 const float *xmlp, const uint32_t *mask_mlp, const float *rstd_mlp, float *dr, float *dz, float *dn,
                 float *dhn, float *dz_mlp, void *stream);

int harl_head_blocks(long M);
int harl_reduce_scalars(const float *part_scalars, int n_blocks, double *scalars, void *stream);

int harl_randperm_replay(const uint8_t *state_in, long state_bytes, long n, int32_t *out, uint32_t *scratch,
                         uint8_t *state_out);
int harl_rng_advance(const uint8_t *state_in, long state_bytes, long n_draws, uint8_t *state_out);
int harl_rng_jump(const uint8_t *state_in, long state_bytes, long n_draws, uint8_t *state_out);

int harl_comm_create(int world, int rank, long cap_bytes, int n_blocks, void *handle_out, void *ctx_out);
int harl_comm_connect(void *ctx, const void *all_handles);
int harl_comm_allreduce(void *ctx, void *msg, long n, int is_f64, void *stream);
int harl_comm_set_timeout(void *ctx, double seconds);
int harl_comm_status(void *ctx);
int harl_comm_destroy(void *ctx);

#ifdef __cplusplus
}
#endif
#endif
```

Measured before the change: 52.64 million transitions/s.

## Batch per-update fold and moments work into one head kernel; compute ValueNorm sums once

Adds a multi-job kernel that runs weight-folding rows and masked-moment reductions for several agents in one launch instead of separate per-agent launches. The logp pass can now read the incoming factor directly instead of copying it first. ValueNorm return sums are computed once per update and reused across critic epochs. Launch overhead and redundant reductions are reduced, at the cost of a more complex job-table dispatch and self-resetting ticket scratch.

```diff
diff --git a/harl_amd/_lib.py b/harl_amd/_lib.py
--- a/harl_amd/_lib.py
+++ b/harl_amd/_lib.py
@@ -27,6 +27,7 @@
     "harl_adv_normalize": [_vp, _vp, _vp, _l, _vp],
     "harl_factor_update": [_vp, _vp, _vp, _l, _i, _i, _vp],
     "harl_sum_sumsq": [_vp, _vp, _l, _vp, _vp],
+    "harl_sum_sumsq_set": [_vp, _vp, _l, _vp, _vp, _vp],
     "harl_valuenorm_apply": [_vp, _vp, _d, _d, _vp],
     "harl_gradnorm_clip_adam": [_vp, _vp, _vp, _vp, _l, _vp, _i, _f, _d, _d, _d, _f, _f, _d, _d, _vp, _vp],
     "harl_fold_linear": [_vp] * 6 + [_i, _i, _vp],
@@ -73,6 +74,7 @@
     "harl_gru_bwd": [_vp] * 9 + [_i, _i, _l] + [_vp] * 8 + [_vp],
     "harl_fold_linear_tangent": [_vp] * 9 + [_i, _i, _vp],
     "harl_fold_table": [_vp, _vp, _vp, _i, _i, _vp],
+    "harl_update_head": [_vp, _i, _vp],
     "harl_unfold_table": [_vp, _vp, _vp, _vp, _i, _i, _vp],
     "harl_fold_tangent_table": [_vp, _vp, _vp, _vp, _i, _i, _vp],
     "harl_mlp_tangent_input": [_vp, _l, _vp, _l, _i, _vp, _vp, _i, _i, _vp, _vp, _vp, _vp, _vp],
@@ -84,7 +86,7 @@
     "harl_trpo_kl_sum": [_vp, _vp, _vp, _vp, _f, _f, _l, _i, _i, _vp, _vp],
     "harl_update_supported": [_i, _i, _i, _i],
     "harl_update_fwd_actor": [_vp, _l, _i, _i] + [_vp] * 7 + [_f, _f, _i, _i] + [_vp] * 7 + [_d, _f, _i, _i] + [_vp] * 4 + [_i] + [_vp] * 4,
-    "harl_update_logp": [_vp, _l, _i, _i] + [_vp] * 7 + [_f, _f, _i, _i] + [_vp] * 5 + [_i, _vp, _vp],
+    "harl_update_logp": [_vp, _l, _i, _i] + [_vp] * 7 + [_f, _f, _i, _i] + [_vp] * 5 + [_i, _vp, _vp, _vp],
     "harl_update_last_actor": [_vp, _l, _i] + [_vp] * 5 + [_f, _f, _i, _i] + [_vp] * 8 + [_d, _f, _i, _i] + [_vp] * 4 + [_i, _vp],
     "harl_update_last_critic": [_vp, _l, _i] + [_vp] * 8 + [_f, _i, _i, _f] + [_vp] * 3 + [_i, _vp],
     "harl_update_fwd_critic": [_vp, _l, _i, _i] + [_vp] * 9 + [_f, _i, _i, _f] + [_vp] * 3 + [_i] + [_vp] * 4,
@@ -255,6 +257,27 @@
     return True
 
 
+UPDATE_HEAD_MAX = 32
+
+
+class HeadJob(C.Structure):
+    _fields_ = [("kind", _i), ("n_layers", _i), ("total_rows", _i), ("reserved", _i), ("param", _vp), ("packs", _vp),
+                ("table", _vp), ("x", _vp), ("active", _vp), ("out3", _vp), ("scratch", _vp), ("n", _l)]
+
+
+def head_fold_job(param: int, packs: int, table: int, n_layers: int, total_rows: int) -> HeadJob:
+    return HeadJob(0, n_layers, total_rows, 0, param, packs, table, None, None, None, None, 0)
+
+
+def head_moments_job(x: int, active: Optional[int], n: int, out3: int, scratch_ptr: int) -> HeadJob:
+    return HeadJob(1, 0, 0, 0, None, None, None, x, active, out3, scratch_ptr, n)
+
+
+def update_head(jobs, tag: Optional[str] = "update_head") -> None:
+    table = (HeadJob * len(jobs))(*jobs)
+    call("harl_update_head", table, len(jobs), stream(), tag=tag)
+
+
 SCRATCH_BYTES = {"mm": 24640, "cg": 1088}
 _scratch: Dict[tuple, torch.Tensor] = {}
 
diff --git a/harl_amd/csrc/elementwise.hip b/harl_amd/csrc/elementwise.hip
--- a/harl_amd/csrc/elementwise.hip
+++ b/harl_amd/csrc/elementwise.hip
@@ -168,12 +168,13 @@
   unsigned ticket;
 };
 
-__global__ __launch_bounds__(256) void k_masked_moments(const float *__restrict__ x, const float *__restrict__ active,
-                                                        long n, double *__restrict__ out3, MmScratch *__restrict__ ws) {
+template <bool SET>
+__device__ __forceinline__ void mm_block(const float *__restrict__ x, const float *__restrict__ active, long n,
+                                         double *__restrict__ out3, MmScratch *__restrict__ ws, unsigned bid, unsigned nblk) {
   double(*g_mm_part)[3] = ws->part;
   unsigned &g_mm_ticket = ws->ticket;
   double s1 = 0, s2 = 0, cnt = 0;
-  for (long i = (long)blockIdx.x * blockDim.x + threadIdx.x; i < n; i += (long)gridDim.x * blockDim.x) {
+  for (long i = (long)bid * blockDim.x + threadIdx.x; i < n; i += (long)nblk * blockDim.x) {
     float a = active ? active[i] : 1.f;
     if (a != 0.f) {
       double v = x[i];
@@ -195,13 +196,13 @@
   }
   __syncthreads();
   if (threadIdx.x < 3)
-    __hip_atomic_store(&g_mm_part[blockIdx.x][threadIdx.x],
+    __hip_atomic_store(&g_mm_part[bid][threadIdx.x],
                        sh[threadIdx.x][0] + sh[threadIdx.x][1] + sh[threadIdx.x][2] + sh[threadIdx.x][3], __ATOMIC_RELAXED,
                        __HIP_MEMORY_SCOPE_AGENT);
   __syncthreads();
   if (threadIdx.x == 0) {
     __threadfence();
-    s_last = __hip_atomic_fetch_add(&g_mm_ticket, 1u, __ATOMIC_ACQ_REL, __HIP_MEMORY_SCOPE_AGENT) == gridDim.x - 1 ? 1u : 0u;
+    s_last = __hip_atomic_fetch_add(&g_mm_ticket, 1u, __ATOMIC_ACQ_REL, __HIP_MEMORY_SCOPE_AGENT) == nblk - 1 ? 1u : 0u;
   }
   __syncthreads();
   if (!s_last) return;
@@ -209,7 +210,7 @@
   __shared__ double red[3][256];
   for (int k = 0; k < 3; ++k) {
     double t = 0;
-    for (unsigned b = threadIdx.x; b < gridDim.x; b += 256)
+    for (unsigned b = threadIdx.x; b < nblk; b += 256)
       t += __hip_atomic_load(&g_mm_part[b][k], __ATOMIC_RELAXED, __HIP_MEMORY_SCOPE_AGENT);
     red[k][threadIdx.x] = t;
   }
@@ -217,8 +218,15 @@
   if (threadIdx.x < 3) {
     double t = 0;
     for (int i = 0; i < 256; ++i) t += red[threadIdx.x][i];
-    out3[threadIdx.x] += t;
-  }
+    if (SET) out3[threadIdx.x] = t;
+    else out3[threadIdx.x] += t;
+  }
+  if (threadIdx.x == 0) __hip_atomic_store(&g_mm_ticket, 0u, __ATOMIC_RELAXED, __HIP_MEMORY_SCOPE_AGENT);
+}
+
+__global__ __launch_bounds__(256) void k_masked_moments(const float *__restrict__ x, const float *__restrict__ active,
+                                                        long n, double *__restrict__ out3, MmScratch *__restrict__ ws) {
+  mm_block<false>(x, active, n, out3, ws, blockIdx.x, gridDim.x);
 }
 
 static_assert(sizeof(MmScratch) <= HARL_MM_SCRATCH_BYTES, "HARL_MM_SCRATCH_BYTES too small");
@@ -444,6 +452,65 @@
   return check_launch("harl_sum_sumsq");
 }
 
+__global__ __launch_bounds__(256) void k_sum_sumsq_set(const float *__restrict__ x, const int64_t *__restrict__ idx, long m,
+                                                       double *__restrict__ out2, MmScratch *__restrict__ ws) {
+  double s1 = 0, s2 = 0;
+  for (long i = (long)blockIdx.x * blockDim.x + threadIdx.x; i < m; i += (long)gridDim.x * blockDim.x) {
+    double v = x[idx ? idx[i] : i];
+    s1 += v;
+    s2 += v * v;
+  }
+  s1 = wave_reduce_sum_d(s1);
+  s2 = wave_reduce_sum_d(s2);
+  __shared__ double sh[2][4];
+  __shared__ unsigned s_last;
+  int w = threadIdx.x >> 6, l = threadIdx.x & 63;
+  if (l == 0) {
+    sh[0][w] = s1;
+    sh[1][w] = s2;
+  }
+  __syncthreads();
+  if (threadIdx.x < 2)
+    __hip_atomic_store(&ws->part[blockIdx.x][threadIdx.x],
+                       sh[threadIdx.x][0] + sh[threadIdx.x][1] + sh[threadIdx.x][2] + sh[threadIdx.x][3], __ATOMIC_RELAXED,
+                       __HIP_MEMORY_SCOPE_AGENT);
+  __syncthreads();
+  if (threadIdx.x == 0) {
+    __threadfence();
+    s_last = __hip_atomic_fetch_add(&ws->ticket, 1u, __ATOMIC_ACQ_REL, __HIP_MEMORY_SCOPE_AGENT) == gridDim.x - 1 ? 1u : 0u;
+  }
+  __syncthreads();
+  if (!s_last) return;
+  __threadfence();
+  __shared__ double red[2][256];
+  for (int k = 0; k < 2; ++k) {
+    double t = 0;
+    for (unsigned b = threadIdx.x; b < gridDim.x; b += 256)
+      t += __hip_atomic_load(&ws->part[b][k], __ATOMIC_RELAXED, __HIP_MEMORY_SCOPE_AGENT);
+    red[k][threadIdx.x] = t;
+  }
+  __syncthreads();
+  if (threadIdx.x < 2) {
+    double t = 0;
+    for (int i = 0; i < 256; ++i) t += red[threadIdx.x][i];
+    out2[threadIdx.x] = t;
+  }
+  if (threadIdx.x == 0) __hip_atomic_store(&ws->ticket, 0u, __ATOMIC_RELAXED, __HIP_MEMORY_SCOPE_AGENT);
+}
+
+extern "C" int harl_sum_sumsq_set(const float *x, const int64_t *idx, long m, double *sums2, void *scratch, void *stream) {
+  MmScratch *ws = static_cast<MmScratch *>(scratch);
+  if (!x || !sums2 || !ws || (reinterpret_cast<uintptr_t>(ws) & 7) != 0) {
+    set_error("harl_sum_sumsq_set: needs x, sums2 and HARL_MM_SCRATCH_BYTES of 8-byte aligned, zero-filled device scratch");
+    return -2;
+  }
+  long nb = m <= 0 ? 1 : (m + 2047) / 2048;
+  if (nb > 1024) nb = 1024;
+  static_assert(MM_MAX_BLOCKS >= 1024, "one scratch row per block");
+  hipLaunchKernelGGL(k_sum_sumsq_set, dim3((unsigned)nb), dim3(256), 0, (hipStream_t)stream, x, idx, m < 0 ? 0 : m, sums2, ws);
+  return check_launch("harl_sum_sumsq_set");
+}
+
 __global__ void k_valuenorm_apply(float *__restrict__ vn, const double *__restrict__ sums2, double count, float w,
                                   float omw) {
 #pragma clang fp contract(off)
@@ -889,9 +956,9 @@
   return check_launch("harl_unfold_table");
 }
 
-__global__ __launch_bounds__(64) void k_fold_table(const float *__restrict__ p, float *__restrict__ packs,
-                                                   const int *__restrict__ tab, int n_layers) {
-  int o = blockIdx.x, l = 0;
+__device__ __forceinline__ void fold_table_row(const float *__restrict__ p, float *__restrict__ packs,
+                                               const int *__restrict__ tab, int n_layers, int o, int lane) {
+  int l = 0;
   for (; l < n_layers; ++l) {
     if (o < tab[l * TS + 4]) break;
     o -= tab[l * TS + 4];
@@ -903,19 +970,90 @@
   const float *gamma = t[2] >= 0 ? p + t[2] : nullptr, *beta = t[3] >= 0 ? p + t[3] : nullptr;
   float *Wp = packs + t[6], *bp = packs + t[7];
   float acc = 0.f;
-  for (int k = threadIdx.x; k < in_dim; k += 64) {
+  for (int k = lane; k < in_dim; k += 64) {
     float w = W[(long)o * in_dim + k];
     Wp[(long)o * in_dim + k] = gamma ? w * gamma[k] : w;
     if (beta) acc += w * beta[k];
   }
   acc = wave_reduce_sum(acc);
-  if (threadIdx.x == 0) bp[o] = b[o] + acc;
+  if (lane == 0) bp[o] = b[o] + acc;
+}
+
+__global__ __launch_bounds__(64) void k_fold_table(const float *__restrict__ p, float *__restrict__ packs,
+                                                   const int *__restrict__ tab, int n_layers) {
+  fold_table_row(p, packs, tab, n_layers, blockIdx.x, threadIdx.x);
 }
 
 extern "C" int harl_fold_table(const float *param, float *packs, const int *table, int n_layers, int total_rows, void *stream) {
   if (n_layers <= 0 || total_rows <= 0) return 0;
   hipLaunchKernelGGL(k_fold_table, dim3(total_rows), dim3(64), 0, (hipStream_t)stream, param, packs, table, n_layers);
   return check_launch("harl_fold_table");
+}
+
+struct UpdateHeadArgs {
+  harl_head_job j[HARL_UPDATE_HEAD_MAX];
+  int blk_end[HARL_UPDATE_HEAD_MAX];
+  int n;
+};
+
+__global__ __launch_bounds__(256) void k_update_head(const UpdateHeadArgs a) {
+  int j = 0;
+  while (j + 1 < a.n && (int)blockIdx.x >= a.blk_end[j]) ++j;
+  const int b0 = j ? a.blk_end[j - 1] : 0;
+  const harl_head_job &q = a.j[j];
+  if (q.kind == HARL_HEAD_FOLD) {
+    const int o = ((int)blockIdx.x - b0) * 4 + (threadIdx.x >> 6);
+    if (o < q.total_rows)
+      fold_table_row(q.param, q.packs, q.table, q.n_layers, o, threadIdx.x & 63);
+  } else {
+    mm_block<true>(q.x, q.active, q.n, q.out3, static_cast<MmScratch *>(q.scratch), blockIdx.x - b0, a.blk_end[j] - b0);
+  }
+}
+
+extern "C" int harl_update_head(const harl_head_job *jobs, int n_jobs, void *stream) {
+  if (n_jobs == 0) return 0;
+  if (!jobs || n_jobs < 0 || n_jobs > HARL_UPDATE_HEAD_MAX) {
+    set_error("harl_update_head: 1 .. HARL_UPDATE_HEAD_MAX jobs");
+    return -2;
+  }
+  UpdateHeadArgs a;
+  long end = 0;
+  for (int j = 0; j < n_jobs; ++j) {
+    const harl_head_job &q = jobs[j];
+    long nb;
+    if (q.kind == HARL_HEAD_FOLD) {
+      if (!q.param || !q.packs || !q.table || q.n_layers <= 0 || q.total_rows <= 0) {
+        set_error("harl_update_head: a fold job needs param, packs, table, n_layers and total_rows");
+        return -2;
+      }
+      nb = ((long)q.total_rows + 3) / 4;
+    } else if (q.kind == HARL_HEAD_MOMENTS) {
+      if (!q.x || !q.out3 || q.n < 0 || !q.scratch || (reinterpret_cast<uintptr_t>(q.scratch) & 7) != 0) {
+        set_error("harl_update_head: a moments job needs x, out3 and HARL_MM_SCRATCH_BYTES of 8-byte aligned scratch of its own");
+        return -2;
+      }
+      for (int i = 0; i < j; ++i)
+        if (jobs[i].kind == HARL_HEAD_MOMENTS && jobs[i].scratch == q.scratch) {
+          set_error("harl_update_head: two moments jobs share one scratch block");
+          return -2;
+        }
+      nb = (q.n + 2047) / 2048;
+      nb = nb < 1 ? 1 : (nb > MM_MAX_BLOCKS ? MM_MAX_BLOCKS : nb);
+    } else {
+      set_error("harl_update_head: unknown job kind");
+      return -2;
+    }
+    a.j[j] = q;
+    end += nb;
+    a.blk_end[j] = (int)end;
+  }
+  for (int j = n_jobs; j < HARL_UPDATE_HEAD_MAX; ++j) {
+    a.j[j] = harl_head_job{};
+    a.blk_end[j] = (int)end;
+  }
+  a.n = n_jobs;
+  hipLaunchKernelGGL(k_update_head, dim3((unsigned)end), dim3(256), 0, (hipStream_t)stream, a);
+  return check_launch("harl_update_head");
 }
 
 __global__ __launch_bounds__(64) void k_fold_tangent_table(const float *__restrict__ p, const float *__restrict__ vec,
diff --git a/harl_amd/csrc/heads.hip b/harl_amd/csrc/heads.hip
--- a/harl_amd/csrc/heads.hip
+++ b/harl_amd/csrc/heads.hip
@@ -516,6 +516,7 @@
   A.std_x_coef = std_x_coef; A.std_y_coef = std_y_coef; A.act_dim = act_dim;
   A.actions = actions; A.avail = avail; A.old_logp = old_logp; A.agg_mean = agg_mean;
   A.logp_out = logp_out; A.factor_out = factor; A.n_slabs = n_slabs_of(M);
+  A.factor_in = factor;
   if (factor && !old_logp) {
     set_error("harl_actor_head_logp: factor update needs old_logp");
     return -2;
diff --git a/harl_amd/csrc/heads_common.h b/harl_amd/csrc/heads_common.h
--- a/harl_amd/csrc/heads_common.h
+++ b/harl_amd/csrc/heads_common.h
@@ -470,7 +470,7 @@
     R.adv = A.adv[row];
     R.fct = A.factor_in ? A.factor_in[row] : 1.f;
   } else {
-    R.fct = A.factor_out ? A.factor_out[jc] : 1.f;
+    R.fct = A.factor_in ? A.factor_in[jc] : 1.f;
   }
 }
 
@@ -512,7 +512,7 @@
     R.adv = A.adv[row];
     R.fct = *(A.factor_in ? A.factor_in + row : mapped);
   } else {
-    R.fct = *(A.factor_out ? A.factor_out + jc : mapped);
+    R.fct = *(A.factor_in ? A.factor_in + jc : mapped);
   }
 }
 
@@ -613,7 +613,7 @@
             if (d < D) A.logp_out[j * D + d] = logp_d[d];
         }
       }
-      if (A.factor_out) A.factor_out[j] = R.fct * imp;
+      if (A.factor_out) A.factor_out[j] = (A.factor_in ? R.fct : 1.f) * imp;
     }
     return false;
   }
diff --git a/harl_amd/csrc/update.hip b/harl_amd/csrc/update.hip
--- a/harl_amd/csrc/update.hip
+++ b/harl_amd/csrc/update.hip
@@ -685,7 +685,7 @@
                                 const float *W2p, const float *b2p, const float *Whp, const float *bhp,
                                 const float *log_std, float std_x_coef, float std_y_coef, int discrete, int act_dim,
                                 const float *actions, const float *avail, float *logp_out, const float *old_logp,
-                                float *factor, int agg_mean, float *head_out, void *stream) {
+                                float *factor, int agg_mean, float *head_out, const float *factor_in, void *stream) {
   if (M <= 0) return 0;
   if (D < 1 || D > 64) return bad("harl_update_logp: input width must be <= 64");
   if (factor && !old_logp) return bad("harl_update_logp: factor update needs old_logp");
@@ -696,6 +696,7 @@
   A.std_x_coef = std_x_coef; A.std_y_coef = std_y_coef; A.act_dim = act_dim;
   A.actions = actions; A.avail = avail; A.old_logp = old_logp; A.agg_mean = agg_mean;
   A.logp_out = logp_out; A.factor_out = factor; A.n_slabs = U.n_slabs;
+  A.factor_in = factor_in;
   return dispatch_fwd_actor<false>(U, A, H, discrete, (hipStream_t)stream);
 }
 
diff --git a/harl_amd/dropin.py b/harl_amd/dropin.py
--- a/harl_amd/dropin.py
+++ b/harl_amd/dropin.py
@@ -59,6 +59,8 @@
         _ensure_update_state = ours._ensure_update_state
         _critic_first_ok = getattr(ours, "_critic_first_ok", None)
         _prepare_inputs = ours._prepare_inputs
+        _update_head = ours._update_head
+        _on_gpu = ours._on_gpu
         _fp_normalised_advantages = ours._fp_normalised_advantages
         _check_comms = ours._check_comms
         warmup = ours.warmup
diff --git a/harl_amd/happo.py b/harl_amd/happo.py
--- a/harl_amd/happo.py
+++ b/harl_amd/happo.py
@@ -62,9 +62,14 @@
             g["lr"] = lr
 
     def _logp_pass(self, obs, actions, avail, M, logp_out, old_logp=None, factor=None, head_out=None,
-                   rnn_states=None, masks=None, h_last=False, reuse_trunk=False):
+                   rnn_states=None, masks=None, h_last=False, reuse_trunk=False, factor_in=None):
         net = self.actor
         agg = int(self.action_aggregation == "mean")
+        if factor_in is not None:
+            one_launch = not (net.grouped and not net.recurrent) and not reuse_trunk and net.fused_update_ok(None, train=False)
+            if not one_launch:
+                factor.copy_(factor_in.reshape(factor.shape))
+                factor_in = None
         if net.grouped and not net.recurrent:
             if not reuse_trunk:
                 net.forward_trunk(obs, None, M, for_backward=False)
@@ -80,7 +85,7 @@
         if not reuse_trunk and net.fused_update_ok(None, train=False):
             call("harl_update_logp", *net.fused_args(obs, M), ptr(net.log_std()), net.std_x_coef, net.std_y_coef,
                  int(net.discrete), net.act_dim, ptr(actions), ptr(avail), ptr(logp_out), ptr(old_logp), ptr(factor), agg,
-                 ptr(head_out), stream(), tag="update_logp")
+                 ptr(head_out), ptr(factor if factor_in is None else factor_in), stream(), tag="update_logp")
             return None
         if not net.recurrent:
             if not reuse_trunk:
diff --git a/harl_amd/nets.py b/harl_amd/nets.py
--- a/harl_amd/nets.py
+++ b/harl_amd/nets.py
@@ -313,6 +313,17 @@
             call("harl_fold_linear", ptr(fp[wo:]), ptr(fp[bo:]), ptr(fp[go:]) if go >= 0 else None,
                  ptr(fp[beo:]) if beo >= 0 else None, ptr(pa[pw:]), ptr(pa[pb:]), o, k, s)
         self._fold_version = ver
+
+    def fold_job(self):
+        if not self._packs:
+            self._build_tables()
+        if self.table is None or os.environ.get("HARL_FOLD_TABLE", "1") == "0":
+            return None
+        return _lib.head_fold_job(ptr(self.flat_param), ptr(self.pack_arena), ptr(self.table), self.n_entries,
+                                  sum(r[4] for r in self._table_rows))
+
+    def fold_done(self) -> None:
+        self._fold_version = self.flat_param._version
 
     def _ensure_ws(self, M: int) -> None:
         if M <= self._max_rows:
diff --git a/harl_amd/runner.py b/harl_amd/runner.py
--- a/harl_amd/runner.py
+++ b/harl_amd/runner.py
@@ -126,7 +126,7 @@
         actor_train_infos = []
         for x in self.actor:
             x.actor.invalidate_caches()
-        self._prepare_inputs()
+        mom_all = self._prepare_inputs()
         factor = torch.ones(T, N, 1, dtype=torch.float32, device=dev)
         advantages = self.critic_buffer.advantages
         if self.state_type == "FP":
@@ -137,11 +137,12 @@
             rng_sync()
             agent_order = [int(a) for a in torch.randperm(self.num_agents).numpy()]
         fast = [hasattr(a, "masked_moments") for a in self.actor]
-        mom_all = torch.zeros(self.num_agents, 3, dtype=torch.float64, device=dev)
-        for a in range(self.num_agents):
-            if fast[a]:
-                adv_a = advantages if self.state_type == "EP" else advantages[:, :, a].contiguous()
-                self.actor[a].masked_moments(self.actor_buffer[a], adv_a, mom_all[a])
+        if mom_all is None:
+            mom_all = torch.zeros(self.num_agents, 3, dtype=torch.float64, device=dev)
+            for a in range(self.num_agents):
+                if fast[a]:
+                    adv_a = advantages if self.state_type == "EP" else advantages[:, :, a].contiguous()
+                    self.actor[a].masked_moments(self.actor_buffer[a], adv_a, mom_all[a])
         self.comm.all_reduce_sum(mom_all)
         if self._counts_host is None or self._counts_host.numel() != self.num_agents:
             self._counts_host = torch.empty(self.num_agents, dtype=torch.float64, pin_memory=torch.cuda.is_available())
@@ -280,14 +281,16 @@
                 ps.wait_stream(torch.cuda.current_stream(dev))
                 keep_alive += [factor, self._logp_old]
                 with torch.cuda.stream(ps):
-                    new_factor = factor.clone()
-                    actor._logp_pass(obs, actions, avail, B, None, old_logp=self._logp_old, factor=new_factor.reshape(B), **rnn_kw)
+                    new_factor = torch.empty_like(factor)
+                    actor._logp_pass(obs, actions, avail, B, None, old_logp=self._logp_old, factor=new_factor.reshape(B),
+                                     factor_in=factor.reshape(B), **rnn_kw)
                     factor_ev = torch.cuda.Event()
                     factor_ev.record(ps)
                 factor = new_factor
                 continue
-            new_factor = factor.clone()
-            actor._logp_pass(obs, actions, avail, B, None, old_logp=self._logp_old, factor=new_factor.reshape(B), **rnn_kw)
+            new_factor = torch.empty_like(factor)
+            actor._logp_pass(obs, actions, avail, B, None, old_logp=self._logp_old, factor=new_factor.reshape(B),
+                             factor_in=factor.reshape(B), **rnn_kw)
             factor = new_factor
         if keep_alive:
             torch.cuda.current_stream(dev).wait_stream(self._post_stream)
@@ -322,8 +325,8 @@
 
     def _prepare_inputs(self) -> None:
         from . import graphs
-        if os.environ.get("HARL_X0N_MULTI", "1") == "0" or self.device.type != "cuda" or graphs.enabled():
-            return
+        if os.environ.get("HARL_X0N_MULTI", "1") == "0" or not self._on_gpu() or graphs.enabled():
+            return None
         from .nets import prepare_x0n_multi
         items = []
         for a, buf in zip(self.actor, self.actor_buffer):
@@ -335,11 +338,46 @@
         if crit:
             c.critic.invalidate_caches()
             items.append((c.critic, self.critic_buffer.flat("share_obs")))
-        for net, _ in items:
-            net.fold()
+        head = os.environ.get("HARL_UPDATE_HEAD", "1") != "0"
+        if not head:
+            for net, _ in items:
+                net.fold()
         built = prepare_x0n_multi([(net, X, X.shape[0]) for net, X in items])
         if crit and built:
             c._inputs_prepared = True
+        return self._update_head([net for net, _ in items]) if head else None
+
+    def _on_gpu(self) -> bool:
+        return self.device.type == "cuda"
+
+    def _update_head(self, nets):
+        jobs, done = [], []
+        for net in nets:
+            j = net.fold_job()
+            if j is None or len(jobs) >= _lib.UPDATE_HEAD_MAX:
+                net.fold()
+            else:
+                jobs.append(j)
+                done.append(net)
+        A = self.num_agents
+        mom_all = None
+        n = self.algo_args["train"]["episode_length"] * (self.col_hi - self.col_lo)
+        if (self.state_type == "EP" and n >= 1 and all(hasattr(a, "masked_moments") for a in self.actor)
+                and len(jobs) + A <= _lib.UPDATE_HEAD_MAX):
+            words = _lib.SCRATCH_BYTES["mm"] // 8
+            if getattr(self, "_head_scratch", None) is None or self._head_scratch.numel() != A * words:
+                self._head_scratch = torch.zeros(A * words, dtype=torch.float64, device=self.device)
+                self._head_mom = torch.zeros(A, 3, dtype=torch.float64, device=self.device)
+            mom_all = self._head_mom
+            adv = self.critic_buffer.advantages
+            for a in range(A):
+                jobs.append(_lib.head_moments_job(ptr(adv), ptr(self.actor_buffer[a].flat("active_masks")), n,
+                                                  ptr(mom_all[a]), ptr(self._head_scratch[a * words:])))
+        if jobs:
+            _lib.update_head(jobs)
+        for net in done:
+            net.fold_done()
+        return mom_all
 
     def graph_stats(self) -> dict:
         from .graphs import sum_stats
diff --git a/harl_amd/traffic.py b/harl_amd/traffic.py
--- a/harl_amd/traffic.py
+++ b/harl_amd/traffic.py
@@ -142,7 +142,11 @@
     M, D, disc, ad = a[1], a[2], a[13], a[14]
     w = 1 if disc else ad
     return M * (4.0 * _kp(D) + 4.0 * w + (4.0 * ad if a[16] else 0.0) + (4.0 * w if a[17] else 0.0) + (4.0 * w if a[18] else 0.0)
-                + (8.0 if a[19] else 0.0) + (4.0 * ad if a[21] else 0.0))
+                + (4.0 if a[19] else 0.0) + (4.0 if a[19] and a[22] else 0.0) + (4.0 * ad if a[21] else 0.0))
+
+
+def _update_head(a: Sequence) -> float:
+    return float(sum(8.0 * a[0][j].n + 24.0 for j in range(a[1]) if a[0][j].kind == 1))
 
 
 def _update_fwd_critic(a: Sequence) -> float:
@@ -208,6 +212,7 @@
     "harl_critic_head_loss": _critic_head_loss,
     "harl_update_fwd_actor": _update_fwd_actor,
     "harl_update_logp": _update_logp,
+    "harl_update_head": _update_head,
     "harl_update_fwd_critic": _update_fwd_critic,
     "harl_update_values": _update_values,
     "harl_update_last_actor": _update_last_actor,
diff --git a/harl_amd/v_critic.py b/harl_amd/v_critic.py
--- a/harl_amd/v_critic.py
+++ b/harl_amd/v_critic.py
@@ -40,6 +40,7 @@
         self.critic_optimizer = FusedAdam(self.critic, self.critic_lr, self.opti_eps, self.weight_decay)
         self.comm = Comm()
         self.shard = None
+        self._vn_sums_ready = False
         self._inputs_prepared = False
         self._info = torch.zeros(2, dtype=torch.float64, device=self.device)
         self._grad_tap = None
@@ -110,7 +111,7 @@
                 bool(self.use_huber_loss), float(self.huber_delta), float(self.value_loss_coef), bool(self.use_max_grad_norm),
                 float(self.max_grad_norm), tuple(g["betas"]), float(g["eps"]), float(g["weight_decay"]),
                 None if vn is None else vn.beta, e("HARL_FUSED_UPDATE"), e("HARL_BWD_FUSED"), e("HARL_BWD_K64"),
-                e("HARL_TRUNK_FUSED"))
+                e("HARL_TRUNK_FUSED"), self._vn_sums_ready)
         key = warm + (p(share_obs), p(idx), p(value_preds), p(returns), None if vn is None else (p(vn.stats), p(vn._sums)),
                       p(self._info), p(net.flat_param), p(net.pack_arena), p(opt.exp_avg), p(opt._hyper_dev), opt._hyper_rows)
         G.run(warm, key, step, opt)
@@ -118,7 +119,9 @@
     def _step(self, share_obs, idx, m, m_global, value_preds, returns, vn: Optional[ValueNorm], seq=None):
         net = self.critic
         s = stream()
-        if vn is not None:
+        if vn is not None and self._vn_sums_ready:
+            vn.apply_sums(m_global)
+        elif vn is not None:
             vidx = seq["valid_idx"] if seq is not None else idx
             vn.update(returns, vidx, count=m_global, reduce_fn=self.comm.all_reduce_sum if self.comm.enabled else None,
                       local_count=(seq["L"] * seq["m"] if seq is not None else m))
@@ -233,6 +236,7 @@
 
     def _epochs(self, buf, share_obs, value_preds, returns, value_normalizer, A, B, n_global, graph: bool):
         dev = self.device
+        sums_set = False
         for _ in range(self.critic_epoch):
             if self.use_recurrent_policy or self.use_naive_recurrent_policy:
                 for seq in buf.recurrent_batches(self.critic_num_mini_batch, self.data_chunk_length,
@@ -247,7 +251,16 @@
                 continue
             if self.critic_num_mini_batch == 1:
                 consume_randperm(n_global)
-                self._update_core(share_obs, None, B, n_global, value_preds, returns, value_normalizer, _graph=graph)
+                if value_normalizer is not None and os.environ.get("HARL_VN_SUMS_ONCE", "1") != "0":
+                    if not sums_set:
+                        value_normalizer.set_sums(returns, reduce_fn=self.comm.all_reduce_sum if self.comm.enabled else None,
+                                                  local_count=B)
+                        sums_set = True
+                    self._vn_sums_ready = True
+                try:
+                    self._update_core(share_obs, None, B, n_global, value_preds, returns, value_normalizer, _graph=graph)
+                finally:
+                    self._vn_sums_ready = False
                 yield
                 continue
             sampler = minibatch_indices(n_global, self.critic_num_mini_batch, dev)
diff --git a/harl_amd/valuenorm.py b/harl_amd/valuenorm.py
--- a/harl_amd/valuenorm.py
+++ b/harl_amd/valuenorm.py
@@ -20,6 +20,7 @@
         self.epsilon = float(epsilon)
         self.stats = torch.zeros(3, dtype=torch.float32, device=self.device)
         self._sums = torch.zeros(2, dtype=torch.float64, device=self.device)
+        self._scratch = None
 
     @property
     def running_mean(self):
@@ -54,6 +55,23 @@
         call("harl_valuenorm_apply", ptr(self.stats), ptr(self._sums), float(count if count is not None else m),
              self.beta, stream())
 
+    @torch.no_grad()
+    def set_sums(self, input_vector, reduce_fn=None, local_count: Optional[int] = None) -> None:
+        x = _as_dev(input_vector, self.device).reshape(-1)
+        m = x.numel() if local_count is None else local_count
+        if m > 0:
+            if getattr(self, "_scratch", None) is None:
+                self._scratch = torch.zeros(_lib.SCRATCH_BYTES["mm"] // 8, dtype=torch.float64, device=self.device)
+            call("harl_sum_sumsq_set", ptr(x), None, m, ptr(self._sums), ptr(self._scratch), stream())
+        else:
+            self._sums.zero_()
+        if reduce_fn is not None:
+            reduce_fn(self._sums)
+
+    @torch.no_grad()
+    def apply_sums(self, count) -> None:
+        call("harl_valuenorm_apply", ptr(self.stats), ptr(self._sums), float(count), self.beta, stream())
+
     def normalize(self, input_vector):
         x = _as_dev(input_vector, self.device)
         mean, var = self.running_mean_var()
diff --git a/include/harl_hip.h b/include/harl_hip.h
--- a/include/harl_hip.h
+++ b/include/harl_hip.h
@@ -37,6 +37,7 @@
                        int agg_mean, void *stream);
 
 int harl_sum_sumsq(const float *x, const int64_t *idx, long m, double *sums2, void *stream);
+int harl_sum_sumsq_set(const float *x, const int64_t *idx, long m, double *sums2, void *scratch, void *stream);
 int harl_valuenorm_apply(float *vn_stats, const double *sums2, double count, double beta, void *stream);
 
 int harl_gradnorm_clip_adam(float *param, float *grad, float *exp_avg, float *exp_avg_sq, long n,
@@ -110,6 +111,20 @@
 int harl_reduce_partials_multi(const float *part, const int *table, int n_layers, int n_wg, long total_elems,
                                float *dwp, void *stream);
 int harl_fold_table(const float *param, float *packs, const int *table, int n_layers, int total_rows, void *stream);
+#define HARL_UPDATE_HEAD_MAX 32
+#define HARL_HEAD_FOLD 0
+#define HARL_HEAD_MOMENTS 1
+typedef struct {
+  int kind, n_layers, total_rows, reserved;
+  const float *param;
+  float *packs;
+  const int *table;
+  const float *x, *active;
+  double *out3;
+  void *scratch;
+  long n;
+} harl_head_job;
+int harl_update_head(const harl_head_job *jobs, int n_jobs, void *stream);
 int harl_unfold_table(const float *param, float *grad, const float *dwp, const int *table, int n_layers, int total_cols,
                       void *stream);
 int harl_fold_tangent_table(const float *param, const float *vec, float *pack_d, const int *table, int n_layers,
@@ -225,7 +240,8 @@
 int harl_update_logp(const float *x0n, long M, int D, int H, const float *W1p, const float *b1p, const float *W2p,
                      const float *b2p, const float *Whp, const float *bhp, const float *log_std, float std_x_coef,
                      float std_y_coef, int discrete, int act_dim, const float *actions, const float *avail,
-                     float *logp_out, const float *old_logp, float *factor, int agg_mean, float *head_out, void *stream);
+                     float *logp_out, const float *old_logp, float *factor, int agg_mean, float *head_out,
+                     const float *factor_in, void *stream);
 int harl_update_fwd_critic(const float *x0n, long M, int D, int H, const float *W1p, const float *b1p, const float *W2p,
                            const float *b2p, const float *Whp, const float *bhp, const float *value_preds,
                            const float *returns, const float *vn_stats, float clip_param, int use_clipped, int use_huber,
```

New measurement: 52.90 million transitions/s (median of 6 runs). No clear change (+0.5%).
